# giladfrid009/WTracker

Measured on AMD Instinct MI355X. Metric: frames/sec YOLOv8s+ResMLP sim loop @640x640, higher is better.
Workload: dtype f16x3; 1 GPU; BASELINE configs[2]: full sim loop, YOLOv8s (nc=1, seeded synthetic weights) + ResMLP(imaging-100ms_pred-40ms_moving-50ms, reference weights); batch_per_gpu=64, lanes_per_gpu=2, global_batch=64, headline_mode=f16x3, parallelism=single GPU

## Files before the change

wtracker_amd/csrc/conv3x3_halo.hip:

```cpp
#include "wtk_kernels.h"

#include <cstdlib>
#include <type_traits>

namespace wtk {

typedef _Float16 half8 __attribute__((ext_vector_type(8)));
typedef float floatx4 __attribute__((ext_vector_type(4)));

namespace {

template <typename T> struct ElemH;
template <> struct ElemH<_Float16> {
    static constexpr int CE = 8;
};
template <> struct ElemH<float> {
    static constexpr int CE = 4;
};

__device__ __forceinline__ float silu_h(float x) {
    return wtk_silu_scaled(x);
}

__device__ __forceinline__ void mma_h(const uint4 &wf, const uint4 &pf, floatx4 &acc, _Float16 *) {
    acc = __builtin_amdgcn_mfma_f32_16x16x32_f16(__builtin_bit_cast(half8, wf), __builtin_bit_cast(half8, pf), acc, 0, 0, 0);
}
__device__ __forceinline__ void mma_h(const uint4 &wf, const uint4 &pf, floatx4 &acc, float *) {
    acc = __builtin_amdgcn_mfma_f32_16x16x4f32(__builtin_bit_cast(float, wf.x), __builtin_bit_cast(float, pf.x), acc, 0, 0, 0);
    acc = __builtin_amdgcn_mfma_f32_16x16x4f32(__builtin_bit_cast(float, wf.y), __builtin_bit_cast(float, pf.y), acc, 0, 0, 0);
    acc = __builtin_amdgcn_mfma_f32_16x16x4f32(__builtin_bit_cast(float, wf.z), __builtin_bit_cast(float, pf.z), acc, 0, 0, 0);
    acc = __builtin_amdgcn_mfma_f32_16x16x4f32(__builtin_bit_cast(float, wf.w), __builtin_bit_cast(float, pf.w), acc, 0, 0, 0);
}

template <int NV> __device__ __forceinline__ void load_run_h(const _Float16 *p, float (&v)[NV]) {
#pragma unroll
    for (int i = 0; i < NV; i += 8) {
        half8 h = *reinterpret_cast<const half8 *>(p + i);
#pragma unroll
        for (int j = 0; j < 8; ++j) v[i + j] = (float)h[j];
    }
}
template <int NV> __device__ __forceinline__ void load_run_h(const float *p, float (&v)[NV]) {
#pragma unroll
    for (int i = 0; i < NV; i += 4) {
        float4 f = *reinterpret_cast<const float4 *>(p + i);
        v[i] = f.x, v[i + 1] = f.y, v[i + 2] = f.z, v[i + 3] = f.w;
    }
}
template <int NV> __device__ __forceinline__ void store_run_h(_Float16 *p, const float (&v)[NV]) {
#pragma unroll
    for (int i = 0; i < NV; i += 8) {
        half8 h;
#pragma unroll
        for (int j = 0; j < 8; ++j) h[j] = (_Float16)v[i + j];
        *reinterpret_cast<half8 *>(p + i) = h;
    }
}
template <int NV> __device__ __forceinline__ void store_run_h(float *p, const float (&v)[NV]) {
#pragma unroll
    for (int i = 0; i < NV; i += 4) *reinterpret_cast<float4 *>(p + i) = make_float4(v[i], v[i + 1], v[i + 2], v[i + 3]);
}

constexpr int kBM = 256;

template <bool RAW> __device__ __forceinline__ void lds_dma16(const char *src, char *lds_dst) {
    if constexpr (RAW) {
        const unsigned lds = (unsigned)(uintptr_t)(__attribute__((address_space(3))) char *)lds_dst;
        asm volatile("s_mov_b32 m0, %1\n\ts_nop 0\n\tglobal_load_lds_dwordx4 %0, off" ::"v"(src), "s"(lds) : "memory");
    } else {
        __builtin_amdgcn_global_load_lds((const __attribute__((address_space(1))) void *)src, (__attribute__((address_space(3))) void *)lds_dst, 16, 0, 0);
    }
}

#ifndef WTK_HALO_BUFFER_DMA
#define WTK_HALO_BUFFER_DMA 1
#endif
typedef int rsrc_t __attribute__((ext_vector_type(4)));
__device__ __forceinline__ rsrc_t make_rsrc(const void *base) {
    const unsigned long long b = (unsigned long long)base;
    rsrc_t r;
    r.x = (int)(unsigned)(b & 0xffffffffu);
    r.y = (int)(unsigned)((b >> 32) & 0xffffu);
    r.z = (int)0xffffff00u;
    r.w = 0x00020000;
    return r;
}
__device__ __forceinline__ void lds_dma16_buf(const rsrc_t &rs, unsigned voff, unsigned soff, char *lds_dst) {
    const unsigned lds = (unsigned)(uintptr_t)(__attribute__((address_space(3))) char *)lds_dst;
    asm volatile("s_mov_b32 m0, %3\n\ts_nop 0\n\tbuffer_load_dwordx4 %0, %1, %2 offen lds" ::"v"(voff), "s"(rs), "s"(soff), "s"(lds) : "memory");
}

__device__ __forceinline__ void wait_vmcnt(int n) {
    switch (n) {
    case 0: asm volatile("s_waitcnt vmcnt(0)" ::: "memory"); break;
    case 1: asm volatile("s_waitcnt vmcnt(1)" ::: "memory"); break;
    case 2: asm volatile("s_waitcnt vmcnt(2)" ::: "memory"); break;
    case 3: asm volatile("s_waitcnt vmcnt(3)" ::: "memory"); break;
    case 4: asm volatile("s_waitcnt vmcnt(4)" ::: "memory"); break;
    case 5: asm volatile("s_waitcnt vmcnt(5)" ::: "memory"); break;
    case 6: asm volatile("s_waitcnt vmcnt(6)" ::: "memory"); break;
    case 7: asm volatile("s_waitcnt vmcnt(7)" ::: "memory"); break;
    case 8: asm volatile("s_waitcnt vmcnt(8)" ::: "memory"); break;
    case 9: asm volatile("s_waitcnt vmcnt(9)" ::: "memory"); break;
    case 10: asm volatile("s_waitcnt vmcnt(10)" ::: "memory"); break;
    case 11: asm volatile("s_waitcnt vmcnt(11)" ::: "memory"); break;
    case 12: asm volatile("s_waitcnt vmcnt(12)" ::: "memory"); break;
    case 13: asm volatile("s_waitcnt vmcnt(13)" ::: "memory"); break;
    case 14: asm volatile("s_waitcnt vmcnt(14)" ::: "memory"); break;
    case 15: asm volatile("s_waitcnt vmcnt(15)" ::: "memory"); break;
    case 16: asm volatile("s_waitcnt vmcnt(16)" ::: "memory"); break;
    default: asm volatile("s_waitcnt vmcnt(0)" ::: "memory"); break;
    }
}

__device__ __forceinline__ bool halo_in_coords(const HaloArgs &a, int flat, int xs, int &n, int &iy, int &ix) {
    const int rho = (int)fdiv((unsigned)flat, a.d_pitch);
    const int cc = flat - rho * a.pitch;
    n = (int)fdiv((unsigned)rho, a.d_h1);
    iy = rho - n * (a.H + 1) - 1;
    ix = xs + cc - 1;
    return n < a.N && iy >= 0 && (unsigned)ix < (unsigned)a.W;
}
__device__ __forceinline__ bool halo_out_coords(const HaloArgs &a, int o, int xs, int &n, int &y, int &x) {
    const int q = (int)fdiv((unsigned)o, a.d_pitch);
    x = o - q * a.pitch;
    n = (int)fdiv((unsigned)q, a.d_h1);
    y = q - n * (a.H + 1);
    return n < a.N && y < a.H && x < a.S && xs + x < a.W;
}

template <typename T, int KMAX>
__device__ __forceinline__ void halo_piece_offsets(const HaloArgs &a, int o0, int xs, int n_base, int halo_rows, int wave, int lane, unsigned (&hoff)[KMAX],
                                                   unsigned &hvalid) {
    static_assert(KMAX <= 8, "one lane per (piece, row)");
    constexpr int CE = ElemH<T>::CE;
    const int hr_e = (wave + 8 * (lane >> 3)) * 8 + (lane & 7);
    int pn, iy, ix;
    const bool ok_e = halo_in_coords(a, o0 + hr_e, xs, pn, iy, ix) && hr_e < halo_rows;
    const unsigned row_e = ok_e ? (unsigned)(((((long long)(pn - n_base) * a.H + iy) * a.W + ix) * a.in_ld) * (long long)sizeof(T)) : 0xffffffffu;
    const unsigned lc_term = (unsigned)((((lane & 7) ^ ((lane >> 3) & 7)) * CE) * (int)sizeof(T));
    hvalid = 0;
#pragma unroll
    for (int q = 0; q < KMAX; ++q) {
        const unsigned v = (unsigned)__builtin_amdgcn_ds_bpermute((q * 8 + (lane >> 3)) * 4, (int)row_e);
        const bool ok = v != 0xffffffffu;
        hoff[q] = ok ? v + lc_term : 0u;
        hvalid |= ok ? (1u << q) : 0u;
    }
}
__device__ __forceinline__ void halo_out_pixel(const HaloArgs &a, int o_first, int xs, int lane, int &pix_e, int &col_e) {
    int n, y, x;
    const bool ok = halo_out_coords(a, o_first + lane, xs, n, y, x);
    col_e = xs + x;
    pix_e = ok ? (n * a.H + y) * a.W + col_e : -1;
}
__device__ __forceinline__ int lane_fetch(int src_lane, int v) { return __builtin_amdgcn_ds_bpermute(src_lane * 4, v); }

template <typename T, int BN, int NHALO, int MINW, int NWB, int HROWS, int BMT = 256, bool TAIL = false, bool SPLIT = false>
__global__ __launch_bounds__(512, MINW) void conv3x3_halo_kernel(const HaloArgs a) {
    static_assert(!SPLIT || (sizeof(T) == 2 && BN != 192 && (MINW <= 2 || (BN == 64 && BMT == 128 && NHALO == 1))),
                  "split mode: fp16 storage, 64 / 128 couts, 256-register budget (128 for the two-blocks-per-CU form: 64 couts x 128 pixels, one window buffer)");
#ifdef WTK_HALO_STAMPS
    const unsigned long long st_t0 = __builtin_amdgcn_s_memrealtime();
#endif
    asm volatile("" ::"s"(a.in), "s"(a.w), "s"(a.bias), "s"(a.zeros), "s"(a.in_ld), "s"(a.in_coff), "s"(a.N), "s"(a.H), "s"(a.W), "s"(a.Cin), "s"(a.CoutPad),
                 "s"(a.Kpad), "s"(a.S), "s"(a.pitch), "s"(a.strips), "s"(a.d_strips.mul), "s"(a.d_strips.sh1), "s"(a.d_strips.sh2), "s"(a.d_pitch.mul),
                 "s"(a.d_pitch.sh1), "s"(a.d_pitch.sh2), "s"(a.d_nct.mul), "s"(a.d_nct.sh1), "s"(a.d_nct.sh2), "s"(a.d_h1.mul), "s"(a.d_h1.sh1), "s"(a.d_h1.sh2), "s"(a.grid));
    constexpr int CE = ElemH<T>::CE;
    constexpr int CCH = 8 * CE;
    constexpr int WAVES_C = BN == 64 ? 1 : 2, WAVES_P = 8 / WAVES_C;
    constexpr int WC = BN / WAVES_C;
    constexpr int WP = BMT / WAVES_P, TP = WP / 16, TC = WC / 16, NV = 4 * TC;
    constexpr int WR = BN / 64;

    constexpr int kHaloBytesT = HROWS * 128;
    __shared__ __attribute__((aligned(16))) char halo0[kHaloBytesT];
    __shared__ __attribute__((aligned(16))) char halo1[NHALO == 2 ? kHaloBytesT : 16];
    static_assert(NWB == 2 || NWB == 3 || (NWB == 6 && NHALO == 2 && !TAIL && SPLIT), "slab ring: 2, 3 or 6 (split tiles, two window buffers, no fused tail)");
    constexpr bool kRing = NWB >= 3;
    __shared__ __attribute__((aligned(16))) char wbuf0[NWB > 3 ? 16 : BN * 128];
    __shared__ __attribute__((aligned(16))) char wbuf1[NWB > 3 ? 16 : BN * 128];
    __shared__ __attribute__((aligned(16))) char wbuf2[NWB == 3 ? BN * 128 : 16];
    __shared__ __attribute__((aligned(16))) char wring[NWB > 3 ? NWB * BN * 128 : 16];

    const int tid = threadIdx.x;
    const int lane = tid & 63;
    const int wave = __builtin_amdgcn_readfirstlane(tid >> 6);
    const int wave_p = wave / WAVES_C, wave_c = wave % WAVES_C;
    const int lr = lane & 15, lg = lane >> 4;

    const int nct = a.CoutPad / BN;
    int nwg = a.grid;
    if (a.n_dyn) {
        const int lim = min(max(*a.n_dyn, 0), a.N) * (a.H + 1) * a.pitch;
        const int live = ((lim + BMT - 1) / BMT) * a.strips * nct;
        if ((int)blockIdx.x >= live) return;
        nwg = min(nwg, live);
    }
    int L;
    {
        const int bid = blockIdx.x;
        const int xcd = bid & 7, q = nwg >> 3, r = nwg & 7;
        L = (xcd < r ? xcd * (q + 1) : r * (q + 1) + (xcd - r) * q) + (bid >> 3);
    }
    const unsigned t = fdiv((unsigned)L, a.d_nct);
    const int n0 = (L - (int)t * nct) * BN;
    const int rb = (int)fdiv(t, a.d_strips);
    const int strip = (int)t - rb * a.strips;
    const int o0 = rb * BMT;
    const int xs = strip * a.S;
    const int pitch = a.pitch;
    const int halo_rows = BMT + 2 * pitch + 2;
    const int halo_pieces = (halo_rows + 7) >> 3;
    const int n_base = (int)fdiv(fdiv((unsigned)o0, a.d_pitch), a.d_h1);

    const T *in = reinterpret_cast<const T *>(a.in) + (long long)n_base * a.H * a.W * a.in_ld + a.in_coff;
    const T *wgt = reinterpret_cast<const T *>(a.w);
    const char *zero_page = reinterpret_cast<const char *>(a.zeros);

    constexpr int kMaxPiecesPerWave = (HROWS / 8 + 7) / 8;
    unsigned hoff[kMaxPiecesPerWave];
    unsigned hvalid;
    halo_piece_offsets<T, kMaxPiecesPerWave>(a, o0, xs, n_base, halo_rows, wave, lane, hoff, hvalid);
    const char *img = reinterpret_cast<const char *>(in);
    auto issue_halo_piece = [&](char *buf, int q, int c) {
        const int piece = wave + 8 * q;
        if (piece >= halo_pieces) return;
        if constexpr (kRing && WTK_HALO_BUFFER_DMA) {
            lds_dma16_buf(make_rsrc(img), ((hvalid >> q) & 1u) ? hoff[q] : 0xffffffffu, (unsigned)(c * (CCH * (int)sizeof(T))), buf + piece * 1024);
        } else {
            const char *src = ((hvalid >> q) & 1u) ? img + (size_t)c * (CCH * sizeof(T)) + hoff[q] : zero_page;
            lds_dma16<kRing>(src, buf + piece * 1024);
        }
    };
    auto issue_halo_piece_always = [&](char *buf, int q, int c) __attribute__((always_inline)) {
        constexpr int kPieces = HROWS / 8;
        static_assert(kPieces >= 16, "window buffer too small");
        const bool back = q > 0 && wave + 8 * q >= kPieces;
        const int piece = back ? wave + 8 * (q - 1) : wave + 8 * q;
        const unsigned off = back ? hoff[q > 0 ? q - 1 : 0] : hoff[q];
        const bool ok = back ? ((hvalid >> (q > 0 ? q - 1 : 0)) & 1u) : ((hvalid >> q) & 1u);
        if constexpr (kRing && WTK_HALO_BUFFER_DMA) {
            lds_dma16_buf(make_rsrc(img), ok ? off : 0xffffffffu, (unsigned)(c * (CCH * (int)sizeof(T))), buf + piece * 1024);
        } else {
            const char *src = ok ? img + (size_t)c * (CCH * sizeof(T)) + off : zero_page;
            lds_dma16<kRing>(src, buf + piece * 1024);
        }
    };
    const int wrow0 = tid >> 3, wp = tid & 7;
    unsigned wvoff[WR];
#pragma unroll
    for (int i = 0; i < WR; ++i) {
        const int row = wrow0 + 64 * i;
        const int key = ((row >> 1) & 1) | (((row / NV) & 3) << 1);
        wvoff[i] = (unsigned)(((long long)row * a.Kpad + (wp ^ key) * CE) * (long long)sizeof(T));
    }
    const char *wtile = reinterpret_cast<const char *>(wgt + (long long)n0 * a.Kpad);
    auto issue_weights = [&](char *buf, int tap, int c) {
        if constexpr (kRing && WTK_HALO_BUFFER_DMA) {
            const rsrc_t rs = make_rsrc(wtile);
            const unsigned so = (unsigned)((tap * a.Cin + c * CCH) * (int)sizeof(T));
#pragma unroll
            for (int i = 0; i < WR; ++i) lds_dma16_buf(rs, wvoff[i], so, buf + (64 * i + 8 * wave) * 128);
        } else {
            const char *ub = wtile + ((size_t)tap * a.Cin + (size_t)c * CCH) * sizeof(T);
#pragma unroll
            for (int i = 0; i < WR; ++i) lds_dma16<kRing>(ub + wvoff[i], buf + (64 * i + 8 * wave) * 128);
        }
    };

    floatx4 acc[TC][TP];
    floatx4 acc1[SPLIT ? TC : 1][SPLIT ? TP : 1];
#pragma unroll
    for (int i = 0; i < TC; ++i)
#pragma unroll
        for (int j = 0; j < TP; ++j) {
            acc[i][j] = (floatx4){0.f, 0.f, 0.f, 0.f};
            if constexpr (SPLIT) acc1[i][j] = (floatx4){0.f, 0.f, 0.f, 0.f};
        }

    const int wrow_l = wave_c * WC + (lr >> 2) * NV + (lr & 3);
    const int wkey_l = ((wrow_l >> 1) & 1) | (((wrow_l / NV) & 3) << 1);
    const unsigned wfrag0 = wrow_l * 128 + ((lg ^ wkey_l) << 4);
    const int prow0 = wave_p * WP + lr;

    auto compute_tap = [&](const char *halo, const char *wb, int tapoff) {
        const int base = prow0 + tapoff;
        const unsigned pfrag0 = base * 128 + ((lg ^ (base & 7)) << 4);
        if constexpr (SPLIT) {
            uint4 ph[TP], wh[TC], wl[TC], pl[TP];
#pragma unroll
            for (int j = 0; j < TP; ++j) ph[j] = *reinterpret_cast<const uint4 *>(halo + pfrag0 + j * 2048);
#pragma unroll
            for (int i = 0; i < TC; ++i) wh[i] = *reinterpret_cast<const uint4 *>(wb + wfrag0 + i * 512);
#pragma unroll
            for (int i = 0; i < TC; ++i) wl[i] = *reinterpret_cast<const uint4 *>(wb + (wfrag0 ^ 64u) + i * 512);
#pragma unroll
            for (int j = 0; j < TP; ++j) pl[j] = *reinterpret_cast<const uint4 *>(halo + (pfrag0 ^ 64u) + j * 2048);
#pragma unroll
            for (int i = 0; i < TC; ++i)
#pragma unroll
                for (int j = 0; j < TP; ++j) {
                    mma_h(wh[i], ph[j], acc[i][j], (T *)nullptr);
                    mma_h(wl[i], ph[j], acc1[i][j], (T *)nullptr);
                }
#pragma unroll
            for (int i = 0; i < TC; ++i)
#pragma unroll
                for (int j = 0; j < TP; ++j) mma_h(wh[i], pl[j], acc1[i][j], (T *)nullptr);
            return;
        }
#pragma unroll
        for (int kh2 = 0; kh2 < 2; ++kh2) {
            const unsigned pa = kh2 ? (pfrag0 ^ 64u) : pfrag0;
            const unsigned wa = kh2 ? (wfrag0 ^ 64u) : wfrag0;
            uint4 pf[TP], wf[TC];
#pragma unroll
            for (int j = 0; j < TP; ++j) pf[j] = *reinterpret_cast<const uint4 *>(halo + pa + j * 2048);
#pragma unroll
            for (int i = 0; i < TC; ++i) wf[i] = *reinterpret_cast<const uint4 *>(wb + wa + i * 512);
#pragma unroll
            for (int i = 0; i < TC; ++i)
#pragma unroll
                for (int j = 0; j < TP; ++j) mma_h(wf[i], pf[j], acc[i][j], (T *)nullptr);
        }
    };

    constexpr int kFr = (NWB > 3 && SPLIT) ? 2 * TP + 2 * TC : 1;
    uint4 fr[NWB > 3 ? 2 : 1][kFr];
    auto load_frags = [&](uint4(&f)[kFr], const char *halo, const char *wb, int tapoff) __attribute__((always_inline)) {
        if constexpr (NWB > 3 && SPLIT) {
            const int base = prow0 + tapoff;
            const unsigned pfrag0 = base * 128 + ((lg ^ (base & 7)) << 4);
#pragma unroll
            for (int j = 0; j < TP; ++j) f[j] = *reinterpret_cast<const uint4 *>(halo + pfrag0 + j * 2048);
#pragma unroll
            for (int i = 0; i < TC; ++i) f[2 * TP + i] = *reinterpret_cast<const uint4 *>(wb + wfrag0 + i * 512);
#pragma unroll
            for (int i = 0; i < TC; ++i) f[2 * TP + TC + i] = *reinterpret_cast<const uint4 *>(wb + (wfrag0 ^ 64u) + i * 512);
#pragma unroll
            for (int j = 0; j < TP; ++j) f[TP + j] = *reinterpret_cast<const uint4 *>(halo + (pfrag0 ^ 64u) + j * 2048);
        }
    };
    auto mma_frags = [&](const uint4(&f)[kFr]) __attribute__((always_inline)) {
        if constexpr (NWB > 3 && SPLIT) {
#pragma unroll
            for (int i = 0; i < TC; ++i)
#pragma unroll
                for (int j = 0; j < TP; ++j) {
                    mma_h(f[2 * TP + i], f[j], acc[i][j], (T *)nullptr);
                    mma_h(f[2 * TP + TC + i], f[j], acc1[i][j], (T *)nullptr);
                }
#pragma unroll
            for (int i = 0; i < TC; ++i)
#pragma unroll
                for (int j = 0; j < TP; ++j) mma_h(f[2 * TP + i], f[TP + j], acc1[i][j], (T *)nullptr);
        }
    };

    const int nchunks = a.Cin / CCH;
    const int cb = n0 + wave_c * WC + lg * NV;
#pragma unroll
    for (int i = 0; i < TC; ++i) {
        const floatx4 b4 = (floatx4){a.bias[cb + i * 4 + 0], a.bias[cb + i * 4 + 1], a.bias[cb + i * 4 + 2], a.bias[cb + i * 4 + 3]};
#pragma unroll
        for (int j = 0; j < TP; ++j) acc[i][j] = b4;
    }

#ifdef WTK_HALO_STAMPS
    const unsigned long long st_t1 = __builtin_amdgcn_s_memrealtime();
#endif
// ... 1158 lines not shown
#pragma unroll
            for (int i = 0; i < TC; ++i) wh[i] = *reinterpret_cast<const uint4 *>(wb + wfrag0 + i * 512);
#pragma unroll
            for (int i = 0; i < TC; ++i) wl[i] = *reinterpret_cast<const uint4 *>(wb + (wfrag0 ^ 64u) + i * 512);
#pragma unroll
            for (int j = 0; j < TP; ++j) pl[j] = *reinterpret_cast<const uint4 *>(win + (pfrag0 ^ 64u) + j * 2048);
#pragma unroll
            for (int i = 0; i < TC; ++i)
#pragma unroll
                for (int j = 0; j < TP; ++j) {
                    mma_h(wh[i], ph[j], acc[i][j], (T *)nullptr);
                    mma_h(wl[i], ph[j], acc1[i][j], (T *)nullptr);
                }
#pragma unroll
            for (int i = 0; i < TC; ++i)
#pragma unroll
                for (int j = 0; j < TP; ++j) mma_h(wh[i], pl[j], acc1[i][j], (T *)nullptr);
            return;
        }
#pragma unroll
        for (int kh2 = 0; kh2 < 2; ++kh2) {
            const unsigned pa = kh2 ? (pfrag0 ^ 64u) : pfrag0;
            const unsigned wa = kh2 ? (wfrag0 ^ 64u) : wfrag0;
            uint4 pf[TP], wf[TC];
#pragma unroll
            for (int j = 0; j < TP; ++j) pf[j] = *reinterpret_cast<const uint4 *>(win + pa + j * 2048);
#pragma unroll
            for (int i = 0; i < TC; ++i) wf[i] = *reinterpret_cast<const uint4 *>(wb + wa + i * 512);
#pragma unroll
            for (int i = 0; i < TC; ++i)
#pragma unroll
                for (int j = 0; j < TP; ++j) mma_h(wf[i], pf[j], acc[i][j], (T *)nullptr);
        }
    };

    constexpr int kStepTap[9] =      { 0, 2, 6, 8,  3, 5,  1, 7,  4};
    constexpr int kStepDY[9] =       {-1,-1, 0, 0,  0, 0, -1, 0,  0};
    constexpr int kStepDX[9] =       {-1, 0,-1, 0, -1, 0,  0, 0,  0};
    constexpr int kStepBuf[9] =      { 0, 0, 0, 0,  1, 1,  0, 0,  1};
    constexpr int kStepReq[9] =      { 2, 2, 2, 0,  KW,0,  KW,0,  KW};
    constexpr int kStepReqFrom[9] =  { 0, 2, 4, 0,  0, 0,  0, 0,  0};
    constexpr int kNextPy[9] =       { 0, 0, 0, 0,  1, 1,  0, 0,  1};
    constexpr int kNextPx[9] =       { 1, 1, 1, 1,  0, 0,  0, 0,  1};
    static_assert(KW == 6, "request schedule written for six window pieces per wave");
    const int nchunks = a.Cin / 64;

#pragma unroll
    for (int q = 0; q < KW; ++q) issue_piece(win0, q, 1, 1, 0);
    issue_weights(wbuf0, kStepTap[0], 0);
    issue_weights(wbuf1, kStepTap[1], 0);
    asm volatile("s_waitcnt vmcnt(0)" ::: "memory");
    __syncthreads();

    auto step = [&](auto s_tag, int c, bool more) __attribute__((always_inline)) {
        constexpr int S = decltype(s_tag)::value;
        const char *wcur = S % 3 == 0 ? wbuf0 : (S % 3 == 1 ? wbuf1 : wbuf2);
        char *wnext2 = (S + 2) % 3 == 0 ? wbuf0 : ((S + 2) % 3 == 1 ? wbuf1 : wbuf2);
        const char *wcur_win = kStepBuf[S] ? win1 : win0;
        char *wnext_win = kStepBuf[S] ? win0 : win1;
        compute_tap(wcur_win, wcur, (kStepDY[S] + 1) * pitch + (kStepDX[S] + 1));
        const int cn = S == 8 ? (more ? c + 1 : c) : c;
        if constexpr (kStepReq[S] > 0) {
#pragma unroll
            for (int q = 0; q < kStepReq[S]; ++q) issue_piece(wnext_win, kStepReqFrom[S] + q, kNextPy[S], kNextPx[S], cn);
        }
        if constexpr (S < 7)
            issue_weights(wnext2, kStepTap[S + 2], c);
        else
            issue_weights(wnext2, kStepTap[S - 7], more ? c + 1 : c);
        constexpr bool plane_end = S == 3 || S == 5 || S == 7 || S == 8;
        wait_vmcnt(plane_end ? WR : WR + kStepReq[S]);
        asm volatile("s_waitcnt lgkmcnt(0)" ::: "memory");
        __builtin_amdgcn_s_barrier();
        asm volatile("" ::: "memory");
    };
    for (int c = 0; c < nchunks; ++c) {
        const bool more = c + 1 < nchunks;
        step(std::integral_constant<int, 0>{}, c, more);
        step(std::integral_constant<int, 1>{}, c, more);
        step(std::integral_constant<int, 2>{}, c, more);
        step(std::integral_constant<int, 3>{}, c, more);
        step(std::integral_constant<int, 4>{}, c, more);
        step(std::integral_constant<int, 5>{}, c, more);
        step(std::integral_constant<int, 6>{}, c, more);
        step(std::integral_constant<int, 7>{}, c, more);
        step(std::integral_constant<int, 8>{}, c, more);
    }

    int pix_e, col_e;
    halo_out_pixel(a, o0 + wave_p * WP, 0, lane, pix_e, col_e);
    long long pixj[TP];
#pragma unroll
    for (int j = 0; j < TP; ++j) pixj[j] = lane_fetch(j * 16 + lr, pix_e);
    T *out = reinterpret_cast<T *>(a.out);
    if (cb + NV <= a.Cout) {
#pragma unroll
        for (int j = 0; j < TP; ++j) {
            if (pixj[j] < 0) continue;
            float v[NV];
#pragma unroll
            for (int i = 0; i < TC; ++i)
#pragma unroll
                for (int r = 0; r < 4; ++r) {
                    if constexpr (SPLIT)
                        v[i * 4 + r] = wtk_split_value(acc[i][j][r], acc1[i][j][r]);
                    else
                        v[i * 4 + r] = acc[i][j][r];
                }
            if (a.act) {
                wtk_silu_scaled_run<NV>(v);
            }
            if constexpr (SPLIT)
                wtk_split_store<NV>(reinterpret_cast<_Float16 *>(a.out) + pixj[j] * a.out_ld + a.out_coff, cb, v);
            else
                store_run_h<NV>(out + pixj[j] * a.out_ld + a.out_coff + cb, v);
        }
    }
    asm volatile("s_waitcnt vmcnt(0)" ::: "memory");
}

template <int BMT, bool SPLIT = false> hipError_t launch_s2(HaloArgs a, hipStream_t stream) {
    const long long blocks = (long long)a.blocks_per_strip * (a.CoutPad / 128);
    if (blocks <= 0 || blocks > 0x7fffffffLL) return hipErrorInvalidValue;
    a.d_nct = make_fastdiv((unsigned)(a.CoutPad / 128));
    a.d_bps = make_fastdiv((unsigned)a.blocks_per_strip);
    a.d_strips = make_fastdiv(1u);
    a.d_pitch = make_fastdiv((unsigned)a.pitch);
    a.d_h1 = make_fastdiv((unsigned)(a.H + 1));
    a.grid = (int)blocks;
    hipLaunchKernelGGL((conv3x3_s2_kernel<BMT, SPLIT>), dim3((unsigned)blocks), dim3(512), 0, stream, a);
    return hipGetLastError();
}

template <typename T, int BN, int HROWS> hipError_t launch_hp(HaloArgs a, int num_cus, hipStream_t stream) {
    const long long tiles = (long long)a.strips * a.blocks_per_strip * (a.CoutPad / BN);
    if (tiles <= 0 || tiles > 0x3fffffffLL || num_cus < 8) return hipErrorInvalidValue;
    if (kBM + 2 * a.pitch + 2 > HROWS || (a.Cin / (8 * ElemH<T>::CE)) % 2 != 0) return hipErrorInvalidValue;
    a.d_nct = make_fastdiv((unsigned)(a.CoutPad / BN));
    a.d_bps = make_fastdiv((unsigned)a.blocks_per_strip);
    a.d_strips = make_fastdiv((unsigned)a.strips);
    a.d_pitch = make_fastdiv((unsigned)a.pitch);
    a.d_h1 = make_fastdiv((unsigned)(a.H + 1));
    const long long cap = num_cus / 8 * 8;
    const unsigned grid = (unsigned)(tiles < cap ? tiles : cap);
    a.grid = (int)grid;
    hipLaunchKernelGGL((conv3x3_halo_pkernel<T, BN, HROWS>), dim3(grid), dim3(512), 0, stream, a);
    return hipGetLastError();
}

template <typename T, int BN, int NHALO, int MINW, int NWB, int HROWS, int BMT = 256, bool TAIL = false, bool SPLIT = false> hipError_t launch_h(HaloArgs a, hipStream_t stream) {
    const long long blocks = (long long)a.strips * a.blocks_per_strip * (a.CoutPad / BN);
    if (blocks <= 0 || blocks > 0x7fffffffLL) return hipErrorInvalidValue;
    if (BMT + 2 * a.pitch + 2 > HROWS || (long long)a.blocks_per_strip * BMT < (long long)a.N * (a.H + 1) * a.pitch) return hipErrorInvalidValue;
    a.d_nct = make_fastdiv((unsigned)(a.CoutPad / BN));
    a.d_bps = make_fastdiv((unsigned)a.blocks_per_strip);
    a.d_strips = make_fastdiv((unsigned)a.strips);
    a.d_pitch = make_fastdiv((unsigned)a.pitch);
    a.d_h1 = make_fastdiv((unsigned)(a.H + 1));
    a.grid = (int)blocks;
    hipLaunchKernelGGL((conv3x3_halo_kernel<T, BN, NHALO, MINW, NWB, HROWS, BMT, TAIL, SPLIT>), dim3((unsigned)blocks), dim3(512), 0, stream, a);
    return hipGetLastError();
}

}

bool halo_eligible(int k, int stride, int cin, int is_f16) {
    const int cch = is_f16 ? 64 : 32;
    return k == 3 && stride == 1 && cin % cch == 0;
}

bool split_halo_eligible(int k, int stride, int cin, int cout) { return k == 3 && stride == 1 && cin % 32 == 0 && cout % 64 == 0; }
int split_halo_cout_tile(int cout_stored) { return cout_stored % 128 == 0 ? 128 : 64; }

hipError_t launch_conv3x3_halo_split(const HaloArgs &a, hipStream_t stream) {
    const int bn = (a.narrow && !a.tail_w) ? 64 : split_halo_cout_tile(a.Cout);
    if (a.Cin % 64 != 0 || a.CoutPad % bn != 0 || a.Cout != a.CoutPad || a.slabs == 2) return hipErrorInvalidValue;
    if (a.tail_w && a.Cout == 128) {
        if (a.res || a.out2 || !a.tail_bias || !a.tail_out || a.tail_kpad != 256 || a.tail_cout < 1 || a.tail_cout > 32 || !a.tail_f32 || a.tail_ld % 4 || a.tail_coff % 4) return hipErrorInvalidValue;
    } else if (a.tail_w && (a.Cout != 64 || a.res || a.out2 || !a.tail_bias || !a.tail_out || a.tail_kpad != 128 || a.tail_cout != 64 || (a.tail_f32 ? (a.tail_ld % 4 || a.tail_coff % 4) : (a.tail_ld % 64 || a.tail_coff % 64))))
        return hipErrorInvalidValue;
    if (a.in_ld % 64 || a.in_coff % 64 || a.out_ld % 64 || a.out_coff % 64 || a.Kpad != 9 * a.Cin) return hipErrorInvalidValue;
    if (a.pitch != (a.strips == 1 ? a.S + 1 : a.S + 2) || kBM + 2 * a.pitch + 2 > kHaloRowsMax || a.strips * a.S < a.W || (a.strips == 1 && a.S != a.W))
        return hipErrorInvalidValue;
    const int bm = a.bm == 128 ? 128 : kBM;
    if ((long long)a.blocks_per_strip * bm < (long long)a.N * (a.H + 1) * a.pitch) return hipErrorInvalidValue;
    if (a.res && (a.res_ld % 64 || a.res_coff % 64)) return hipErrorInvalidValue;
    if (a.out2 && (a.out2_ld % 64 || a.out2_coff % 64)) return hipErrorInvalidValue;
    if (bn == 128 && a.tail_w) return bm == 128 ? launch_h<_Float16, 128, 2, 2, 3, kHaloRowsMax, 128, true, true>(a, stream) : launch_h<_Float16, 128, 2, 2, 3, kHaloRowsMax, 256, true, true>(a, stream);
    if (bn == 128) return bm == 128 ? launch_h<_Float16, 128, 2, 2, 3, kHaloRowsMax, 128, false, true>(a, stream) : launch_h<_Float16, 128, 2, 2, 3, kHaloRowsMax, 256, false, true>(a, stream);
    if (a.tail_w) return bm == 128 ? launch_h<_Float16, 64, 2, 2, 3, kHaloRowsMax, 128, true, true>(a, stream) : launch_h<_Float16, 64, 2, 2, 3, kHaloRowsMax, 256, true, true>(a, stream);
    if (a.deep && bm == 128) return launch_h<_Float16, 64, 2, 1, 6, kHaloRowsMax, 128, false, true>(a, stream);
    return bm == 128 ? launch_h<_Float16, 64, 2, 2, 3, kHaloRowsMax, 128, false, true>(a, stream) : launch_h<_Float16, 64, 2, 2, 3, kHaloRowsMax, 256, false, true>(a, stream);
}

int halo_rows_max(int cout_stored, int slabs) { return (slabs == 3 && halo_cout_tile(cout_stored) == 192) ? kHaloRowsSmall : kHaloRowsMax; }

void halo_geometry(int H, int W, int rows_max, int *S, int *pitch, int *strips, int *blocks_per_strip, int bm) {
    const int smax = (rows_max - kBM - 2) / 2 - 2;
    *strips = (W + smax - 1) / smax;
    *S = (W + *strips - 1) / *strips;
    *pitch = *S + 2;
    *blocks_per_strip = (H * *pitch + bm - 1) / bm;
}

void halo_geometry_stacked(int N, int H, int W, int rows_max, int *S, int *pitch, int *strips, int *blocks_per_strip, int bm) {
    const int smax = (rows_max - kBM - 2) / 2 - 2;
    *strips = (W + smax - 1) / smax;
    *S = (W + *strips - 1) / *strips;
    *pitch = *strips == 1 ? *S + 1 : *S + 2;
    *blocks_per_strip = (int)(((long long)N * (H + 1) * *pitch + bm - 1) / bm);
}

bool s2win_eligible(int k, int stride, int cin, int cout, int cout_pad, int is_f16, int wo, bool plain) {
    return is_f16 && k == 3 && stride == 2 && cin % 64 == 0 && cin >= 128 && cout_pad % 128 == 0 && cout % 16 == 0 && plain && 256 + (wo + 1) + 2 <= kS2Rows;
}

hipError_t launch_conv3x3_s2(const HaloArgs &a, hipStream_t stream) {
    if (a.Cin % 64 || a.CoutPad % 128 || a.Cout > a.CoutPad || a.Cout % 16 || a.out2 || a.tail_w || a.res || a.Kpad < 9 * a.Cin || a.Kpad % 64) return hipErrorInvalidValue;
    if (a.in_ld % 8 || a.in_coff % 8 || a.out_ld % 8 || a.out_coff % 8) return hipErrorInvalidValue;
    const int bm = a.bm == 128 ? 128 : 256;
    if (a.strips != 1 || a.S != a.W || a.pitch != a.W + 1 || bm + a.pitch + 2 > kS2Rows) return hipErrorInvalidValue;
    if ((long long)a.blocks_per_strip * bm < (long long)a.N * (a.H + 1) * a.pitch) return hipErrorInvalidValue;
    return bm == 128 ? launch_s2<128>(a, stream) : launch_s2<256>(a, stream);
}

bool split_s2win_eligible(int k, int stride, int cin, int cout, int cout_pad, int wo, bool plain) {
    return k == 3 && stride == 2 && cin % 32 == 0 && cout_pad % 128 == 0 && cout == cout_pad && plain && 256 + (wo + 1) + 2 <= kS2Rows;
}
hipError_t launch_conv3x3_s2_split(const HaloArgs &a, hipStream_t stream) {
    if (a.Cin % 64 || a.CoutPad % 128 || a.Cout != a.CoutPad || a.out2 || a.tail_w || a.res || a.Kpad != 9 * a.Cin) return hipErrorInvalidValue;
    if (a.in_ld % 64 || a.in_coff % 64 || a.out_ld % 64 || a.out_coff % 64) return hipErrorInvalidValue;
    const int bm = a.bm == 128 ? 128 : 256;
    if (a.strips != 1 || a.S != a.W || a.pitch != a.W + 1 || bm + a.pitch + 2 > kS2Rows) return hipErrorInvalidValue;
    if ((long long)a.blocks_per_strip * bm < (long long)a.N * (a.H + 1) * a.pitch) return hipErrorInvalidValue;
    return bm == 128 ? launch_s2<128, true>(a, stream) : launch_s2<256, true>(a, stream);
}

int ws64_rows_max() { return kWsRows; }

bool ws64_eligible(int k, int stride, int cin, int cout, int cout_pad, int is_f16, bool has_out2, bool has_tail) {
    return is_f16 && k == 3 && stride == 1 && cin == 64 && cout == 64 && cout_pad == 64 && !has_out2 && !has_tail;
}

hipError_t launch_conv3x3_ws64(const HaloArgs &a, int num_cus, hipStream_t stream) {
    if (a.Cin != 64 || a.Cout != 64 || a.CoutPad != 64 || a.out2 || a.tail_w || a.Kpad < 576 || a.Kpad % 64) return hipErrorInvalidValue;
    if (a.in_ld % 8 || a.in_coff % 8 || a.out_ld % 8 || a.out_coff % 8) return hipErrorInvalidValue;
    if (a.res && (a.res_ld % 8 || a.res_coff % 8)) return hipErrorInvalidValue;
    if (a.pitch != (a.strips == 1 ? a.S + 1 : a.S + 2) || a.strips * a.S < a.W || (a.strips == 1 && a.S != a.W)) return hipErrorInvalidValue;
    if ((long long)a.blocks_per_strip * 256 < (long long)a.N * (a.H + 1) * a.pitch) return hipErrorInvalidValue;
    return launch_ws64(a, num_cus, stream);
}

int halo_cout_tile(int cout_stored) { return cout_stored % 128 == 0 ? 128 : (cout_stored % 192 == 0 ? 192 : 64); }

hipError_t launch_conv3x3_halo(const HaloArgs &a, int is_f16, hipStream_t stream) {
    const int ce = is_f16 ? 8 : 4;
    const int cch = 8 * ce;
    const int bn = (a.narrow && !a.tail_w && a.CoutPad % 64 == 0) ? 64 : halo_cout_tile(a.Cout);
    if (a.Cin % cch != 0 || a.CoutPad % bn != 0 || a.Cout > a.CoutPad || a.Cout % (bn == 192 ? 24 : 16) != 0) return hipErrorInvalidValue;
    if (a.in_ld % ce || a.in_coff % ce || a.out_ld % ce || a.out_coff % ce || a.Kpad % cch || a.Kpad < 9 * a.Cin) return hipErrorInvalidValue;
    if (a.pitch != (a.strips == 1 ? a.S + 1 : a.S + 2) || kBM + 2 * a.pitch + 2 > kHaloRowsMax || a.strips * a.S < a.W || (a.strips == 1 && a.S != a.W))
        return hipErrorInvalidValue;
    if (a.tail_w && (!is_f16 || (bn != 64 && bn != 128) || a.Cout != bn || a.CoutPad != bn || a.res || a.out2 || !a.tail_bias || !a.tail_out ||
                     a.tail_kpad < bn || a.tail_kpad % 8 || a.tail_ld % 8 || a.tail_coff % 8 || a.slabs == 2))
        return hipErrorInvalidValue;
    const int bm = a.bm == 128 ? 128 : kBM;
    if ((long long)a.blocks_per_strip * bm < (long long)a.N * (a.H + 1) * a.pitch) return hipErrorInvalidValue;
    if (a.res && (a.res_ld % ce || a.res_coff % ce)) return hipErrorInvalidValue;
    if (a.out2 && (a.out2_ld % ce || a.out2_coff % ce)) return hipErrorInvalidValue;
    const int nchunks = a.Cin / cch;
    const long long tiles = (long long)a.strips * a.blocks_per_strip * (a.CoutPad / bn);
    if (a.slabs != 2 && !a.tail_w && bm == kBM && a.persist_cus > 0 && 2 * tiles >= 3 * (long long)a.persist_cus && nchunks % 2 == 0 && (bn == 128 || bn == 192)) {
        if (is_f16) return bn == 128 ? launch_hp<_Float16, 128, kHaloRowsMax>(a, a.persist_cus, stream) : launch_hp<_Float16, 192, kHaloRowsSmall>(a, a.persist_cus, stream);
        return bn == 128 ? launch_hp<float, 128, kHaloRowsMax>(a, a.persist_cus, stream) : launch_hp<float, 192, kHaloRowsSmall>(a, a.persist_cus, stream);
    }
    if (a.tail_w && bn == 128) {
        if (bm == 128) return launch_h<_Float16, 128, 2, 2, 3, kHaloRowsMax, 128, true>(a, stream);
        return launch_h<_Float16, 128, 2, 2, 3, kHaloRowsMax, 256, true>(a, stream);
    }
    if (a.tail_w) {
        if (bm == 128) return nchunks == 1 ? launch_h<_Float16, 64, 1, 4, 3, kHaloRowsMax, 128, true>(a, stream) : launch_h<_Float16, 64, 2, 2, 3, kHaloRowsMax, 128, true>(a, stream);
        return nchunks == 1 ? launch_h<_Float16, 64, 1, 4, 3, kHaloRowsMax, 256, true>(a, stream) : launch_h<_Float16, 64, 2, 2, 3, kHaloRowsMax, 256, true>(a, stream);
    }
    if (a.slabs != 2 && bm == 128) {
        if (is_f16) {
            if (bn == 128) return launch_h<_Float16, 128, 2, 2, 3, kHaloRowsMax, 128>(a, stream);
            if (bn == 192) return launch_h<_Float16, 192, 2, 2, 3, kHaloRowsSmall, 128>(a, stream);
            if (nchunks == 1) return launch_h<_Float16, 64, 1, 4, 3, kHaloRowsMax, 128>(a, stream);
            return launch_h<_Float16, 64, 2, 2, 3, kHaloRowsMax, 128>(a, stream);
        }
        if (bn == 128) return launch_h<float, 128, 2, 2, 3, kHaloRowsMax, 128>(a, stream);
        if (bn == 192) return launch_h<float, 192, 2, 2, 3, kHaloRowsSmall, 128>(a, stream);
        if (nchunks == 1) return launch_h<float, 64, 1, 4, 3, kHaloRowsMax, 128>(a, stream);
        return launch_h<float, 64, 2, 2, 3, kHaloRowsMax, 128>(a, stream);
    }
    if (bm != kBM) return hipErrorInvalidValue;
    if (a.slabs != 2) {
        if (is_f16) {
            if (bn == 128) return launch_h<_Float16, 128, 2, 2, 3, kHaloRowsMax>(a, stream);
            if (bn == 192) return launch_h<_Float16, 192, 2, 2, 3, kHaloRowsSmall>(a, stream);
            if (nchunks == 1) return launch_h<_Float16, 64, 1, 4, 3, kHaloRowsMax>(a, stream);
            return launch_h<_Float16, 64, 2, 2, 3, kHaloRowsMax>(a, stream);
        }
        if (bn == 128) return launch_h<float, 128, 2, 2, 3, kHaloRowsMax>(a, stream);
        if (bn == 192) return launch_h<float, 192, 2, 2, 3, kHaloRowsSmall>(a, stream);
        if (nchunks == 1) return launch_h<float, 64, 1, 4, 3, kHaloRowsMax>(a, stream);
// ... 16 lines not shown
```

wtracker_amd/csrc/head.hip:

```cpp
#include "wtk_kernels.h"

namespace wtk {

template <typename T> __device__ __forceinline__ float ldf(const T *p) { return (float)*p; }

constexpr int kStatusNonFinite = 1;
__device__ __forceinline__ bool not_finite(float x) { return !(fabsf(x) <= 3.402823466e+38f); }

__device__ __forceinline__ void better(float &s, int &i, float s2, int i2) {
    if (s2 > s || (s2 == s && i2 < i)) {
        s = s2;
        i = i2;
    }
}

template <typename T>
__global__ __launch_bounds__(1024) void head_select_kernel(const HeadArgs a) {
    const int n = blockIdx.x;
    const int A0 = a.lh[0] * a.lw[0], A1 = a.lh[1] * a.lw[1], A2 = a.lh[2] * a.lw[2];
    const int A = A0 + A1 + A2;

    float best = -INFINITY, best_l = -INFINITY, second = -INFINITY;
    int best_i = 0x7fffffff;
    bool bad = false;
    auto merge = [](float &b, int &bi, float &bl, float &s2nd, float b2, int bi2, float bl2, float s2) __attribute__((always_inline)) {
        if (b2 > b || (b2 == b && bi2 < bi)) {
            s2nd = fmaxf(fmaxf(bl, s2nd), s2);
            b = b2;
            bi = bi2;
            bl = bl2;
        } else {
            s2nd = fmaxf(fmaxf(bl2, s2nd), s2);
        }
    };
    for (int i = threadIdx.x; i < A; i += 1024) {
        int lvl, j;
        if (i < A0) {
            lvl = 0, j = i;
        } else if (i < A0 + A1) {
            lvl = 1, j = i - A0;
        } else {
            lvl = 2, j = i - A0 - A1;
        }
        const int Al = lvl == 0 ? A0 : (lvl == 1 ? A1 : A2);
        const T *c = reinterpret_cast<const T *>(a.cls[lvl]) + ((long long)n * Al + j) * a.cls_ld;
        float m = ldf(c);
        bad |= not_finite(m);
        for (int k = 1; k < a.nc; ++k) {
            const float v = ldf(c + k);
            bad |= not_finite(v);
            m = fmaxf(m, v);
        }
        merge(best, best_i, best_l, second, 1.0f / (1.0f + expf(-m)), i, m, -INFINITY);
    }
    if (bad && a.status) __hip_atomic_fetch_or(a.status, kStatusNonFinite, __ATOMIC_RELAXED, __HIP_MEMORY_SCOPE_SYSTEM);
#pragma unroll
    for (int off = 32; off >= 1; off >>= 1) {
        const float b2 = __shfl_xor(best, off, 64);
        const int i2 = __shfl_xor(best_i, off, 64);
        const float l2 = __shfl_xor(best_l, off, 64);
        const float s2 = __shfl_xor(second, off, 64);
        merge(best, best_i, best_l, second, b2, i2, l2, s2);
    }
    __shared__ float ws[16], wl[16], wsec[16];
    __shared__ int wi[16];
    if ((threadIdx.x & 63) == 0) {
        ws[threadIdx.x >> 6] = best;
        wi[threadIdx.x >> 6] = best_i;
        wl[threadIdx.x >> 6] = best_l;
        wsec[threadIdx.x >> 6] = second;
    }
    __syncthreads();
    if (threadIdx.x >= 64) return;
    best = ws[0];
    best_i = wi[0];
    best_l = wl[0];
    second = wsec[0];
#pragma unroll
    for (int w = 1; w < 16; ++w) merge(best, best_i, best_l, second, ws[w], wi[w], wl[w], wsec[w]);
    if (a.out_margin && threadIdx.x == 0) a.out_margin[n] = fminf(best_l - second, fabsf(best_l - a.conf_logit));

    const float score = best;
    const bool keep = (best_i != 0x7fffffff) && (score > a.conf);

    float dist = 0.f;
    int lvl = 0, j = 0;
    if (keep) {
        if (best_i < A0) {
            lvl = 0, j = best_i;
        } else if (best_i < A0 + A1) {
            lvl = 1, j = best_i - A0;
        } else {
            lvl = 2, j = best_i - A0 - A1;
        }
    }
    const int lane = threadIdx.x;
    if (keep && lane < 4) {
        const int Al = lvl == 0 ? A0 : (lvl == 1 ? A1 : A2);
        const T *b = reinterpret_cast<const T *>(a.box[lvl]) + ((long long)n * Al + j) * 64 + lane * 16;
        float x[16];
        float mx = -INFINITY;
        bool badb = false;
#pragma unroll
        for (int k = 0; k < 16; ++k) {
            x[k] = ldf(b + k);
            badb |= not_finite(x[k]);
            mx = fmaxf(mx, x[k]);
        }
        if (badb && a.status) __hip_atomic_fetch_or(a.status, kStatusNonFinite, __ATOMIC_RELAXED, __HIP_MEMORY_SCOPE_SYSTEM);
        float sum = 0.f;
#pragma unroll
        for (int k = 0; k < 16; ++k) {
            x[k] = expf(x[k] - mx);
            sum += x[k];
        }
        float d = 0.f;
#pragma unroll
        for (int k = 0; k < 16; ++k) d += (x[k] / sum) * (float)k;
        dist = d;
    }
    const float dl = __shfl(dist, 0, 64), dt = __shfl(dist, 1, 64), dr = __shfl(dist, 2, 64), db = __shfl(dist, 3, 64);
    if (lane != 0) return;
    float *o = a.out_xywh + (long long)n * 4;
    if (!keep) {
        const float nanv = __builtin_nanf("");
        o[0] = o[1] = o[2] = o[3] = nanv;
        if (a.out_conf) a.out_conf[n] = 0.f;
        if (a.out_anchor) a.out_anchor[n] = -1;
        return;
    }
    const int w_l = a.lw[lvl];
    const float stride = lvl == 0 ? 8.f : (lvl == 1 ? 16.f : 32.f);
    const float ax = (float)(j % w_l) + 0.5f, ay = (float)(j / w_l) + 0.5f;
    const float x1 = ax - dl, y1 = ay - dt, x2 = ax + dr, y2 = ay + db;
    const float cx = (x1 + x2) / 2.f * stride, cy = (y1 + y2) / 2.f * stride;
    const float w = (x2 - x1) * stride, h = (y2 - y1) * stride;
    float bx1 = cx - w / 2.f, by1 = cy - h / 2.f, bx2 = cx + w / 2.f, by2 = cy + h / 2.f;
    bx1 = (bx1 - a.pad_x) / a.gain;
    bx2 = (bx2 - a.pad_x) / a.gain;
    by1 = (by1 - a.pad_y) / a.gain;
    by2 = (by2 - a.pad_y) / a.gain;
    bx1 = fminf(fmaxf(bx1, 0.f), a.img_w);
    bx2 = fminf(fmaxf(bx2, 0.f), a.img_w);
    by1 = fminf(fmaxf(by1, 0.f), a.img_h);
    by2 = fminf(fmaxf(by2, 0.f), a.img_h);
    o[0] = bx1;
    o[1] = by1;
    o[2] = bx2 - bx1;
    o[3] = by2 - by1;
    if (a.out_conf) a.out_conf[n] = score;
    if (a.out_anchor) a.out_anchor[n] = best_i;
}

constexpr float kNmsMaxWh = 7680.f;

template <typename T> __device__ __forceinline__ void decode_anchor(const HeadArgs &a, int n, int lvl, int j, int Al, float (&xyxy)[4]) {
    const T *b = reinterpret_cast<const T *>(a.box[lvl]) + ((long long)n * Al + j) * 64;
    float dist[4];
#pragma unroll
    for (int side = 0; side < 4; ++side) {
        float x[16];
        float mx = -INFINITY;
#pragma unroll
        for (int k = 0; k < 16; ++k) {
            x[k] = ldf(b + side * 16 + k);
            mx = fmaxf(mx, x[k]);
        }
        float sum = 0.f;
#pragma unroll
        for (int k = 0; k < 16; ++k) {
            x[k] = expf(x[k] - mx);
            sum += x[k];
        }
        float d = 0.f;
#pragma unroll
        for (int k = 0; k < 16; ++k) d += (x[k] / sum) * (float)k;
        dist[side] = d;
    }
    const int w_l = a.lw[lvl];
    const float stride = lvl == 0 ? 8.f : (lvl == 1 ? 16.f : 32.f);
    const float ax = (float)(j % w_l) + 0.5f, ay = (float)(j / w_l) + 0.5f;
    const float x1 = ax - dist[0], y1 = ay - dist[1], x2 = ax + dist[2], y2 = ay + dist[3];
    const float cx = (x1 + x2) / 2.f * stride, cy = (y1 + y2) / 2.f * stride;
    const float w = (x2 - x1) * stride, h = (y2 - y1) * stride;
    xyxy[0] = cx - w / 2.f, xyxy[1] = cy - h / 2.f, xyxy[2] = cx + w / 2.f, xyxy[3] = cy + h / 2.f;
}

template <typename T>
__global__ __launch_bounds__(1024) void head_nms_kernel(const NmsArgs q) {
    const HeadArgs &a = q.h;
    const int n = blockIdx.x;
    const int A0 = a.lh[0] * a.lw[0], A1 = a.lh[1] * a.lw[1], A2 = a.lh[2] * a.lw[2];
    const int A = A0 + A1 + A2;
    float *sc = q.scratch_score + (long long)n * A;
    int *cl = q.scratch_cls + (long long)n * A;
    float *bx = q.scratch_box + (long long)n * A * 4;
    for (int i = threadIdx.x; i < A; i += 1024) {
        int lvl, j;
        if (i < A0) {
            lvl = 0, j = i;
        } else if (i < A0 + A1) {
            lvl = 1, j = i - A0;
        } else {
            lvl = 2, j = i - A0 - A1;
        }
        const int Al = lvl == 0 ? A0 : (lvl == 1 ? A1 : A2);
        const T *c = reinterpret_cast<const T *>(a.cls[lvl]) + ((long long)n * Al + j) * a.cls_ld;
        float m = ldf(c);
        int mk = 0;
        bool bad = not_finite(m);
        for (int k = 1; k < a.nc; ++k) {
            const float v = ldf(c + k);
            bad |= not_finite(v);
            if (v > m) m = v, mk = k;
        }
        if (bad && a.status) __hip_atomic_fetch_or(a.status, kStatusNonFinite, __ATOMIC_RELAXED, __HIP_MEMORY_SCOPE_SYSTEM);
        const float score = 1.0f / (1.0f + expf(-m));
        const bool cand = score > a.conf;
        sc[i] = cand ? score : -INFINITY;
        cl[i] = mk;
        if (cand) {
            float b4[4];
            decode_anchor<T>(a, n, lvl, j, Al, b4);
            bx[4 * i + 0] = b4[0], bx[4 * i + 1] = b4[1], bx[4 * i + 2] = b4[2], bx[4 * i + 3] = b4[3];
        }
    }
    __syncthreads();
    __shared__ float ws[16];
    __shared__ int wi[16];
    __shared__ float kept[4];
    __shared__ int kept_i;
    int count = 0;
    for (int det = 0; det < q.max_det; ++det) {
        float best = -INFINITY;
        int best_i = 0x7fffffff;
        for (int i = threadIdx.x; i < A; i += 1024) {
            const float s = sc[i];
            if (s > -INFINITY) better(best, best_i, s, i);
        }
#pragma unroll
        for (int off = 32; off >= 1; off >>= 1) {
            const float s2 = __shfl_xor(best, off, 64);
            const int i2 = __shfl_xor(best_i, off, 64);
            better(best, best_i, s2, i2);
        }
        if ((threadIdx.x & 63) == 0) ws[threadIdx.x >> 6] = best, wi[threadIdx.x >> 6] = best_i;
        __syncthreads();
        if (threadIdx.x == 0) {
            float b = ws[0];
            int bi = wi[0];
            for (int w = 1; w < 16; ++w) better(b, bi, ws[w], wi[w]);
            kept_i = bi;
            if (bi != 0x7fffffff) {
                const int kc = cl[bi];
                const float x1 = bx[4 * bi], y1 = bx[4 * bi + 1], x2 = bx[4 * bi + 2], y2 = bx[4 * bi + 3];
                const float offc = (float)kc * kNmsMaxWh;
                kept[0] = x1 + offc, kept[1] = y1 + offc, kept[2] = x2 + offc, kept[3] = y2 + offc;
                float ox1 = (x1 - a.pad_x) / a.gain, ox2 = (x2 - a.pad_x) / a.gain, oy1 = (y1 - a.pad_y) / a.gain, oy2 = (y2 - a.pad_y) / a.gain;
                ox1 = fminf(fmaxf(ox1, 0.f), a.img_w), ox2 = fminf(fmaxf(ox2, 0.f), a.img_w);
                oy1 = fminf(fmaxf(oy1, 0.f), a.img_h), oy2 = fminf(fmaxf(oy2, 0.f), a.img_h);
                const long long r = (long long)n * q.max_det + det;
                q.out_xywh[4 * r] = ox1, q.out_xywh[4 * r + 1] = oy1, q.out_xywh[4 * r + 2] = ox2 - ox1, q.out_xywh[4 * r + 3] = oy2 - oy1;
                if (q.out_conf) q.out_conf[r] = b;
                if (q.out_cls) q.out_cls[r] = kc;
                if (q.out_anchor) q.out_anchor[r] = bi;
                sc[bi] = -INFINITY;
            }
        }
        __syncthreads();
        if (kept_i == 0x7fffffff) break;
        ++count;
        if (det + 1 == q.max_det) break;
        const float k0 = kept[0], k1 = kept[1], k2 = kept[2], k3 = kept[3];
        const float ka = (k2 - k0) * (k3 - k1);
        for (int i = threadIdx.x; i < A; i += 1024) {
            if (!(sc[i] > -INFINITY)) continue;
            const float offc = (float)cl[i] * kNmsMaxWh;
            const float b0 = bx[4 * i] + offc, b1 = bx[4 * i + 1] + offc, b2 = bx[4 * i + 2] + offc, b3 = bx[4 * i + 3] + offc;
            const float ix1 = fmaxf(k0, b0), iy1 = fmaxf(k1, b1), ix2 = fminf(k2, b2), iy2 = fminf(k3, b3);
            const float inter = fmaxf(ix2 - ix1, 0.f) * fmaxf(iy2 - iy1, 0.f);
            const float ba = (b2 - b0) * (b3 - b1);
            if (inter / (ka + ba - inter) > q.iou) sc[i] = -INFINITY;
        }
        __syncthreads();
    }
    for (int r = count + threadIdx.x; r < q.max_det; r += 1024) {
        const long long o = (long long)n * q.max_det + r;
        const float nanv = __builtin_nanf("");
        q.out_xywh[4 * o] = q.out_xywh[4 * o + 1] = q.out_xywh[4 * o + 2] = q.out_xywh[4 * o + 3] = nanv;
        if (q.out_conf) q.out_conf[o] = 0.f;
        if (q.out_cls) q.out_cls[o] = -1;
        if (q.out_anchor) q.out_anchor[o] = -1;
    }
    if (threadIdx.x == 0 && q.out_count) q.out_count[n] = count;
}

hipError_t launch_head_nms(const NmsArgs &a, int is_f16, hipStream_t stream) {
    if (a.h.N <= 0 || a.h.nc < 1 || a.h.cls_ld < a.h.nc || a.max_det < 1 || !a.scratch_score || !a.scratch_cls || !a.scratch_box || !a.out_xywh)
        return hipErrorInvalidValue;
    if (is_f16)
        hipLaunchKernelGGL((head_nms_kernel<_Float16>), dim3(a.h.N), dim3(1024), 0, stream, a);
    else
        hipLaunchKernelGGL((head_nms_kernel<float>), dim3(a.h.N), dim3(1024), 0, stream, a);
    return hipGetLastError();
}

hipError_t launch_head(const HeadArgs &a, int is_f16, hipStream_t stream) {
    if (a.N <= 0 || a.nc < 1 || a.cls_ld < a.nc) return hipErrorInvalidValue;
    if (is_f16)
        hipLaunchKernelGGL((head_select_kernel<_Float16>), dim3(a.N), dim3(1024), 0, stream, a);
    else
        hipLaunchKernelGGL((head_select_kernel<float>), dim3(a.N), dim3(1024), 0, stream, a);
    return hipGetLastError();
}

}
```

wtracker_amd/csrc/wtk_internal.h:

```cpp
#pragma once
#include "../../include/wtk_hip.h"
#include "wtk_kernels.h"

#include <cstring>
#include <map>
#include <mutex>
#include <string>
#include <utility>
#include <vector>

namespace wtk {
int fail(const std::string &msg);
int fail_hip(const char *what, hipError_t e);
int ensure_attributes(int device);
}
#define HIP_TRY(expr)                                                                                                          \
    do {                                                                                                                       \
        hipError_t _e = (expr);                                                                                                \
        if (_e != hipSuccess) return wtk::fail_hip(#expr, _e);                                                                 \
    } while (0)

struct DeviceGuard {
    int prev = -1;
    bool switched = false;
    hipError_t err = hipSuccess;
    explicit DeviceGuard(int device) {
        err = hipGetDevice(&prev);
        if (err == hipSuccess && prev != device) {
            err = hipSetDevice(device);
            switched = err == hipSuccess;
        }
    }
    ~DeviceGuard() {
        if (switched) (void)hipSetDevice(prev);
    }
};
#define DEVICE_GUARD(h)                                                                                                        \
    DeviceGuard _guard((h)->device);                                                                                           \
    if (_guard.err != hipSuccess) return wtk::fail_hip("selecting the handle's device", _guard.err)

inline uint16_t f32_to_f16_bits(float f) {
    _Float16 h = (_Float16)f;
    uint16_t b;
    std::memcpy(&b, &h, 2);
    return b;
}

inline float f16_bits_to_f32(uint16_t b) {
    _Float16 h;
    std::memcpy(&h, &b, 2);
    return (float)h;
}


struct ConvSpec {
    std::string name;
    int cout, cin, k, stride, act;
};

struct ModelDims {
    int c[5];
    int n[4];
    int hb, hc;
    int nc;
};

struct Buf {
    size_t elems_per_image = 0;
    int h = 0, w = 0, C = 0;
    int f32 = 0;
    void *ptr = nullptr;
};

enum OpKind { OP_STEM, OP_CONV, OP_POOL };

struct Op {
    OpKind kind;
    int in_buf = -1, in_coff = 0, cin = 0;
    int out_buf = -1, out_coff = 0;
    int out2_buf = -1, out2_coff = 0;
    int res_buf = -1, res_coff = 0;
    int tail_op = -1;
    int folded = 0;
    int in2_buf = -1, in2_coff = 0, in2_split = 0;
    int cout = 0, cout_pad = 0, k = 1, stride = 1, act = 1;
    int cfg = 0;
    int K = 0, Kpad = 0;
    int tile_w = 0;
    int halo = 0;
    int side = 0;
    int wait_feat = -1;
    int signal_feat = -1;
    void *w = nullptr;
    float *bias = nullptr;
    double macs_per_image = 0;
    int spec = -1;
    int sk = 0;
    int sk_atoms = 0;
    float *sk_partial = nullptr;
    unsigned *sk_tickets = nullptr;
};

enum ProfClass {
    PROF_STEM = 0,
    PROF_IGEMM = 1,
    PROF_POOL = 2,
    PROF_HEAD = 3,
    PROF_HALO = 4,
    PROF_FUSED = 5,
    PROF_C32 = 6,
};

enum LaunchKind { L_IGEMM, L_IGEMM_SPLIT, L_WIDE_1X1, L_HALO, L_HALO_SPLIT, L_C32, L_C32_SPLIT, L_WS64, L_S2WIN, L_S2WIN_SPLIT, L_SK };
struct ConvLaunch {
    LaunchKind kind;
    ProfClass cls;
    int cfg;
    wtk::ConvArgs a;
    wtk::HaloArgs g;
};

struct wtk_yolo {
    int device = 0;
    int is_f16 = 1;
    int esize = 2;
    int split = 0;
    const int *n_dyn = nullptr;
    int S_h = 0, S_w = 0, max_batch = 0;
    ModelDims dims;
    std::vector<Buf> bufs;
    std::vector<Op> ops;
    std::vector<std::pair<void *, size_t>> dev_allocs;
    int box_buf[3] = {-1, -1, -1}, cls_buf[3] = {-1, -1, -1};
    int lh[3] = {0, 0, 0}, lw[3] = {0, 0, 0};
    int cls_ld = 32;
    double macs_per_frame = 0;
    int anchors = 0;
    uint8_t *frames_dev = nullptr;
    size_t frames_cap = 0;
    uint8_t *lb_dev = nullptr;
    size_t lb_cap = 0;
    void *zero_page = nullptr;
    float *o_xywh = nullptr, *o_conf = nullptr;
    float *o_margin = nullptr;
    int *o_anchor = nullptr;
    float *nms_score = nullptr, *nms_box = nullptr;
    int *nms_cls = nullptr;
    int use_halo = 1;
    int front_debug = 0;
    int use_tail = 1;
    int use_tail_cls_split = 1;
    int halo_small_blocks = 1;
    int halo_persist = 1;
    int halo_slabs = 3;
    int use_c32s = 1;
    int use_s2win = 1;
    int use_ws64 = 1;
    int use_wide = 1;
    int use_c2f = 0;
    int use_front = 0;
    int num_cus = 0;
    int latency = 0;
    int sk_group = 1;
    int sk_force_tile = -1, sk_force_form = -1;
    std::map<long long, wtk::SkChoice> sk_choices;
    int sk_autotune = 1;
    int tune_pass = -1;
    std::map<long long, std::vector<wtk::SkChoice>> sk_cands;
    std::map<long long, std::vector<float>> tune_ms;
    std::vector<hipEvent_t> tune_ev;
    std::vector<long long> tune_key;
    std::vector<int> sk_tuned;
    std::vector<std::vector<int>> lat_sched;
    int small_narrow = 0;
    int halo_deep = 0;
    int *status_host = nullptr;
    int *status_dev = nullptr;
    int status_static = 0;
    int profiling = 0;
    static constexpr int kProfKernels = 7, kProfEvents = 96;
    hipEvent_t ev[kProfEvents];
    static constexpr int kSideStreams = 3;
    hipStream_t side_stream[kSideStreams] = {};
    hipEvent_t feat_ev[2] = {nullptr, nullptr}, side_done[kSideStreams] = {};
    int use_side = 1;
    int side_streams = 2;
    hipStream_t host_stream = nullptr;
    int ev_created = 0;
    double prof_ms[kProfKernels] = {};
    double prof_flops[kProfKernels] = {};
    long long prof_launches[kProfKernels] = {};
};

namespace wtk {
int pooled_stream(int device, hipStream_t *s);
void unpool_stream(int device, hipStream_t s);
}
```

wtracker_amd/csrc/wtk_kernels.h:

```cpp
#pragma once
#include <hip/hip_runtime.h>
#include <stdint.h>

namespace wtk {

struct FastDiv {
    unsigned mul, sh1, sh2;
};
inline FastDiv make_fastdiv(unsigned d) {
    FastDiv f;
    if (d == 0) d = 1;
    unsigned l = 0;
    while ((1ull << l) < d) ++l;
    const unsigned long long m = ((1ull << 32) * ((1ull << l) - d)) / d + 1;
    f.mul = (unsigned)m;
    f.sh1 = l < 1 ? l : 1;
    f.sh2 = l > 0 ? l - 1 : 0;
    return f;
}
__device__ __forceinline__ unsigned fdiv(unsigned n, const FastDiv &f) {
    const unsigned t = __umulhi(n, f.mul);
    return (t + ((n - t) >> f.sh1)) >> f.sh2;
}

// ... 59 lines not shown
#pragma unroll
        for (int j = 0; j < 8; ++j) {
            const _Float16 h = (_Float16)v[i + j];
            hv[j] = h;
            lv[j] = (_Float16)((v[i + j] - (float)h) * kSplitScale);
        }
        *reinterpret_cast<wtk_h8 *>(p + i) = hv;
        *reinterpret_cast<wtk_h8 *>(p + 32 + i) = lv;
    }
}
template <int NV> __device__ __forceinline__ void wtk_split_load(const _Float16 *pix, int c, float (&v)[NV]) {
    static_assert(NV % 8 == 0 && NV <= 32, "runs of 8 channels inside one 32-channel block");
    const _Float16 *p = pix + 64 * (c >> 5) + (c & 31);
#pragma unroll
    for (int i = 0; i < NV; i += 8) {
        const wtk_h8 hv = *reinterpret_cast<const wtk_h8 *>(p + i), lv = *reinterpret_cast<const wtk_h8 *>(p + 32 + i);
#pragma unroll
        for (int j = 0; j < 8; ++j) v[i + j] = wtk_split_value((float)hv[j], (float)lv[j]);
    }
}

struct ConvArgs {
    const void *in;
    int in_ld, in_coff;
    int N, H, W, Cin;
    int Ho, Wo, Cout;
    int CoutPad;
    int KH, KW, stride, pad;
    const void *w;
    const float *bias;
    void *out;
    int out_ld, out_coff;
    void *out2;
    int out2_ld, out2_coff;
    const void *res;
    int res_ld, res_coff;
    const void *in2;
    int in2_ld, in2_coff, in2_split;
    int act;
    int K, Kpad;
    int tile_w;
    int tiles_x, tiles_y;
    long long M;
    int ptiles;
    FastDiv d_howo, d_wo, d_tilew, d_tilesx, d_tpi, d_nct;
    const void *zeros;
    const void *tail_w;
    const float *tail_bias;
    void *tail_out;
    int tail_kpad, tail_ld, tail_coff, tail_act;
    const int *n_dyn;
#ifdef WTK_IGEMM_STAMPS
    unsigned long long *dbg_stamps;
#endif
    int out_f32;
};

enum ConvCfg { CFG_128x128 = 0, CFG_256x64 = 1, CFG_256x32 = 2, CFG_128x64 = 4 };
int conv_cfg_bm(int cfg);
int conv_cfg_bn(int cfg);
hipError_t launch_conv(const ConvArgs &a, int cfg, int is_f16, hipStream_t stream);
hipError_t launch_conv_split(const ConvArgs &a, int cfg, hipStream_t stream);
hipError_t conv_init_attributes();
int conv_sk_slices(int nk);
bool conv_sk_eligible(const ConvArgs &a, int split);
int conv_sk_plan_atoms(long long M, int cout_pad, int nk, int num_cus, int split);
size_t conv_sk_partial_bytes(const ConvArgs &a, int split, int atoms = 0);
size_t conv_sk_ticket_count(long long M, int cout_pad);
hipError_t launch_conv_sk(const ConvArgs &a, int split, int atoms, float *partial, unsigned *tickets, int num_cus, hipStream_t stream);
constexpr int kSkGroupMax = 4;
struct SkMember {
    ConvArgs a;
    int atoms;
    float *partial;
    unsigned *tickets;
};
struct SkChoice {
    int valid = 0;
    int separate = 0;
    int tile = 3;
    int S[kSkGroupMax] = {1, 1, 1, 1};
    int m_tile[kSkGroupMax] = {3, 3, 3, 3}, m_S[kSkGroupMax] = {1, 1, 1, 1};
    double est_us = 0.0;
};
hipError_t launch_conv_sk_group(const SkMember *m, int n, int split, int num_cus, int force_tile, int force_form, hipStream_t stream, struct SkChoice *choice);
constexpr int kSkMaxCandidates = 4 * (1 << kSkGroupMax);
int conv_sk_enumerate(const SkMember *m, int n, int split, int num_cus, int force_tile, int force_form, SkChoice *out, int cap);
struct SkArgs {
    const char *in;
    unsigned in_ldb, in_offb;
    const char *in2;
    unsigned in2_ldb, in2_offb;
    int in2_blocks;
    int N, H, W, Ho, Wo;
    int cpb;
    int KW, stride, pad;
    int nk, S;
    int NA;
    const char *w;
    unsigned w_rowb;
    const float *bias;
    int Cout, CoutPad, act;
    void *out;
    int out_ld, out_coff, out_f32;
    const void *res;
    int res_ld, res_coff;
    float *partial;
    unsigned *tickets;
    long long M;
    int ptiles, nct;
    FastDiv d_ptiles, d_nct, d_howo, d_wo, d_cpb, d_cg;
    const int *n_dyn;
};

struct SkGroupArgs {
    SkArgs p[kSkGroupMax];
    unsigned first[kSkGroupMax];
};
bool conv1x1_wide_eligible(const ConvArgs &a, int is_f16);
hipError_t launch_conv1x1_wide(ConvArgs a, hipStream_t stream);

constexpr int kHaloRowsMax = 432;
constexpr int kHaloRowsSmall = 352;
struct HaloArgs {
    const void *in;
    int in_ld, in_coff;
    int N, H, W, Cin;
    int Cout, CoutPad;
    const void *w;
    const float *bias;
    void *out;
    int out_ld, out_coff;
    void *out2;
    int out2_ld, out2_coff;
    const void *res;
    int res_ld, res_coff;
    int act;
    int Kpad;
    int S, pitch, strips, blocks_per_strip;
    const void *zeros;
    unsigned long long *dbg_stamps;
    const void *tail_w;
    const float *tail_bias;
    void *tail_out;
    int tail_kpad, tail_ld, tail_coff;
    int tail_cout;
    int tail_f32;
    int bm;
    int persist_cus;
    int slabs;
    int deep;
    int narrow;
    int grid;
    const int *n_dyn;
    FastDiv d_bps, d_strips, d_pitch, d_nct, d_h1;
};
bool halo_eligible(int k, int stride, int cin, int is_f16);
bool split_halo_eligible(int k, int stride, int cin, int cout);
int split_halo_cout_tile(int cout_stored);
hipError_t launch_conv3x3_halo_split(const HaloArgs &a, hipStream_t stream);
bool split_s2win_eligible(int k, int stride, int cin, int cout, int cout_pad, int wo, bool plain);
hipError_t launch_conv3x3_s2_split(const HaloArgs &a, hipStream_t stream);
int halo_rows_max(int cout_stored, int slabs);
void halo_geometry(int H, int W, int rows_max, int *S, int *pitch, int *strips, int *blocks_per_strip, int bm = 256);
void halo_geometry_stacked(int N, int H, int W, int rows_max, int *S, int *pitch, int *strips, int *blocks_per_strip, int bm = 256);
int halo_cout_tile(int cout_stored);
hipError_t launch_conv3x3_halo(const HaloArgs &a, int is_f16, hipStream_t stream);
bool s2win_eligible(int k, int stride, int cin, int cout, int cout_pad, int is_f16, int wo, bool plain);
hipError_t launch_conv3x3_s2(const HaloArgs &a, hipStream_t stream);
int ws64_rows_max();
bool ws64_eligible(int k, int stride, int cin, int cout, int cout_pad, int is_f16, bool has_out2, bool has_tail);
hipError_t launch_conv3x3_ws64(const HaloArgs &a, int num_cus, hipStream_t stream);
bool c32_eligible(int k, int stride, int cin, int cout_stored, int is_f16, bool has_out2);
hipError_t launch_conv3x3_c32(HaloArgs a, hipStream_t stream);
bool c32_split_eligible(int k, int stride, int cin, int cout, bool plain_out);
int c32_split_rows_max();
hipError_t launch_conv3x3_c32_split(HaloArgs a, hipStream_t stream);

struct StemArgs {
    const uint8_t *frames;
    int N, H, W, C;
    const void *w;
    const float *bias;
    void *out;
    int Cout;
    int Ho, Wo;
    int out_split;
    int in_split;
    const int *n_dyn;
};
hipError_t launch_stem(const StemArgs &a, int is_f16, hipStream_t stream);

struct FrontArgs {
    const uint8_t *frames;
    int N, H, W, C;
    const void *w0;
    const float *b0;
    const void *w1;
    const float *b1;
    int Kpad1;
    const void *w2;
    const float *b2;
    int Kpad2;
    void *out;
    int out_ld, out_coff;
    unsigned long long *dbg_stamps;
    void *dbg_t0, *dbg_t1;
    const int *n_dyn;
    int stem_split;
    int Ho, Wo, tiles_x, tiles_y, total_tiles;
    FastDiv d_tpi, d_tilesx;
};
struct C2fArgs {
    const void *cat;
    int cat_ld, a_coff, b_coff;
    int N, H, W;
    const void *w_m1, *w_m2;
    const float *b_m1, *b_m2;
    int Kpad_m;
    const void *w_cv2;
    const float *b_cv2;
    int Kpad_cv2;
    void *out;
    int out_ld, out_coff;
    const void *zeros;
    unsigned long long *dbg_stamps;
    int tiles_x, tiles_y, total_tiles;
    FastDiv d_tpi, d_tilesx;
};
bool c2f_fused_eligible(int is_f16, int c_hidden, int n_bottlenecks, int shortcut, int c_out);
hipError_t launch_c2f_fused(C2fArgs a, int num_cus, hipStream_t stream);

bool front_fused_eligible(int is_f16, int c0, int c1, int c2_out);
bool front_fused_split_eligible(int c0, int c1, int c2_out);
hipError_t launch_front_fused_split(FrontArgs a, int num_cus, hipStream_t stream);
hipError_t launch_front_fused(FrontArgs a, int num_cus, hipStream_t stream);

struct LetterboxArgs {
    const uint8_t *src;
    uint8_t *dst;
    int N, H, W, C;
    int Sh, Sw;
    int new_h, new_w;
    int top, left;
};
hipError_t launch_letterbox(const LetterboxArgs &a, hipStream_t stream);

struct CropArgs {
    const uint8_t *frames;
    const int *pos_xy;
    uint8_t *views;
    int N, H, W, C;
    int view_w, view_h;
    int rows, cols;
};
hipError_t launch_crop_views(const CropArgs &a, hipStream_t stream);

struct ViewLetterboxArgs {
    const uint8_t *frames;
    const int *frame_index;
    const int *pos_xy;
    uint8_t *dst;
    int N, H, W, C;
    int F;
    int view_w, view_h;
    int rows, cols;
    int Sh, Sw;
    int new_h, new_w, top, left;
};
hipError_t launch_view_letterbox(const ViewLetterboxArgs &a, hipStream_t stream);

struct PoolArgs {
    void *buf;
    int N, H, W, c;
    FastDiv d_w;
    int split;
};
hipError_t launch_sppf_pool(const PoolArgs &a, int is_f16, hipStream_t stream);
hipError_t pool_init_attributes();

struct HeadArgs {
    const void *box[3];
    const void *cls[3];
    int cls_ld;
    int nc;
    int lh[3], lw[3];
    int N;
    float conf;
    float gain, pad_x, pad_y;
    float img_w, img_h;
    float *out_xywh;
    float *out_conf;
    int *out_anchor;
    float *out_margin;
    float conf_logit;
    int *status;
};
hipError_t launch_head(const HeadArgs &a, int is_f16, hipStream_t stream);

struct NmsArgs {
    HeadArgs h;
    float iou;
    int max_det;
    float *scratch_score;
    int *scratch_cls;
    float *scratch_box;
    float *out_xywh;
    float *out_conf;
    int *out_cls;
    int *out_anchor;
    int *out_count;
};
hipError_t launch_head_nms(const NmsArgs &a, int is_f16, hipStream_t stream);

struct MlpLayerDev {
    int in_dim, out_dim;
    int in_pad;
    int out_pad;
    int relu;
    int w_off;
    int b_off;
    int pad_;
};
constexpr int kMlpMaxLayers = 64;
constexpr int kMlpMaxDim = 128;
constexpr int kMlpMaxInputFrames = 16;
struct MlpArgs {
    const float *params;
    int n_params;
    const MlpLayerDev *layers;
    int n_layers, n_blocks, layers_per_block;
    int in_dim, out_dim;
    const float *x;
    const float *track;
    int n_frames;
    const int *anchor_frames;
    int input_frames[kMlpMaxInputFrames];
    int n_in;
    int *valid;
    float *y;
    int B;
};
hipError_t launch_mlp(const MlpArgs &a, hipStream_t stream);

constexpr int kTrackMaxWindow = 64;
constexpr int kTrackMaxTimes = 16;
constexpr int kTrackMaxCoef = 8;
struct TrackMedianArgs {
    const void *track;
    int n_frames;
    const int *cycles;
    int n_samples;
    int cycle_frame_num, imaging_frame_num;
    double *pred;
    int *valid;
};
hipError_t launch_track_median(const TrackMedianArgs &a, int track_f64, hipStream_t stream);
struct TrackPolyfitArgs {
    const void *track;
    int n_frames;
    const int *cycles;
    int n_samples;
    int cycle_frame_num;
    int times[kTrackMaxTimes];
    double weights[kTrackMaxTimes];
    int n_times, degree;
    double t_eval;
    double *pred;
    int *valid;
};
hipError_t launch_track_polyfit(const TrackPolyfitArgs &a, int track_f64, hipStream_t stream);
struct TrackPairsArgs {
    const void *track;
    int n_frames;
    int row0, n_rows;
    int in_frames[kTrackMaxTimes], out_frames[kTrackMaxTimes];
    int n_in, n_out;
    float *X;
    float *Y;
    int *keep;
};
hipError_t launch_track_pairs(const TrackPairsArgs &a, int track_f64, hipStream_t stream);

struct RecheckArgs {
    const float *margins;
    int B, K;
    int *slots;
    float thr;
    const float *src_xywh, *src_conf;
    const int *src_anchor;
    float *dst_xywh, *dst_conf;
    int *dst_anchor;
    int *n_replaced;
    int *n_weak;
    int *n_overflow;
};
hipError_t launch_recheck_select(const RecheckArgs &a, hipStream_t stream);
hipError_t launch_recheck_merge(const RecheckArgs &a, hipStream_t stream);

struct RecheckQueueArgs {
    const float *margins;
    int B;
    float thr;
    const unsigned char *frames;
    long long frame_bytes;
    unsigned char *q_frames;
    int q_cap;
    int *q_len;
    float **q_xywh, **q_conf;
    int **q_anchor;
    float *dst_xywh, *dst_conf;
    int *dst_anchor;
    int *pos;
    int *n_overflow;
    const float *src_xywh, *src_conf;
    const int *src_anchor;
    int *n_replaced;
};
hipError_t launch_recheck_enqueue(const RecheckQueueArgs &a, hipStream_t stream);
hipError_t launch_recheck_scatter(const RecheckQueueArgs &a, hipStream_t stream);
hipError_t launch_recheck_gather_views(const int *slots, int K, const int *frame_index, const int *pos_xy, int *idx_out, int *pos_out, hipStream_t stream);

}
```

wtracker_amd/csrc/wtk_plan.hip:

```cpp
#include <execinfo.h>
#include <signal.h>
#include <unistd.h>

#include "wtk_internal.h"

#include <algorithm>
#include <cmath>
#include <cstdio>
#include <cstdlib>

using namespace wtk;

namespace {
static int make_divisible8(double x) { return (int)(std::ceil(x / 8.0) * 8.0); }

static ModelDims model_dims(float width, float depth, int max_ch, int nc) {
    ModelDims d;
    const int base[5] = {64, 128, 256, 512, 1024};
    for (int i = 0; i < 5; ++i) d.c[i] = make_divisible8(std::min(base[i], max_ch) * (double)width);
    const int nb[4] = {3, 6, 6, 3};
    for (int i = 0; i < 4; ++i) d.n[i] = std::max((int)std::lround(nb[i] * (double)depth), 1);
    d.hb = std::max(std::max(16, d.c[2] / 4), 64);
    d.hc = std::max(d.c[2], std::min(nc, 100));
    d.nc = nc;
// ... 172 lines not shown
        for (size_t i = 0; i < wf.size(); ++i) wh[i] = f32_to_f16_bits(wf[i]);
        if (dev_alloc(h, &op.w, wh.size() * 2)) return 1;
        HIP_TRY(hipMemcpy(op.w, wh.data(), wh.size() * 2, hipMemcpyHostToDevice));
    } else {
        if (dev_alloc(h, &op.w, wf.size() * 4)) return 1;
        HIP_TRY(hipMemcpy(op.w, wf.data(), wf.size() * 4, hipMemcpyHostToDevice));
    }
    return 0;
}

namespace {
struct Planner {
    wtk_yolo *h;
    const std::vector<ConvSpec> &specs;
    const wtk_conv_blob *blobs;
    bool failed = false;

    int new_buf(int hh, int ww, int C) {
        Buf b;
        b.h = hh;
        b.w = ww;
        b.C = C;
        b.elems_per_image = (size_t)hh * ww * C;
        h->bufs.push_back(b);
        return (int)h->bufs.size() - 1;
    }
    void conv(const std::vector<std::string> &names, int in_buf, int in_coff, int out_buf, int out_coff, int out2_buf = -1,
              int out2_coff = 0, int res_buf = -1, int res_coff = 0, int cout_store_pad = 0, int in2_buf = -1, int in2_coff = 0,
              int in2_split = 0) {
        if (failed) return;
        Op op;
        op.kind = OP_CONV;
        std::vector<const float *> wp, bp;
        std::vector<int> couts;
        int cout = 0;
        for (auto &nm : names) {
            const int i = find_spec(specs, nm);
            if (i < 0) {
                failed = true;
                fail("internal: unknown conv " + nm);
                return;
            }
            const ConvSpec &s = specs[i];
            if (op.spec < 0) op.spec = i;
            op.cin = s.cin;
            op.k = s.k;
            op.stride = s.stride;
            op.act = s.act;
            wp.push_back(blobs[i].weight);
            bp.push_back(blobs[i].bias);
            couts.push_back(s.cout);
            cout += s.cout;
        }
        op.cout = std::max(cout, cout_store_pad);
        op.cfg = pick_cfg(op.cout, op.k == 1 && op.stride == 1);
        if (h->split && op.cfg == CFG_256x64) op.cfg = CFG_128x64;
        op.in_buf = in_buf;
        op.in_coff = in_coff;
        op.out_buf = out_buf;
        op.out_coff = out_coff;
        op.out2_buf = out2_buf;
        op.out2_coff = out2_coff;
        op.res_buf = res_buf;
        op.res_coff = res_coff;
        op.in2_buf = in2_buf;
        op.in2_coff = in2_coff;
        op.in2_split = in2_split;
        if (in2_buf >= 0) {
            const Buf &lb = h->bufs[in2_buf];
            const Buf &hb = h->bufs[in_buf];
            if (op.cfg != CFG_128x128 || op.k != 1 || lb.h * 2 != hb.h || lb.w * 2 != hb.w || in2_coff + in2_split > lb.C || in2_split > op.cin) {
                failed = true;
                fail("internal: two-source conv " + names[0] + " does not fit the 128x128 loader");
                return;
            }
        }
        const Buf &ib = h->bufs[in_buf];
        const Buf &ob = h->bufs[out_buf];
        const int pad = op.k / 2;
        const int ho = (ib.h + 2 * pad - op.k) / op.stride + 1, wo = (ib.w + 2 * pad - op.k) / op.stride + 1;
        if (ho != ob.h || wo != ob.w || in_coff + op.cin > ib.C || out_coff + op.cout > ob.C) {
            failed = true;
            fail("internal: shape mismatch planning conv " + names[0]);
            return;
        }
        const int bm = conv_cfg_bm(op.cfg);
        op.tile_w = 0;
        if (op.k == 3 && wo >= 64 && wo % 16 == 0 && ho % (bm / 16) == 0) op.tile_w = 16;
        op.halo = halo_eligible(op.k, op.stride, op.cin, h->is_f16) && h->use_halo ? 1 : 0;
        if (h->split) op.halo = split_halo_eligible(op.k, op.stride, op.cin, op.cout) && h->use_halo ? 1 : 0;
        if (!h->split && h->use_halo && c32_eligible(op.k, op.stride, op.cin, op.cout, h->is_f16, out2_buf >= 0)) op.halo = 2;
        if (h->split && h->use_halo && h->use_c32s && c32_split_eligible(op.k, op.stride, op.cin, op.cout, out2_buf < 0 && in2_buf < 0 && !ob.f32)) op.halo = 2;
        op.macs_per_image = (double)ho * wo * cout * op.k * op.k * op.cin;
        if (pack_conv(h, op, wp, bp, couts)) {
            failed = true;
            return;
        }
        h->ops.push_back(op);
    }
    void c2f(const std::string &p, int in_buf, int in_coff, int c2, int n, bool shortcut, int out_buf, int out_coff, int out2_buf = -1,
             int out2_coff = 0, int in2_buf = -1, int in2_coff = 0, int in2_split = 0) {
        if (failed) return;
        const Buf ib = h->bufs[in_buf];
        const int c = c2 / 2;
        const int cat = new_buf(ib.h, ib.w, (2 + n) * c);
        const int tmp = new_buf(ib.h, ib.w, c);
        conv({p + ".cv1"}, in_buf, in_coff, cat, 0, -1, 0, -1, 0, 0, in2_buf, in2_coff, in2_split);
        for (int i = 0; i < n; ++i) {
            const std::string m = p + ".m." + std::to_string(i);
            conv({m + ".cv1"}, cat, (1 + i) * c, tmp, 0);
            conv({m + ".cv2"}, tmp, 0, cat, (2 + i) * c, -1, 0, shortcut ? cat : -1, (1 + i) * c);
        }
        conv({p + ".cv2"}, cat, 0, out_buf, out_coff, out2_buf, out2_coff);
    }
};
}

static int env_int(const char *name, int unset) {
    const char *e = std::getenv(name);
    return e && e[0] ? std::atoi(e) : unset;
}

namespace {
struct PlanSwitches {
    int latency_plan;
    bool no_side_stream;
    bool materialize_upsample;
    bool no_igemm_tail;
    bool no_sk_mixed;
    bool small_narrow;
    int halo_deep;
    bool sk_finish;
    bool no_fused_front;
    bool no_fused_c2f;
};

PlanSwitches read_switches(wtk_yolo *h) {
    h->use_halo = env_int("WTK_NO_HALO", 0) != 1;
    h->halo_slabs = env_int("WTK_HALO_SLABS", 3) == 2 ? 2 : 3;
    h->halo_persist = env_int("WTK_HALO_PERSIST", 1) != 0;
    h->halo_small_blocks = env_int("WTK_HALO_SMALL_BLOCKS", 1) != 0;
    h->use_tail = env_int("WTK_NO_FUSED_TAIL", 0) != 1;
    h->use_tail_cls_split = env_int("WTK_NO_SPLIT_CLS_TAIL", 0) != 1;
    h->use_wide = env_int("WTK_NO_WIDE_1X1", 0) != 1;
    h->use_ws64 = env_int("WTK_NO_WS64", 0) != 1;
    h->use_s2win = env_int("WTK_NO_S2WIN", 0) != 1;
    h->use_c32s = env_int("WTK_NO_C32S", 0) != 1;
    h->sk_group = env_int("WTK_SK_GROUP", 1) != 0;
    h->sk_autotune = env_int("WTK_SK_AUTOTUNE", 1) != 0;
    const int tile = env_int("WTK_SK_TILE", -1), form = env_int("WTK_SK_FORM", -1);
    h->sk_force_tile = tile >= 0 && tile <= 3 ? tile : -1;
    h->sk_force_form = form == 0 || form == 1 ? form : -1;
    h->front_debug = env_int("WTK_FRONT_DEBUG", 0) == 1;
    PlanSwitches s;
    s.latency_plan = env_int("WTK_LATENCY_PLAN", -1);
    s.no_side_stream = env_int("WTK_NO_SIDE_STREAM", 0) == 1;
    s.materialize_upsample = env_int("WTK_MATERIALIZE_UPSAMPLE", 0) == 1;
    s.no_igemm_tail = env_int("WTK_NO_IGEMM_TAIL", 0) == 1;
    s.no_sk_mixed = env_int("WTK_NO_SK_MIXED", 0) == 1;
    s.small_narrow = env_int("WTK_SMALL_NARROW", 1) != 0;
    s.halo_deep = env_int("WTK_HALO_DEEP", 1);
    s.sk_finish = env_int("WTK_SK_FINISH", 0) == 1;
    s.no_fused_front = env_int("WTK_NO_FUSED_FRONT", 0) == 1;
    s.no_fused_c2f = env_int("WTK_NO_FUSED_C2F", 0) == 1;
    return s;
}
}

namespace {
struct sigaction g_old_segv;
void segv_backtrace(int sig, siginfo_t *info, void *ctx) {
    void *frames[64];
    const int n = backtrace(frames, 64);
    static const char msg[] = "\nwtracker_amd: SIGSEGV, native frames:\n";
    if (write(2, msg, sizeof(msg) - 1) < 0) {}
    backtrace_symbols_fd(frames, n, 2);
    if ((g_old_segv.sa_flags & SA_SIGINFO) && g_old_segv.sa_sigaction)
        g_old_segv.sa_sigaction(sig, info, ctx);
    else if (!(g_old_segv.sa_flags & SA_SIGINFO) && g_old_segv.sa_handler != SIG_DFL && g_old_segv.sa_handler != SIG_IGN)
        g_old_segv.sa_handler(sig);
    signal(sig, SIG_DFL);
    raise(sig);
}
__attribute__((constructor)) void install_segv_backtrace() {
    if (env_int("WTK_SEGV_BACKTRACE", 0) != 1) return;
    void *warm[4];
    (void)backtrace(warm, 4);
    struct sigaction sa;
    std::memset(&sa, 0, sizeof(sa));
    sa.sa_sigaction = segv_backtrace;
    sa.sa_flags = SA_SIGINFO | SA_NODEFER;
    sigemptyset(&sa.sa_mask);
    (void)sigaction(SIGSEGV, &sa, &g_old_segv);
}
}

namespace {
std::mutex g_status_mu;
int *g_status_page = nullptr, *g_status_page_dev = nullptr;
std::vector<int> g_status_free;
constexpr int kStatusSlots = 4096;
int acquire_status_word(int **host, int **dev) {
    std::lock_guard<std::mutex> lk(g_status_mu);
    if (!g_status_page) {
        void *hp = nullptr, *dp = nullptr;
        if (hipHostMalloc(&hp, kStatusSlots * sizeof(int), hipHostMallocMapped | hipHostMallocPortable) != hipSuccess) return 1;
        if (hipHostGetDevicePointer(&dp, hp, 0) != hipSuccess) {
            (void)hipHostFree(hp);
            return 1;
        }
        g_status_page = reinterpret_cast<int *>(hp), g_status_page_dev = reinterpret_cast<int *>(dp);
        for (int i = kStatusSlots - 1; i >= 0; --i) g_status_free.push_back(i);
    }
    if (g_status_free.empty()) return 1;
    const int slot = g_status_free.back();
    g_status_free.pop_back();
    g_status_page[slot] = 0;
    *host = g_status_page + slot, *dev = g_status_page_dev + slot;
    return 0;
}
void release_status_word(int *host, int *) {
    std::lock_guard<std::mutex> lk(g_status_mu);
    if (g_status_page && host >= g_status_page && host < g_status_page + kStatusSlots) g_status_free.push_back((int)(host - g_status_page));
}
}


static void sk_schedule(wtk_yolo *h) {
    h->lat_sched.clear();
    const size_t n = h->ops.size();
    if (!h->latency || n <= 3) return;
    auto reads = [&](const Op &o, std::vector<int> &r) {
        r.clear();
        for (int b : {o.in_buf, o.res_buf, o.in2_buf})
            if (b >= 0) r.push_back(b);
    };
    auto writes = [&](const Op &o, std::vector<int> &w) {
        w.clear();
        if (o.kind == OP_POOL) w.push_back(o.in_buf);
        for (int b : {o.out_buf, o.out2_buf})
            if (b >= 0) w.push_back(b);
        if (o.tail_op >= 0 && h->ops[o.tail_op].out_buf >= 0) w.push_back(h->ops[o.tail_op].out_buf);
    };
    auto meets = [](const std::vector<int> &a, const std::vector<int> &b) {
        for (int x : a)
            for (int y : b)
                if (x == y) return true;
        return false;
    };
    std::vector<int> level(n, 0), ri, wi, rj, wj;
    int deepest = 0;
    for (size_t i = 0; i < n; ++i) {
        if (h->ops[i].folded) continue;
        reads(h->ops[i], ri), writes(h->ops[i], wi);
        for (size_t j = 0; j < i; ++j) {
            if (h->ops[j].folded) continue;
            reads(h->ops[j], rj), writes(h->ops[j], wj);
            if (meets(wj, ri) || meets(wj, wi) || meets(rj, wi)) level[i] = std::max(level[i], level[j] + 1);
        }
        deepest = std::max(deepest, level[i]);
    }
    for (int lv = 0; lv <= deepest; ++lv) {
        std::vector<int> group;
        for (size_t i = 3; i < n; ++i) {
            const Op &o = h->ops[i];
            if (o.folded || level[i] != lv) continue;
            if (o.kind == OP_CONV && o.sk) {
                group.push_back((int)i);
                if ((int)group.size() == kSkGroupMax) h->lat_sched.push_back(group), group.clear();
            } else {
                h->lat_sched.push_back({(int)i});
            }
        }
        if (!group.empty()) h->lat_sched.push_back(group);
    }
}

extern "C" void wtk_yolo_destroy(wtk_yolo *h) {
    if (!h) return;
    DeviceGuard guard(h->device);
    (void)hipDeviceSynchronize();
    for (int i = 0; i < h->ev_created; ++i) (void)hipEventDestroy(h->ev[i]);
    for (hipEvent_t e : h->tune_ev) (void)hipEventDestroy(e);
    for (int i = 0; i < 2; ++i)
        if (h->feat_ev[i]) (void)hipEventDestroy(h->feat_ev[i]);
    for (int i = 0; i < wtk_yolo::kSideStreams; ++i) {
        if (h->side_done[i]) (void)hipEventDestroy(h->side_done[i]);
    }
    if (h->host_stream) unpool_stream(h->device, h->host_stream);
    dev_release(h);
    (void)hipFree(h->frames_dev);
    (void)hipFree(h->lb_dev);
    (void)hipFree(h->nms_score);
    (void)hipFree(h->nms_box);
    (void)hipFree(h->nms_cls);
    if (h->status_host) release_status_word(h->status_host, h->status_dev);
    delete h;
}

extern "C" int wtk_yolo_create(wtk_yolo **out, const wtk_yolo_desc *d) { return wtk_yolo_create_planned(out, d, WTK_PLAN_AUTO); }
extern "C" int wtk_yolo_plan(wtk_yolo *h) { return h ? (h->latency ? WTK_PLAN_LATENCY : WTK_PLAN_THROUGHPUT) : -1; }

extern "C" int wtk_yolo_create_planned(wtk_yolo **out, const wtk_yolo_desc *d, int32_t plan) {
    if (!out || !d || !d->convs) return fail("wtk_yolo_create: null argument");
    if (plan != WTK_PLAN_AUTO && plan != WTK_PLAN_THROUGHPUT && plan != WTK_PLAN_LATENCY) return fail("wtk_yolo_create_planned: plan must be WTK_PLAN_AUTO, _THROUGHPUT or _LATENCY");
    if (plan == WTK_PLAN_LATENCY && d->dtype == WTK_F16) return fail("wtk_yolo_create_planned: the latency plan is built for WTK_F32 and WTK_F16X3 handles");
// ... 41 lines not shown
    }
    h->latency = d->max_batch <= 4 && !h->is_f16;
    if (sw.latency_plan >= 0) h->latency = sw.latency_plan == 1 && !h->is_f16;
    if (plan != WTK_PLAN_AUTO) h->latency = plan == WTK_PLAN_LATENCY;
    if (h->latency) h->use_tail = 0;

    Planner P{h, specs, d->convs};
    const int *c = dims.c;
    const int H = h->S_h, W = h->S_w;
    auto hw = [&](int s, int &hh, int &ww) { hh = H / s, ww = W / s; };
    int h2, w2, h4, w4, h8, w8, h16, w16, h32, w32;
    hw(2, h2, w2), hw(4, h4, w4), hw(8, h8, w8), hw(16, h16, w16), hw(32, h32, w32);

    const int t0 = P.new_buf(h2, w2, c[0]);
    const int t1 = P.new_buf(h4, w4, c[1]);
    const int t2 = P.new_buf(h4, w4, c[1]);
    const int t3 = P.new_buf(h8, w8, c[2]);
    const int cat14 = P.new_buf(h8, w8, c[3] + c[2]);
    const int t5 = P.new_buf(h16, w16, c[3]);
    const int cat11 = P.new_buf(h16, w16, c[4] + c[3]);
    const int t7 = P.new_buf(h32, w32, c[4]);
    const int t8 = P.new_buf(h32, w32, c[4]);
    const int sppcat = P.new_buf(h32, w32, 2 * c[4]);
    const int cat20 = P.new_buf(h32, w32, c[3] + c[4]);
    const int cat17 = P.new_buf(h16, w16, c[2] + c[3]);
    const int t15 = P.new_buf(h8, w8, c[2]);
    const int t18 = P.new_buf(h16, w16, c[3]);
    const int t21 = P.new_buf(h32, w32, c[4]);

    {
        Op op;
        op.kind = OP_STEM;
        op.out_buf = t0;
        op.cout = c[0];
        op.macs_per_image = (double)h2 * w2 * c[0] * 27;
        const int i0 = find_spec(specs, "model.0");
        op.spec = i0;
        const float *w0 = d->convs[i0].weight;
        const bool stem_split = h->split;
        const int taps = (h->is_f16 || stem_split) ? 16 : 9;
        std::vector<float> wp((size_t)c[0] * taps * 4, 0.f);
        for (int co = 0; co < c[0]; ++co)
            for (int tap = 0; tap < 9; ++tap)
                for (int ch = 0; ch < 3; ++ch)
                    wp[((size_t)co * taps + tap) * 4 + ch] = (float)((double)w0[((size_t)co * 9 + tap) * 3 + ch] * (double)kActScale);
        if (h->is_f16 || stem_split)
            for (float x : wp) {
                if (!(std::fabs(x) <= 65504.0f)) {
                    wtk_yolo_destroy(h);
                    return fail("wtk_yolo_create: a folded weight of conv blob " + std::to_string(i0) + " (model.0) is outside the fp16 range: this model needs dtype WTK_F32");
                }
            }
        std::vector<float> stem_bias(c[0]);
        for (int co = 0; co < c[0]; ++co) stem_bias[co] = (float)((double)d->convs[i0].bias[co] * (double)kActScale);
        void *wdev;
        float *bdev;
        std::vector<uint16_t> wh;
        const void *src = wp.data();
        size_t bytes = wp.size() * 4;
        if (h->is_f16) {
            wh.resize(wp.size());
            for (size_t i = 0; i < wp.size(); ++i) wh[i] = f32_to_f16_bits(wp[i]);
            src = wh.data();
            bytes = wh.size() * 2;
        } else if (stem_split) {
            wh.resize(2 * wp.size());
            for (size_t i = 0; i < wp.size(); ++i) {
                const uint16_t hb = f32_to_f16_bits(wp[i]);
                wh[i] = hb;
                wh[wp.size() + i] = f32_to_f16_bits((wp[i] - f16_bits_to_f32(hb)) * kSplitScale);
            }
            src = wh.data();
            bytes = wh.size() * 2;
        }
        if (dev_alloc(h, &wdev, bytes) || dev_alloc(h, (void **)&bdev, sizeof(float) * c[0])) {
            wtk_yolo_destroy(h);
            return 1;
        }
        if (hipMemcpy(wdev, src, bytes, hipMemcpyHostToDevice) != hipSuccess ||
            hipMemcpy(bdev, stem_bias.data(), sizeof(float) * c[0], hipMemcpyHostToDevice) != hipSuccess) {
            wtk_yolo_destroy(h);
            return fail("wtk_yolo_create: stem weight upload failed");
        }
        op.w = wdev;
        op.bias = bdev;
        h->ops.push_back(op);
    }
    P.conv({"model.1"}, t0, 0, t1, 0);
    P.c2f("model.2", t1, 0, c[1], dims.n[0], true, t2, 0);
    P.conv({"model.3"}, t2, 0, t3, 0);
    P.c2f("model.4", t3, 0, c[2], dims.n[1], true, cat14, c[3]);
    P.conv({"model.5"}, cat14, c[3], t5, 0);
    P.c2f("model.6", t5, 0, c[3], dims.n[2], true, cat11, c[4]);
    P.conv({"model.7"}, cat11, c[4], t7, 0);
    P.c2f("model.8", t7, 0, c[4], dims.n[3], true, t8, 0);
    P.conv({"model.9.cv1"}, t8, 0, sppcat, 0);
    if (!P.failed) {
        Op op;
        op.kind = OP_POOL;
        op.in_buf = sppcat;
        op.cin = c[4] / 2;
        h->ops.push_back(op);
    }
    const bool lazy_up = c[2] % 128 == 0 && c[3] % 128 == 0 && !sw.materialize_upsample;
    if (lazy_up) {
        P.conv({"model.9.cv2"}, sppcat, 0, cat20, c[3]);
        P.c2f("model.12", cat11, 0, c[3], dims.n[3], false, cat17, c[2], -1, 0, cat20, c[3], c[4]);
        P.c2f("model.15", cat14, 0, c[2], dims.n[3], false, t15, 0, -1, 0, cat17, c[2], c[3]);
    } else {
        P.conv({"model.9.cv2"}, sppcat, 0, cat20, c[3], cat11, 0);
        P.c2f("model.12", cat11, 0, c[3], dims.n[3], false, cat17, c[2], cat14, 0);
        P.c2f("model.15", cat14, 0, c[2], dims.n[3], false, t15, 0);
    }
    if (!P.failed) h->ops.back().signal_feat = 0;
    P.conv({"model.16"}, t15, 0, cat17, 0);
    P.c2f("model.18", cat17, 0, c[3], dims.n[3], false, t18, 0);
    if (!P.failed) h->ops.back().signal_feat = 1;
    P.conv({"model.19"}, t18, 0, cat20, 0);
    P.c2f("model.21", cat20, 0, c[4], dims.n[3], false, t21, 0);
    const int feat[3] = {t15, t18, t21};
    const int fh[3] = {h8, h16, h32}, fw[3] = {w8, w16, w32};
    h->cls_ld = (d->nc + 7) / 8 * 8;
    for (int i = 0; i < 3 && !P.failed; ++i) {
        const std::string b = "model.22.cv2." + std::to_string(i), cl = "model.22.cv3." + std::to_string(i);
        const int d1 = P.new_buf(fh[i], fw[i], dims.hb + dims.hc);
        const int d2b = P.new_buf(fh[i], fw[i], dims.hb);
        const int d2c = P.new_buf(fh[i], fw[i], dims.hc);
        h->box_buf[i] = P.new_buf(fh[i], fw[i], 64);
        h->cls_buf[i] = P.new_buf(fh[i], fw[i], h->cls_ld);
        h->bufs[h->box_buf[i]].f32 = h->bufs[h->cls_buf[i]].f32 = 1;
        h->lh[i] = fh[i];
        h->lw[i] = fw[i];
        const size_t first_op = h->ops.size();
        P.conv({b + ".0", cl + ".0"}, feat[i], 0, d1, 0);
        P.conv({b + ".1"}, d1, 0, d2b, 0);
        P.conv({cl + ".1"}, d1, dims.hb, d2c, 0);
        P.conv({b + ".2"}, d2b, 0, h->box_buf[i], 0);
        P.conv({cl + ".2"}, d2c, 0, h->cls_buf[i], 0, -1, 0, -1, 0, h->cls_ld);
        if (!P.failed && h->use_tail) {
            Op &b1 = h->ops[first_op + 1], &b2 = h->ops[first_op + 3];
            if ((h->is_f16 || h->split) && b1.halo == 1 && b1.cout == 64 && b1.cout_pad == 64 && b2.k == 1 && b2.cin == 64 && b2.cout == 64 && !b2.act &&
                b2.in_buf == b1.out_buf && b2.res_buf < 0 && b2.out2_buf < 0 && b1.res_buf < 0 && b1.out2_buf < 0 && h->halo_slabs == 3) {
                b1.tail_op = (int)first_op + 3;
                b2.folded = 1;
            }
            Op &c1 = h->ops[first_op + 2], &c2 = h->ops[first_op + 4];
            if ((h->is_f16 || (h->split && h->use_tail_cls_split)) && c1.halo == 1 && c1.cout == 128 && c1.cout_pad == 128 && c2.k == 1 && c2.cin == 128 && c2.cout <= 32 && c2.cout_pad == 32 &&
                !c2.act && c2.in_buf == c1.out_buf && c2.res_buf < 0 && c2.out2_buf < 0 && c1.res_buf < 0 && c1.out2_buf < 0 && h->halo_slabs == 3 &&
                c2.cout == h->cls_ld) {
                c1.tail_op = (int)first_op + 4;
                c2.folded = 1;
            }
        }
        if (!P.failed && i < 2) {
            for (size_t k = first_op; k < h->ops.size(); ++k) h->ops[k].side = i == 1 ? 2 : 1;
            h->ops[first_op].wait_feat = i;
        }
    }
    if (!P.failed && h->is_f16 && !sw.no_igemm_tail) {
        for (size_t i = 0; i + 1 < h->ops.size(); ++i) {
            Op &c3 = h->ops[i], &c1 = h->ops[i + 1];
            if (c3.kind != OP_CONV || c1.kind != OP_CONV || c3.halo || c3.k != 3 || c3.stride != 2 || c3.cfg != CFG_128x128 || c3.cout != 128 || c3.cout_pad != 128 ||
                !c3.act || c3.res_buf >= 0 || c3.out2_buf >= 0 || c3.in2_buf >= 0 || c3.tail_op >= 0 || c3.folded)
                continue;
            if (c1.k != 1 || c1.stride != 1 || c1.cin != 128 || c1.cout != 128 || c1.cout_pad != 128 || c1.in_buf != c3.out_buf || c1.in_coff != c3.out_coff ||
                c1.res_buf >= 0 || c1.out2_buf >= 0 || c1.in2_buf >= 0 || c1.folded || c1.tail_op >= 0 || h->bufs[c3.out_buf].C != 128)
                continue;
            bool other_reader = false;
            for (size_t j = 0; j < h->ops.size(); ++j) {
                const Op &o = h->ops[j];
                if (j != i + 1 && (o.in_buf == c3.out_buf || o.res_buf == c3.out_buf || o.in2_buf == c3.out_buf)) other_reader = true;
            }
            if (other_reader) continue;
            c3.tail_op = (int)i + 1;
            c1.folded = 1;
        }
    }
    if (P.failed) {
        wtk_yolo_destroy(h);
        return 1;
    }
    h->anchors = h8 * w8 + h16 * w16 + h32 * w32;
    for (const Op &op : h->ops) h->macs_per_frame += op.macs_per_image;
    const bool sk_mixed = !h->latency && !h->is_f16 && h->max_batch <= 16 && !sw.no_sk_mixed;
    const long long sk_mixed_max_px = h->split ? 4096 : 10000;
    h->small_narrow = !h->is_f16 && h->max_batch <= 16 && sw.small_narrow;
    h->halo_deep = h->split && (sw.halo_deep == 2 || (sw.halo_deep == 1 && h->max_batch <= 16));
    if (h->latency || sk_mixed) {
        for (size_t i = 3; i < h->ops.size(); ++i) {
            Op &op = h->ops[i];
            if (op.kind != OP_CONV || op.folded || op.tail_op >= 0 || op.out2_buf >= 0 || op.cin % 32 || (op.k != 1 && op.k != 3) || op.cout_pad % 32 || op.cout % 8) continue;
            if (op.in2_buf >= 0 && (op.k != 1 || op.in2_split % 32)) continue;
            {
                const Buf &ibx = h->bufs[op.in_buf];
                if (2LL * ibx.h * ibx.w * ibx.C * 4 > 0x7fffffffLL) continue;
            }
            if (sk_mixed && (long long)h->max_batch * h->bufs[op.out_buf].h * h->bufs[op.out_buf].w > sk_mixed_max_px) continue;
            op.sk = 1;
            const Buf &ob = h->bufs[op.out_buf];
            const long long plan_px = (long long)(h->latency ? 1 : h->max_batch) * ob.h * ob.w;
            op.sk_atoms = conv_sk_plan_atoms(plan_px, op.cout_pad, op.k * op.k * op.cin / 32, h->num_cus, h->split);
            const int S = op.sk_atoms;
            if (S > 1 && dev_alloc(h, (void **)&op.sk_partial, (size_t)S * h->max_batch * ob.h * ob.w * op.cout_pad * sizeof(float))) {
                wtk_yolo_destroy(h);
                return 1;
            }
            if (S > 1 && !sw.sk_finish) {
                const size_t nt = conv_sk_ticket_count((long long)h->max_batch * ob.h * ob.w, op.cout_pad) * sizeof(unsigned);
                if (dev_alloc(h, (void **)&op.sk_tickets, nt)) {
                    wtk_yolo_destroy(h);
                    return 1;
                }
                if (hipMemset(op.sk_tickets, 0, nt) != hipSuccess) {
                    wtk_yolo_destroy(h);
                    return fail("wtk_yolo_create: hipMemset failed");
                }
            }
        }
    }
    sk_schedule(h);
    h->use_front = !sw.no_fused_front && h->ops.size() > 3 && h->ops[0].kind == OP_STEM && h->ops[1].kind == OP_CONV && h->ops[2].kind == OP_CONV &&
                   h->ops[1].k == 3 && h->ops[1].stride == 2 && h->ops[2].k == 1 && h->ops[1].act && h->ops[2].act &&
                   h->ops[2].out2_buf < 0 && h->ops[2].res_buf < 0 &&
                   (front_fused_eligible(h->is_f16, h->ops[0].cout, h->ops[1].cout, h->ops[2].cout) ||
                    (h->split && h->ops[1].cin == 32 && front_fused_split_eligible(h->ops[0].cout, h->ops[1].cout, h->ops[2].cout)));
    if (!sw.no_fused_c2f && h->ops.size() > 6 && dims.n[0] == 1) {
        const Op &m1 = h->ops[3], &m2 = h->ops[4], &cv2 = h->ops[5], &cv1 = h->ops[2];
        h->use_c2f = m1.kind == OP_CONV && m2.kind == OP_CONV && cv2.kind == OP_CONV && m1.k == 3 && m2.k == 3 && cv2.k == 1 &&
                     m1.stride == 1 && m2.stride == 1 && m1.act && m2.act && cv2.act && m1.in_buf == cv1.out_buf &&
                     m2.res_buf == cv1.out_buf && m2.res_coff == m1.in_coff && cv2.in_buf == cv1.out_buf && cv2.in_coff == cv1.out_coff &&
                     m1.in_coff == cv1.out_coff + 32 && m2.out_coff == cv1.out_coff + 64 && cv2.cin == 96 && m1.Kpad == m2.Kpad &&
                     cv2.out2_buf < 0 && cv2.res_buf < 0 && m1.cout == 32 && m2.cout == 32 &&
                     c2f_fused_eligible(h->is_f16, m1.cin, dims.n[0], m2.res_buf >= 0, cv2.cout);
    }

    for (Buf &b : h->bufs) {
        if (dev_alloc(h, &b.ptr, b.elems_per_image * (size_t)h->max_batch * (b.f32 ? 4 : h->esize))) {
            wtk_yolo_destroy(h);
            return 1;
        }
    }
    if (dev_alloc(h, (void **)&h->o_xywh, sizeof(float) * 4 * h->max_batch) || dev_alloc(h, (void **)&h->o_conf, sizeof(float) * h->max_batch) ||
        dev_alloc(h, (void **)&h->o_anchor, sizeof(int) * h->max_batch) || dev_alloc(h, (void **)&h->o_margin, sizeof(float) * h->max_batch)) {
        wtk_yolo_destroy(h);
        return 1;
    }
    if (acquire_status_word(&h->status_host, &h->status_dev)) {
        h->status_host = nullptr;
        wtk_yolo_destroy(h);
        return fail("wtk_yolo_create: no pinned status word (hipHostMalloc failed, or more than 4096 live handles)");
    }
    if (dev_alloc(h, &h->zero_page, 256)) {
        wtk_yolo_destroy(h);
        return 1;
    }
    if (hipMemset(h->zero_page, 0, 256) != hipSuccess) {
        wtk_yolo_destroy(h);
        return fail("wtk_yolo_create: hipMemset failed");
    }
    *out = h;
    return 0;
}

extern "C" int wtk_yolo_status(wtk_yolo *h, int32_t *flags, int32_t clear) {
    if (!h || !flags) return fail("wtk_yolo_status: null argument");
    *flags = h->status_static | (h->status_host ? __atomic_load_n(h->status_host, __ATOMIC_RELAXED) : 0);
    if (clear && h->status_host) __atomic_store_n(h->status_host, 0, __ATOMIC_RELAXED);
    return 0;
}

extern "C" int wtk_yolo_workload(wtk_yolo *h, double *macs_per_frame, int32_t *anchors) {
    if (!h) return fail("wtk_yolo_workload: null handle");
    if (macs_per_frame) *macs_per_frame = h->macs_per_frame;
    if (anchors) *anchors = h->anchors;
    return 0;
}

extern "C" int wtk_yolo_set_profiling(wtk_yolo *h, int32_t enabled) {
    if (!h) return fail("wtk_yolo_set_profiling: null handle");
    if (enabled && !h->ev_created) {
        for (int i = 0; i < wtk_yolo::kProfEvents; ++i) {
            HIP_TRY(hipEventCreate(&h->ev[i]));
            h->ev_created = i + 1;
        }
    }
    h->profiling = enabled ? 1 : 0;
    for (int i = 0; i < wtk_yolo::kProfKernels; ++i) h->prof_ms[i] = 0, h->prof_flops[i] = 0, h->prof_launches[i] = 0;
    return 0;
}

extern "C" int wtk_yolo_get_kernel_profile(wtk_yolo *h, int32_t kernel_id, double *total_ms, int64_t *launches, double *flops) {
    if (!h || kernel_id < 0 || kernel_id >= wtk_yolo::kProfKernels) return fail("wtk_yolo_get_kernel_profile: bad argument");
    if (total_ms) *total_ms = h->prof_ms[kernel_id];
    if (launches) *launches = h->prof_launches[kernel_id];
    if (flops) *flops = h->prof_flops[kernel_id];
    return 0;
}

extern "C" int wtk_yolo_get_profile(wtk_yolo *h, int32_t kernel_class, double *total_ms, int64_t *launches) {
    if (!h || kernel_class < 0 || kernel_class > 3) return fail("wtk_yolo_get_profile: bad argument");
    double ms = h->prof_ms[kernel_class];
    long long n = h->prof_launches[kernel_class];
    if (kernel_class == 1)
        for (int k = 4; k < wtk_yolo::kProfKernels; ++k) ms += h->prof_ms[k], n += h->prof_launches[k];
    if (total_ms) *total_ms = ms;
    if (launches) *launches = n;
    return 0;
}
```

wtracker_amd/csrc/wtk_run.hip:

```cpp
#include "wtk_internal.h"

#include <algorithm>
#include <cmath>
#include <cstdio>
#include <cstdlib>

using namespace wtk;

#ifdef WTK_WS64_STAMPS
static unsigned long long *g_dbg_stamps = nullptr;
constexpr size_t kDbgStampBytes = 1 << 20;
extern "C" int wtk_debug_stamps(unsigned long long *host, size_t n_words) {
    if (!g_dbg_stamps || n_words * 8 > kDbgStampBytes) return 1;
    if (hipDeviceSynchronize() != hipSuccess) return 1;
    return hipMemcpy(host, g_dbg_stamps, n_words * 8, hipMemcpyDeviceToHost) == hipSuccess ? 0 : 1;
}
#endif

static void letterbox_geom(int H, int W, int Sh, int Sw, int &new_h, int &new_w, int &top, int &left, float &gain, float &pad_x, float &pad_y) {
    const double r = std::min((double)Sh / H, (double)Sw / W);
    new_w = (int)std::nearbyint(W * r);
    new_h = (int)std::nearbyint(H * r);
    const double dw = (Sw - new_w) / 2.0, dh = (Sh - new_h) / 2.0;
    top = (int)std::nearbyint(dh - 0.1);
    left = (int)std::nearbyint(dw - 0.1);
    gain = (float)std::min((double)Sh / H, (double)Sw / W);
    pad_x = (float)std::nearbyint((Sw - W * (double)gain) / 2.0 - 0.1);
    pad_y = (float)std::nearbyint((Sh - H * (double)gain) / 2.0 - 0.1);
}

struct NmsOut {
    float iou;
    int max_det;
    int *out_cls, *out_count;
};
static int run_head(wtk_yolo *h, int B, int H, int W, float conf, float *out_xywh, float *out_conf, int *out_anchor, hipStream_t st,
                    const NmsOut *nms = nullptr) {
    HeadArgs a;
    std::memset(&a, 0, sizeof(a));
    for (int i = 0; i < 3; ++i) {
        a.box[i] = h->bufs[h->box_buf[i]].ptr;
        a.cls[i] = h->bufs[h->cls_buf[i]].ptr;
        a.lh[i] = h->lh[i];
        a.lw[i] = h->lw[i];
    }
    a.cls_ld = h->cls_ld;
    a.nc = h->dims.nc;
    a.N = B;
    a.conf = conf;
    int nh, nw, top, left;
    letterbox_geom(H, W, h->S_h, h->S_w, nh, nw, top, left, a.gain, a.pad_x, a.pad_y);
    a.img_w = (float)W;
    a.img_h = (float)H;
    a.out_xywh = out_xywh;
    a.out_conf = out_conf;
    a.out_anchor = out_anchor;
    a.out_margin = h->o_margin;
    a.status = h->status_dev;
    a.conf_logit = conf > 0.f && conf < 1.f ? std::log(conf / (1.f - conf)) : (conf <= 0.f ? -INFINITY : INFINITY);
    if (nms) {
        NmsArgs q;
        std::memset(&q, 0, sizeof(q));
        q.h = a;
        q.iou = nms->iou, q.max_det = nms->max_det;
        q.scratch_score = h->nms_score, q.scratch_cls = h->nms_cls, q.scratch_box = h->nms_box;
        q.out_xywh = out_xywh, q.out_conf = out_conf, q.out_anchor = out_anchor, q.out_cls = nms->out_cls, q.out_count = nms->out_count;
        HIP_TRY(launch_head_nms(q, 0, st));
        return 0;
    }
    HIP_TRY(launch_head(a, 0, st));
    return 0;
}

static int ensure_nms_scratch(wtk_yolo *h, hipStream_t st) {
    if (h->nms_score) return 0;
    HIP_TRY(hipStreamSynchronize(st));
    const size_t n = (size_t)h->max_batch * h->anchors;
    HIP_TRY(hipMalloc(&h->nms_score, n * sizeof(float)));
    HIP_TRY(hipMalloc(&h->nms_cls, n * sizeof(int)));
    HIP_TRY(hipMalloc(&h->nms_box, n * 4 * sizeof(float)));
    return 0;
}

static std::mutex g_side_mu;

static int ensure_side_streams(wtk_yolo *h) {
    for (int i = 1; i <= 2; ++i) {
        if (!h->side_stream[i]) {
            static std::mutex mu;
            static std::vector<std::pair<int, hipStream_t>> g_shared[2];
            std::lock_guard<std::mutex> lk(mu);
            for (auto &e : g_shared[i - 1])
                if (e.first == h->device) h->side_stream[i] = e.second;
            if (!h->side_stream[i]) {
                HIP_TRY(hipStreamCreateWithFlags(&h->side_stream[i], hipStreamNonBlocking));
                g_shared[i - 1].emplace_back(h->device, h->side_stream[i]);
            }
        }
        if (!h->side_done[i]) HIP_TRY(hipEventCreateWithFlags(&h->side_done[i], hipEventDisableTiming));
    }
    for (int i = 0; i < 2; ++i)
        if (!h->feat_ev[i]) HIP_TRY(hipEventCreateWithFlags(&h->feat_ev[i], hipEventDisableTiming));
    return 0;
}


static ConvArgs conv_args(const wtk_yolo *h, const Op &op, int B) {
    const Buf &ib = h->bufs[op.in_buf], &ob = h->bufs[op.out_buf];
    ConvArgs a;
    std::memset(&a, 0, sizeof(a));
    a.in = ib.ptr, a.in_ld = ib.C, a.in_coff = op.in_coff;
    a.N = B, a.H = ib.h, a.W = ib.w, a.Cin = op.cin;
    a.Ho = ob.h, a.Wo = ob.w, a.Cout = op.cout, a.CoutPad = op.cout_pad;
    a.KH = a.KW = op.k, a.stride = op.stride, a.pad = op.k / 2;
    a.w = op.w, a.bias = op.bias, a.zeros = h->zero_page, a.n_dyn = h->n_dyn;
    a.out = ob.ptr, a.out_ld = ob.C, a.out_coff = op.out_coff, a.out_f32 = ob.f32;
    if (op.out2_buf >= 0) a.out2 = h->bufs[op.out2_buf].ptr, a.out2_ld = h->bufs[op.out2_buf].C, a.out2_coff = op.out2_coff;
    if (op.in2_buf >= 0) a.in2 = h->bufs[op.in2_buf].ptr, a.in2_ld = h->bufs[op.in2_buf].C, a.in2_coff = op.in2_coff, a.in2_split = op.in2_split;
    if (op.res_buf >= 0) a.res = h->bufs[op.res_buf].ptr, a.res_ld = h->bufs[op.res_buf].C, a.res_coff = op.res_coff;
    a.act = op.act, a.K = op.K, a.Kpad = op.Kpad;
    a.M = (long long)B * ob.h * ob.w;
    a.tile_w = op.tile_w;
    if (op.tile_w) {
        const int th = conv_cfg_bm(op.cfg) / op.tile_w;
        a.tiles_x = (ob.w + op.tile_w - 1) / op.tile_w, a.tiles_y = (ob.h + th - 1) / th;
    }
    if (h->split) {
        a.in_ld *= 2, a.in_coff *= 2, a.Cin *= 2, a.K *= 2, a.Kpad *= 2;
        a.in2_ld *= 2, a.in2_coff *= 2, a.in2_split *= 2;
        a.res_ld *= 2, a.res_coff *= 2, a.out2_ld *= 2, a.out2_coff *= 2;
        if (!a.out_f32) a.out_ld *= 2, a.out_coff *= 2;
    }
    return a;
}

static int sk_args(const wtk_yolo *h, const Op &op, int B, ConvArgs &a) {
    a = conv_args(h, op, B);
    a.tile_w = 0;
    if (!conv_sk_eligible(a, h->split)) return fail("internal: conv " + std::to_string(&op - h->ops.data()) + " of the latency plan does not fit conv_sk_kernel");
    return 0;
}

static HaloArgs halo_args(const wtk_yolo *h, const Op &op, const ConvArgs &a, int H, int W) {
    HaloArgs g;
    std::memset(&g, 0, sizeof(g));
    g.in = a.in, g.in_ld = a.in_ld, g.in_coff = a.in_coff;
    g.N = a.N, g.H = H, g.W = W, g.Cin = a.Cin;
    g.Cout = op.cout, g.CoutPad = op.cout_pad;
    g.w = op.w, g.bias = op.bias;
    g.out = a.out, g.out_ld = a.out_ld, g.out_coff = a.out_coff;
    g.out2 = a.out2, g.out2_ld = a.out2_ld, g.out2_coff = a.out2_coff;
    g.res = a.res, g.res_ld = a.res_ld, g.res_coff = a.res_coff;
    g.act = op.act, g.Kpad = a.Kpad;
    g.n_dyn = h->n_dyn, g.zeros = h->zero_page;
    if (op.tail_op >= 0) {
        const Op &t = h->ops[op.tail_op];
        g.tail_w = t.w, g.tail_bias = t.bias, g.tail_kpad = t.Kpad;
        g.tail_out = h->bufs[t.out_buf].ptr, g.tail_ld = h->bufs[t.out_buf].C, g.tail_coff = t.out_coff;
        g.tail_cout = t.cout, g.tail_f32 = h->bufs[t.out_buf].f32;
        if (h->split) {
            g.tail_kpad *= 2;
            if (!g.tail_f32) g.tail_ld *= 2, g.tail_coff *= 2;
        }
    }
    return g;
}

static HaloArgs s2win_args(const wtk_yolo *h, const Op &op, const ConvArgs &a) {
    HaloArgs g = halo_args(h, op, a, a.Ho, a.Wo);
    g.S = a.Wo, g.pitch = a.Wo + 1, g.strips = 1, g.bm = 256;
    g.blocks_per_strip = (int)(((long long)a.N * (a.Ho + 1) * g.pitch + 255) / 256);
    if (2LL * g.blocks_per_strip * (op.cout_pad / 128) <= h->num_cus) {
        g.bm = 128;
        g.blocks_per_strip = (int)(((long long)a.N * (a.Ho + 1) * g.pitch + 127) / 128);
    }
    return g;
}

static void resolve_window(const wtk_yolo *h, const Op &op, ConvLaunch &r) {
    const int B = r.a.N, H = r.a.H, W = r.a.W;
    HaloArgs &g = r.g;
    g = halo_args(h, op, r.a, H, W);
    g.slabs = h->split ? 3 : h->halo_slabs, g.persist_cus = h->halo_persist ? h->num_cus : 0;
    if (op.halo == 1 && h->use_ws64 && h->halo_slabs == 3 &&
        ws64_eligible(op.k, op.stride, op.cin, op.cout, op.cout_pad, h->is_f16, op.out2_buf >= 0, op.tail_op >= 0)) {
        halo_geometry_stacked(B, H, W, ws64_rows_max(), &g.S, &g.pitch, &g.strips, &g.blocks_per_strip);
        if ((long long)g.strips * g.blocks_per_strip >= 4LL * h->num_cus) {
            r.kind = L_WS64;
            return;
        }
    }
    const int rows_max = (op.halo == 2 && h->split) ? c32_split_rows_max() : (op.halo == 2 || h->split) ? kHaloRowsMax : halo_rows_max(op.cout, h->halo_slabs);
    if (op.halo == 2) {
        halo_geometry(H, W, rows_max, &g.S, &g.pitch, &g.strips, &g.blocks_per_strip);
        r.kind = h->split ? L_C32_SPLIT : L_C32;
        return;
    }
    r.kind = h->split ? L_HALO_SPLIT : L_HALO;
    halo_geometry_stacked(B, H, W, rows_max, &g.S, &g.pitch, &g.strips, &g.blocks_per_strip);
    if (h->halo_slabs == 3 || h->split) {
        const long long tiles = (long long)g.strips * g.blocks_per_strip * (op.cout_pad / (h->split ? split_halo_cout_tile(op.cout) : halo_cout_tile(op.cout)));
        if (h->halo_small_blocks && 2 * tiles <= h->num_cus) {
            g.bm = 128;
            halo_geometry_stacked(B, H, W, rows_max, &g.S, &g.pitch, &g.strips, &g.blocks_per_strip, 128);
            if (h->small_narrow && h->split && op.tail_op < 0 && op.cout_pad % 128 == 0 && 2LL * g.strips * g.blocks_per_strip * (op.cout_pad / 128) <= h->num_cus)
                g.narrow = 1;
        }
    }
    if (h->small_narrow && !h->split && op.tail_op < 0 && op.cout_pad % 64 == 0 && halo_cout_tile(op.cout) != 64 &&
        4LL * g.strips * g.blocks_per_strip * (op.cout_pad / halo_cout_tile(op.cout)) <= 3LL * h->num_cus)
        g.narrow = 1;
    if (h->halo_deep) g.deep = 1;
}

static int resolve_conv(const wtk_yolo *h, const Op &op, int B, ConvLaunch &r) {
    const Buf &ib = h->bufs[op.in_buf], &ob = h->bufs[op.out_buf];
    r.cls = op.sk ? PROF_IGEMM : (op.halo == 2 ? PROF_C32 : (op.halo ? PROF_HALO : PROF_IGEMM));
    r.cfg = op.cfg, r.kind = L_IGEMM;
    if (op.sk) {
        r.kind = L_SK;
        return sk_args(h, op, B, r.a);
    }
    ConvArgs &a = r.a;
    a = conv_args(h, op, B);
    const bool plain = op.res_buf < 0 && op.out2_buf < 0 && op.in2_buf < 0, halves = ib.h == 2 * ob.h && ib.w == 2 * ob.w;
    if (h->split && !op.halo && h->use_s2win && halves && split_s2win_eligible(op.k, op.stride, op.cin, op.cout, op.cout_pad, ob.w, plain && !ob.f32)) {
        r.kind = L_S2WIN_SPLIT;
        r.g = s2win_args(h, op, a);
    } else if (h->split && !op.halo) {
        r.kind = L_IGEMM_SPLIT;
        if (h->small_narrow && r.cfg == CFG_128x128 && !a.in2 && !a.tile_w && 3 * ((a.M + 127) / 128) * (a.CoutPad / 128) <= 2LL * h->num_cus) r.cfg = CFG_128x64;
    } else if (op.halo) {
        resolve_window(h, op, r);
    } else if (h->use_s2win && op.tail_op < 0 && s2win_eligible(op.k, op.stride, op.cin, op.cout, op.cout_pad, h->is_f16, ob.w, plain) && halves) {
        r.kind = L_S2WIN;
        r.g = s2win_args(h, op, a);
    } else if (op.tail_op >= 0) {
        const Op &t = h->ops[op.tail_op];
        a.tail_w = t.w, a.tail_bias = t.bias, a.tail_kpad = t.Kpad, a.tail_act = t.act;
        a.tail_out = h->bufs[t.out_buf].ptr, a.tail_ld = h->bufs[t.out_buf].C, a.tail_coff = t.out_coff;
    } else if (h->use_wide && conv1x1_wide_eligible(a, h->is_f16) && a.CoutPad >= 256 && ((a.M + 255) / 256) * (a.CoutPad / 128) >= 384) {
        r.kind = L_WIDE_1X1;
    }
    return 0;
}

constexpr long long kOpKeyBase = 100000;
static long long choice_key(long long launch, int B) { return (launch << 24) | (long long)B; }

static int issue_conv(wtk_yolo *h, const Op &op, const ConvLaunch &r, hipStream_t st) {
    switch (r.kind) {
    case L_IGEMM: HIP_TRY(launch_conv(r.a, r.cfg, h->is_f16, st)); break;
    case L_IGEMM_SPLIT: HIP_TRY(launch_conv_split(r.a, r.cfg, st)); break;
    case L_WIDE_1X1: HIP_TRY(launch_conv1x1_wide(r.a, st)); break;
    case L_HALO: HIP_TRY(launch_conv3x3_halo(r.g, h->is_f16, st)); break;
    case L_HALO_SPLIT: HIP_TRY(launch_conv3x3_halo_split(r.g, st)); break;
    case L_C32: HIP_TRY(launch_conv3x3_c32(r.g, st)); break;
    case L_C32_SPLIT: HIP_TRY(launch_conv3x3_c32_split(r.g, st)); break;
    case L_S2WIN: HIP_TRY(launch_conv3x3_s2(r.g, st)); break;
    case L_S2WIN_SPLIT: HIP_TRY(launch_conv3x3_s2_split(r.g, st)); break;
    case L_WS64:
#ifdef WTK_WS64_STAMPS
        if (std::getenv("WTK_WS64_STAMPS")) {
            if (!g_dbg_stamps) HIP_TRY(hipMalloc(&g_dbg_stamps, kDbgStampBytes));
            HaloArgs g = r.g;
            g.dbg_stamps = g_dbg_stamps;
            HIP_TRY(launch_conv3x3_ws64(g, h->num_cus, st));
            break;
        }
#endif
        HIP_TRY(launch_conv3x3_ws64(r.g, h->num_cus, st));
        break;
    case L_SK: {
        const SkMember one{r.a, op.sk_atoms, op.sk_partial, op.sk_tickets};
        HIP_TRY(launch_conv_sk_group(&one, 1, h->split, h->num_cus, h->sk_force_tile, h->sk_force_form, st, &h->sk_choices[choice_key(kOpKeyBase + (&op - h->ops.data()), r.a.N)]));
        break;
    }
    }
    return 0;
}

struct ViewSrc {
    const int32_t *pos_xy, *frame_index;
    int view_w, view_h, n_frames;
};

struct Pass {
    wtk_yolo *h;
    const uint8_t *net_in;
    int B, C;
    hipStream_t main_st;
    bool two_lanes = false;
    unsigned side_used = 0;
    int cur_class = -1, nev = 0;
    int ev_class[wtk_yolo::kProfEvents];
    long long launches[wtk_yolo::kProfKernels] = {};
    double flops[wtk_yolo::kProfKernels] = {};
    double op_flops(const Op &o) const { return 2.0 * B * o.macs_per_image; }
    void count(ProfClass cls, double fl = 0.0) { ++launches[cls], flops[cls] += fl; }
};

static int mark(Pass &p, ProfClass cls) {
    if (!p.h->profiling || cls == p.cur_class || p.nev >= wtk_yolo::kProfEvents - 1) return 0;
    HIP_TRY(hipEventRecord(p.h->ev[p.nev], p.main_st));
    p.ev_class[p.nev++] = p.cur_class = cls;
    return 0;
}

static int enqueue_input(Pass &p, const uint8_t *frames_dev, int32_t &H, int32_t &W, const ViewSrc *vs) {
    wtk_yolo *h = p.h;
    float g, px, py;
    if (vs) {
        ViewLetterboxArgs va;
        std::memset(&va, 0, sizeof(va));
        va.frames = frames_dev, va.frame_index = vs->frame_index, va.pos_xy = vs->pos_xy, va.dst = h->lb_dev;
        va.N = p.B, va.H = H, va.W = W, va.C = p.C, va.F = vs->n_frames;
        va.view_w = vs->view_w, va.view_h = vs->view_h, va.Sh = h->S_h, va.Sw = h->S_w;
        va.rows = vs->view_w, va.cols = vs->view_h;
        letterbox_geom(va.rows, va.cols, h->S_h, h->S_w, va.new_h, va.new_w, va.top, va.left, g, px, py);
        HIP_TRY(launch_view_letterbox(va, p.main_st));
        p.net_in = h->lb_dev;
        H = va.rows, W = va.cols;
    } else if (H != h->S_h || W != h->S_w) {
        LetterboxArgs la;
        std::memset(&la, 0, sizeof(la));
        la.src = frames_dev, la.dst = h->lb_dev;
        la.N = p.B, la.H = H, la.W = W, la.C = p.C, la.Sh = h->S_h, la.Sw = h->S_w;
        letterbox_geom(H, W, h->S_h, h->S_w, la.new_h, la.new_w, la.top, la.left, g, px, py);
        HIP_TRY(launch_letterbox(la, p.main_st));
        p.net_in = h->lb_dev;
    }
    return 0;
}

static int enqueue_front(Pass &p) {
    wtk_yolo *h = p.h;
    if (mark(p, PROF_FUSED)) return 1;
    const Op &o0 = h->ops[0], &o1 = h->ops[1], &o2 = h->ops[2];
    FrontArgs f;
    std::memset(&f, 0, sizeof(f));
    f.frames = p.net_in, f.N = p.B, f.H = h->S_h, f.W = h->S_w, f.C = p.C;
    f.w0 = o0.w, f.b0 = o0.bias;
    f.w1 = o1.w, f.b1 = o1.bias, f.Kpad1 = o1.Kpad;
    f.w2 = o2.w, f.b2 = o2.bias, f.Kpad2 = o2.Kpad;
    f.out = h->bufs[o2.out_buf].ptr, f.out_ld = h->bufs[o2.out_buf].C, f.out_coff = o2.out_coff;
    if (h->front_debug) f.dbg_t0 = h->bufs[o0.out_buf].ptr, f.dbg_t1 = h->bufs[o1.out_buf].ptr;
    if (h->split) {
        f.Kpad1 *= 2, f.Kpad2 *= 2, f.out_ld *= 2, f.out_coff *= 2;
        f.n_dyn = h->n_dyn, f.stem_split = 1;
        HIP_TRY(launch_front_fused_split(f, h->num_cus, p.main_st));
    } else
        HIP_TRY(launch_front_fused(f, h->num_cus, p.main_st));
    p.count(PROF_FUSED, p.op_flops(o0) + p.op_flops(o1) + p.op_flops(o2));
    return 0;
}

static int enqueue_c2f(Pass &p, const Op &op) {
    wtk_yolo *h = p.h;
    if (mark(p, PROF_FUSED)) return 1;
    const Op &m1 = h->ops[3], &m2 = h->ops[4];
    const Buf &cb = h->bufs[op.in_buf];
    C2fArgs c;
    std::memset(&c, 0, sizeof(c));
    c.cat = cb.ptr, c.cat_ld = cb.C, c.a_coff = op.in_coff, c.b_coff = m1.in_coff;
    c.N = p.B, c.H = cb.h, c.W = cb.w, c.zeros = h->zero_page;
    c.w_m1 = m1.w, c.b_m1 = m1.bias, c.w_m2 = m2.w, c.b_m2 = m2.bias, c.Kpad_m = m1.Kpad;
    c.w_cv2 = op.w, c.b_cv2 = op.bias, c.Kpad_cv2 = op.Kpad;
    c.out = h->bufs[op.out_buf].ptr, c.out_ld = h->bufs[op.out_buf].C, c.out_coff = op.out_coff;
    HIP_TRY(launch_c2f_fused(c, h->num_cus, p.main_st));
    p.count(PROF_FUSED, p.op_flops(m1) + p.op_flops(m2) + p.op_flops(op));
    return 0;
}

static int enqueue_op(Pass &p, size_t oi) {
    wtk_yolo *h = p.h;
    const Op &op = h->ops[oi];
    if (h->use_c2f && (oi == 3 || oi == 4)) return 0;
    if (op.folded) return 0;
    if (h->use_c2f && oi == 5) return enqueue_c2f(p, op);
    hipStream_t st = p.main_st;
    if (p.two_lanes && op.side) {
        const int sidx = std::min(op.side, h->side_streams);
        st = h->side_stream[sidx];
        if (op.wait_feat >= 0) HIP_TRY(hipStreamWaitEvent(st, h->feat_ev[op.wait_feat], 0));
        p.side_used |= 1u << sidx;
    }
    if (op.kind == OP_STEM) {
        if (mark(p, PROF_STEM)) return 1;
        StemArgs a;
        std::memset(&a, 0, sizeof(a));
        a.frames = p.net_in, a.N = p.B, a.H = h->S_h, a.W = h->S_w, a.C = p.C;
        a.w = op.w, a.bias = op.bias, a.out = h->bufs[op.out_buf].ptr;
        a.Cout = op.cout, a.Ho = h->S_h / 2, a.Wo = h->S_w / 2;
        a.out_split = a.in_split = h->split;
        a.n_dyn = h->n_dyn;
        HIP_TRY(launch_stem(a, h->is_f16, st));
        p.count(PROF_STEM, p.op_flops(op));
        return 0;
    }
    if (op.kind == OP_POOL) {
        if (mark(p, PROF_POOL)) return 1;
        const Buf &b = h->bufs[op.in_buf];
        PoolArgs a;
        std::memset(&a, 0, sizeof(a));
        a.buf = b.ptr, a.N = p.B, a.H = b.h, a.W = b.w, a.c = op.cin, a.split = h->split;
        HIP_TRY(launch_sppf_pool(a, h->is_f16, st));
        p.count(PROF_POOL);
        return 0;
    }
    ConvLaunch r;
    if (resolve_conv(h, op, p.B, r) || mark(p, r.cls) || issue_conv(h, op, r, st)) return 1;
    p.count(r.cls, p.op_flops(op) + (op.tail_op >= 0 ? p.op_flops(h->ops[op.tail_op]) : 0.0));
    if (p.two_lanes && op.signal_feat >= 0) HIP_TRY(hipEventRecord(h->feat_ev[op.signal_feat], p.main_st));
    return 0;
}

static int enqueue_levels(Pass &p, size_t first_op) {
    wtk_yolo *h = p.h;
    for (size_t oi = first_op; oi < 3 && oi < h->ops.size(); ++oi)
        if (enqueue_op(p, oi)) return 1;
    for (size_t li = 0; li < h->lat_sched.size(); ++li) {
        const std::vector<int> &L = h->lat_sched[li];
        if (!(h->ops[L[0]].kind == OP_CONV && h->ops[L[0]].sk)) {
            if (enqueue_op(p, (size_t)L[0])) return 1;
            continue;
        }
        if (mark(p, PROF_IGEMM)) return 1;
        SkMember m[kSkGroupMax];
        const int n = (int)L.size();
        for (int k = 0; k < n; ++k) {
            const Op &op = h->ops[L[k]];
            m[k] = SkMember{ConvArgs(), op.sk_atoms, op.sk_partial, op.sk_tickets};
            if (sk_args(h, op, p.B, m[k].a)) return 1;
            p.flops[PROF_IGEMM] += p.op_flops(op);
        }
        const long long key = choice_key((long long)li, p.B);
        SkChoice *choice = &h->sk_choices[key], cand;
        hipEvent_t *ev = h->tune_pass >= 0 ? &h->tune_ev[2 * li] : nullptr;
        if (ev) {
            std::vector<SkChoice> &cands = h->sk_cands[key];
            if (cands.empty()) {
                cands.resize(kSkMaxCandidates);
                cands.resize((size_t)std::max(conv_sk_enumerate(m, n, h->split, h->num_cus, h->sk_force_tile, h->sk_force_form, cands.data(), kSkMaxCandidates), 0));
                if (cands.empty()) return fail("internal: no launch candidate for level " + std::to_string(li));
                h->tune_ms[key].assign(cands.size(), 1e30f);
            }
            cand = cands[(size_t)h->tune_pass % cands.size()];
            choice = &cand;
            HIP_TRY(hipEventRecord(ev[0], p.main_st));
        }
        HIP_TRY(launch_conv_sk_group(m, n, h->split, h->num_cus, h->sk_force_tile, h->sk_force_form, p.main_st, choice));
        if (ev) {
            HIP_TRY(hipEventRecord(ev[1], p.main_st));
            h->tune_key[li] = key;
        }
        p.count(PROF_IGEMM);
    }
    return 0;
}

static int yolo_enqueue_pass(wtk_yolo *h, const uint8_t *frames_dev, int32_t B, int32_t H, int32_t W, int32_t C, float conf, float *out_xywh,
                             float *out_conf, int32_t *out_anchor, hipStream_t st, const ViewSrc *vs, const NmsOut *nms) {
    Pass p{h, frames_dev, B, C, st};
    if (enqueue_input(p, frames_dev, H, W, vs)) return 1;
    const bool grouped = h->latency && h->sk_group && !h->lat_sched.empty();
    if (!grouped && h->use_side && h->side_streams > 0 && !h->profiling && ensure_side_streams(h)) return 1;
    p.two_lanes = !grouped && h->use_side && h->side_streams > 0 && h->side_stream[1] && !h->profiling;
    std::unique_lock<std::mutex> side_lock;
    if (p.two_lanes) side_lock = std::unique_lock<std::mutex>(g_side_mu);
    const bool front = h->use_front && reinterpret_cast<uintptr_t>(p.net_in) % 4 == 0;
    if (front && enqueue_front(p)) return 1;
    const size_t first_op = front ? 3 : 0;
    if (grouped && enqueue_levels(p, first_op)) return 1;
    for (size_t oi = first_op; !grouped && oi < h->ops.size(); ++oi)
        if (enqueue_op(p, oi)) return 1;
    for (int i = 1; i < wtk_yolo::kSideStreams; ++i)
        if (p.side_used & (1u << i)) {
            HIP_TRY(hipEventRecord(h->side_done[i], h->side_stream[i]));
            HIP_TRY(hipStreamWaitEvent(st, h->side_done[i], 0));
        }
    if (mark(p, PROF_HEAD)) return 1;
    if (run_head(h, B, H, W, conf, out_xywh, out_conf, out_anchor, st, nms)) return 1;
    p.count(PROF_HEAD);
    if (!h->profiling) return 0;
    if (p.nev < wtk_yolo::kProfEvents) {
        HIP_TRY(hipEventRecord(h->ev[p.nev], st));
        p.ev_class[p.nev++] = -1;
    }
    HIP_TRY(hipEventSynchronize(h->ev[p.nev - 1]));
    for (int i = 0; i + 1 < p.nev; ++i) {
        float ms = 0.f;
        HIP_TRY(hipEventElapsedTime(&ms, h->ev[i], h->ev[i + 1]));
        h->prof_ms[p.ev_class[i]] += ms;
    }
    for (int i = 0; i < wtk_yolo::kProfKernels; ++i) h->prof_launches[i] += p.launches[i], h->prof_flops[i] += p.flops[i];
    return 0;
}

static int sk_autotune(wtk_yolo *h, const uint8_t *frames_dev, int32_t B, int32_t H, int32_t W, int32_t C, float conf, float *out_xywh, float *out_conf,
                       int32_t *out_anchor, hipStream_t st, const ViewSrc *vs, const NmsOut *nms) {
    const size_t n = h->lat_sched.size();
    while (h->tune_ev.size() < 2 * n) {
        hipEvent_t e;
        HIP_TRY(hipEventCreate(&e));
        h->tune_ev.push_back(e);
    }
    h->tune_key.assign(n, -1);
    constexpr int kReps = 3;
    size_t most = 1;
    int rc = 0;
    for (size_t pass = 0; pass < most * kReps && !rc; ++pass) {
        h->tune_pass = (int)pass;
        rc = yolo_enqueue_pass(h, frames_dev, B, H, W, C, conf, out_xywh, out_conf, out_anchor, st, vs, nms);
        h->tune_pass = -1;
        if (rc) break;
        if (hipStreamSynchronize(st) != hipSuccess) {
            rc = fail("sk_autotune: hipStreamSynchronize failed");
            break;
        }
        for (size_t li = 0; li < n; ++li) {
            const long long key = h->tune_key[li];
            if (key < 0) continue;
            const std::vector<SkChoice> &cands = h->sk_cands[key];
            float ms = 0.f;
            if (hipEventElapsedTime(&ms, h->tune_ev[2 * li], h->tune_ev[2 * li + 1]) != hipSuccess) continue;
            float &best = h->tune_ms[key][pass % cands.size()];
            best = std::min(best, ms);
            most = std::max(most, cands.size());
        }
    }
    if (rc) return rc;
    for (size_t li = 0; li < n; ++li) {
        const long long key = h->tune_key[li];
        if (key < 0) continue;
        const std::vector<SkChoice> &cands = h->sk_cands[key];
        const std::vector<float> &ms = h->tune_ms[key];
        size_t b = 0;
        for (size_t i = 1; i < cands.size(); ++i)
            if (ms[i] < ms[b] * 0.97f) b = i;
        h->sk_choices[key] = cands[b];
    }
    h->sk_tuned.push_back(B);
    return 0;
}

static int yolo_enqueue(wtk_yolo *h, const uint8_t *frames_dev, int32_t B, int32_t H, int32_t W, int32_t C, float conf, float *out_xywh, float *out_conf,
                        int32_t *out_anchor, hipStream_t st, const ViewSrc *vs = nullptr, const NmsOut *nms = nullptr) {
    if (h->latency && h->sk_group && h->sk_autotune && !h->lat_sched.empty() && !h->profiling && h->tune_pass < 0 &&
        std::find(h->sk_tuned.begin(), h->sk_tuned.end(), (int)B) == h->sk_tuned.end()) {
        hipStreamCaptureStatus cs = hipStreamCaptureStatusNone;
        if (hipStreamIsCapturing(st, &cs) == hipSuccess && cs == hipStreamCaptureStatusNone) {
            if (sk_autotune(h, frames_dev, B, H, W, C, conf, out_xywh, out_conf, out_anchor, st, vs, nms)) return 1;
        }
    }
    return yolo_enqueue_pass(h, frames_dev, B, H, W, C, conf, out_xywh, out_conf, out_anchor, st, vs, nms);
}

static int ensure_staging(wtk_yolo *h, hipStream_t st) {
    if (h->lb_cap) return 0;
    HIP_TRY(hipStreamSynchronize(st));
    HIP_TRY(hipMalloc(&h->lb_dev, (size_t)h->max_batch * h->S_h * h->S_w * 3));
    h->lb_cap = (size_t)h->max_batch * h->S_h * h->S_w * 3;
    return 0;
}

extern "C" int wtk_yolo_predict(wtk_yolo *h, const uint8_t *frames_dev, int32_t B, int32_t H, int32_t W, int32_t C, float conf, float iou,
                                int32_t max_det, float *out_xywh, float *out_conf, int32_t *out_anchor, void *stream) {
    (void)iou;
    if (!h || !frames_dev || !out_xywh) return fail("wtk_yolo_predict: null argument");
    if (B <= 0) return fail("wtk_yolo_predict: empty batch (the reference asserts len(frames) > 0, yolo_controller.py:65)");
    if (B > h->max_batch) return fail("wtk_yolo_predict: batch exceeds max_batch");
    if (C != 1 && C != 3) return fail("wtk_yolo_predict: frames must have 1 (gray) or 3 (BGR) channels");
    if (max_det != 1) return fail("wtk_yolo_predict: max_det must be 1 (yolo_controller.py:76 hard-wires it); wtk_yolo_predict_nms takes max_det > 1");
    if (H <= 0 || W <= 0) return fail("wtk_yolo_predict: bad frame size");
    DEVICE_GUARD(h);
    hipStream_t st = (hipStream_t)stream;
    if ((H != h->S_h || W != h->S_w) && ensure_staging(h, st)) return 1;
    return yolo_enqueue(h, frames_dev, B, H, W, C, conf, out_xywh, out_conf, out_anchor, st);
}

extern "C" int wtk_yolo_predict_nms(wtk_yolo *h, const uint8_t *frames_dev, int32_t B, int32_t H, int32_t W, int32_t C, float conf, float iou,
                                    int32_t max_det, float *out_xywh, float *out_conf, int32_t *out_cls, int32_t *out_anchor, int32_t *out_count,
                                    void *stream) {
    if (!h || !frames_dev || !out_xywh) return fail("wtk_yolo_predict_nms: null argument");
    if (B <= 0) return fail("wtk_yolo_predict_nms: empty batch (the reference asserts len(frames) > 0, yolo_controller.py:65)");
    if (B > h->max_batch) return fail("wtk_yolo_predict_nms: batch exceeds max_batch");
    if (C != 1 && C != 3) return fail("wtk_yolo_predict_nms: frames must have 1 (gray) or 3 (BGR) channels");
    if (max_det < 1 || max_det > 30000) return fail("wtk_yolo_predict_nms: max_det must be in [1, 30000]");
    if (!(iou >= 0.f && iou <= 1.f)) return fail("wtk_yolo_predict_nms: iou must be in [0, 1]");
    if (H <= 0 || W <= 0) return fail("wtk_yolo_predict_nms: bad frame size");
    DEVICE_GUARD(h);
    hipStream_t st = (hipStream_t)stream;
    if ((H != h->S_h || W != h->S_w) && ensure_staging(h, st)) return 1;
    if (ensure_nms_scratch(h, st)) return 1;
    const NmsOut nms{iou, max_det, out_cls, out_count};
    return yolo_enqueue(h, frames_dev, B, H, W, C, conf, out_xywh, out_conf, out_anchor, st, nullptr, &nms);
}

extern "C" int wtk_yolo_predict_views(wtk_yolo *h, const uint8_t *frames_dev, int32_t n_frames, int32_t H, int32_t W, int32_t C,
                                      const int32_t *frame_index_dev, const int32_t *pos_xy_dev, int32_t B, int32_t view_w, int32_t view_h, float conf,
                                      float iou, int32_t max_det, float *out_xywh, float *out_conf, int32_t *out_anchor, void *stream) {
    (void)iou;
    if (!h || !frames_dev || !pos_xy_dev || !out_xywh) return fail("wtk_yolo_predict_views: null argument");
    if (B <= 0) return fail("wtk_yolo_predict_views: empty batch (the reference asserts len(frames) > 0, yolo_controller.py:65)");
    if (B > h->max_batch) return fail("wtk_yolo_predict_views: batch exceeds max_batch");
    if (C != 1 && C != 3) return fail("wtk_yolo_predict_views: frames must have 1 (gray) or 3 (BGR) channels");
    if (max_det != 1) return fail("wtk_yolo_predict_views: max_det must be 1 (yolo_controller.py:76 hard-wires it)");
    if (H <= 0 || W <= 0 || view_w <= 0 || view_h <= 0 || n_frames <= 0) return fail("wtk_yolo_predict_views: bad frame / view size");
    if (!frame_index_dev && B > n_frames) return fail("wtk_yolo_predict_views: without frame_index the batch rows are frames 0..B-1");
    DEVICE_GUARD(h);
    hipStream_t st = (hipStream_t)stream;
    if (ensure_staging(h, st)) return 1;
    const ViewSrc vs{pos_xy_dev, frame_index_dev, view_w, view_h, n_frames};
    return yolo_enqueue(h, frames_dev, B, H, W, C, conf, out_xywh, out_conf, out_anchor, st, &vs);
}

extern "C" int wtk_yolo_predict_host(wtk_yolo *h, const uint8_t *frames_host, int32_t B, int32_t H, int32_t W, int32_t C, float conf,
                                     float iou, int32_t max_det, float *out_xywh, float *out_conf, int32_t *out_anchor) {
    if (!h || !frames_host || !out_xywh) return fail("wtk_yolo_predict_host: null argument");
    if (B <= 0) return fail("wtk_yolo_predict_host: empty batch (the reference asserts len(frames) > 0, yolo_controller.py:65)");
    if (B > h->max_batch) return fail("wtk_yolo_predict_host: batch exceeds max_batch");
    if (H <= 0 || W <= 0 || (C != 1 && C != 3)) return fail("wtk_yolo_predict_host: bad frame shape");
    DEVICE_GUARD(h);
    const size_t need = (size_t)B * H * W * C;
    if (need > h->frames_cap) {
        (void)hipFree(h->frames_dev);
        h->frames_dev = nullptr;
        h->frames_cap = 0;
        const size_t cap = std::max(need, (size_t)h->max_batch * H * W * C);
        HIP_TRY(hipMalloc(&h->frames_dev, cap));
        h->frames_cap = cap;
    }
    if (!h->host_stream && pooled_stream(h->device, &h->host_stream)) return 1;
    hipStream_t st = h->host_stream;
    HIP_TRY(hipMemcpyAsync(h->frames_dev, frames_host, need, hipMemcpyHostToDevice, st));
    if (wtk_yolo_predict(h, h->frames_dev, B, H, W, C, conf, iou, max_det, h->o_xywh, h->o_conf, h->o_anchor, st)) return 1;
    HIP_TRY(hipMemcpyAsync(out_xywh, h->o_xywh, sizeof(float) * 4 * B, hipMemcpyDeviceToHost, st));
    if (out_conf) HIP_TRY(hipMemcpyAsync(out_conf, h->o_conf, sizeof(float) * B, hipMemcpyDeviceToHost, st));
    if (out_anchor) HIP_TRY(hipMemcpyAsync(out_anchor, h->o_anchor, sizeof(int) * B, hipMemcpyDeviceToHost, st));
    HIP_TRY(hipStreamSynchronize(st));
    return 0;
}

extern "C" int wtk_yolo_set_side_streams(wtk_yolo *h, int32_t n) {
    if (!h || n < 0 || n > 2) return fail("wtk_yolo_set_side_streams: n must be 0, 1 or 2");
    h->side_streams = n;
    h->use_side = n > 0;
    return 0;
}

extern "C" int wtk_yolo_set_dynamic_batch(wtk_yolo *h, const int32_t *n_dev) {
    if (!h) return fail("wtk_yolo_set_dynamic_batch: null handle");
    h->n_dyn = n_dev;
    return 0;
}

extern "C" int wtk_yolo_margin_buffer(wtk_yolo *h, const float **margins_dev) {
    if (!h || !margins_dev) return fail("wtk_yolo_margin_buffer: null argument");
    *margins_dev = h->o_margin;
    return 0;
}

extern "C" int wtk_yolo_last_margins_host(wtk_yolo *h, int32_t B, float *margins_host) {
    if (!h || !margins_host || B <= 0 || B > h->max_batch) return fail("wtk_yolo_last_margins_host: bad argument");
    DEVICE_GUARD(h);
    HIP_TRY(hipDeviceSynchronize());
    HIP_TRY(hipMemcpy(margins_host, h->o_margin, sizeof(float) * B, hipMemcpyDeviceToHost));
    return 0;
}

static void to_f32(const void *src, float *dst, size_t n, int is_f16) {
    if (!is_f16) {
        std::memcpy(dst, src, n * 4);
        return;
    }
    const _Float16 *s = reinterpret_cast<const _Float16 *>(src);
    for (size_t i = 0; i < n; ++i) dst[i] = (float)s[i];
}

extern "C" int wtk_yolo_debug_head(wtk_yolo *h, int32_t level, int32_t B, float *box_host, float *cls_host) {
    if (!h || level < 0 || level > 2 || B <= 0 || B > h->max_batch) return fail("wtk_yolo_debug_head: bad argument");
    DEVICE_GUARD(h);
    HIP_TRY(hipDeviceSynchronize());
    const size_t A = (size_t)h->lh[level] * h->lw[level];
    if (box_host) {
        const size_t n = (size_t)B * A * 64;
        HIP_TRY(hipMemcpy(box_host, h->bufs[h->box_buf[level]].ptr, n * 4, hipMemcpyDeviceToHost));
    }
    if (cls_host) {
        const size_t n = (size_t)B * A * h->cls_ld;
        std::vector<float> full(n);
        HIP_TRY(hipMemcpy(full.data(), h->bufs[h->cls_buf[level]].ptr, n * 4, hipMemcpyDeviceToHost));
        for (size_t i = 0; i < (size_t)B * A; ++i)
            for (int k = 0; k < h->dims.nc; ++k) cls_host[i * h->dims.nc + k] = full[i * h->cls_ld + k];
    }
    return 0;
}

extern "C" int wtk_yolo_debug_tensor(wtk_yolo *h, int32_t conv_index, int32_t B, float *out_host, size_t out_cap, int32_t *shape_hwc) {
    if (!h || B <= 0 || B > h->max_batch) return fail("wtk_yolo_debug_tensor: bad argument");
    const Op *op = nullptr;
    for (const Op &o : h->ops)
        if (o.spec == conv_index && o.out_buf >= 0) op = &o;
    if (!op) return fail("wtk_yolo_debug_tensor: no op computes conv " + std::to_string(conv_index));
    const Buf &b = h->bufs[op->out_buf];
    if (shape_hwc) shape_hwc[0] = b.h, shape_hwc[1] = b.w, shape_hwc[2] = op->cout;
    if (!out_host) return 0;
    const size_t px = (size_t)B * b.h * b.w;
    if (out_cap < px * op->cout) return fail("wtk_yolo_debug_tensor: output buffer too small");
    DEVICE_GUARD(h);
    HIP_TRY(hipDeviceSynchronize());
    std::vector<char> tmp(px * b.C * (b.f32 ? 4 : h->esize));
    HIP_TRY(hipMemcpy(tmp.data(), b.ptr, tmp.size(), hipMemcpyDeviceToHost));
    std::vector<float> full(px * b.C);
    if (h->split && !b.f32) {
        const _Float16 *sp = reinterpret_cast<const _Float16 *>(tmp.data());
        for (size_t i = 0; i < px; ++i)
            for (int c = 0; c < b.C; ++c) {
                const size_t o = i * 2 * b.C + 64 * (c >> 5) + (c & 31);
                full[i * b.C + c] = (float)sp[o] + (float)sp[o + 32] * kSplitInv;
            }
    } else {
        to_f32(tmp.data(), full.data(), full.size(), b.f32 ? 0 : h->is_f16);
    }
    const float unscale = op->act ? 1.0f / kActScale : 1.0f;
    for (size_t i = 0; i < px; ++i)
        for (int k = 0; k < op->cout; ++k) out_host[i * op->cout + k] = full[i * b.C + op->out_coff + k] * unscale;
    return 0;
}

static int upload_head_logits(wtk_yolo *h, const float *box_host, const float *cls_host, int32_t B);

extern "C" int wtk_yolo_decode_nms_host(wtk_yolo *h, const float *box_host, const float *cls_host, int32_t B, int32_t H, int32_t W, float conf, float iou,
                                        int32_t max_det, float *out_xywh, float *out_conf, int32_t *out_cls, int32_t *out_anchor, int32_t *out_count) {
    if (!h || !box_host || !cls_host || !out_xywh || B <= 0 || B > h->max_batch || max_det < 1) return fail("wtk_yolo_decode_nms_host: bad argument");
    DEVICE_GUARD(h);
    HIP_TRY(hipDeviceSynchronize());
    if (upload_head_logits(h, box_host, cls_host, B)) return 1;
    if (ensure_nms_scratch(h, nullptr)) return 1;
    const size_t rows = (size_t)B * max_det;
    float *d_xywh = nullptr, *d_conf = nullptr;
    int *d_cls = nullptr, *d_anchor = nullptr, *d_count = nullptr;
    hipError_t e = hipSuccess;
    if ((e = hipMalloc(&d_xywh, rows * 16)) != hipSuccess || (e = hipMalloc(&d_conf, rows * 4)) != hipSuccess || (e = hipMalloc(&d_cls, rows * 4)) != hipSuccess ||
        (e = hipMalloc(&d_anchor, rows * 4)) != hipSuccess || (e = hipMalloc(&d_count, (size_t)B * 4)) != hipSuccess) {
        (void)hipFree(d_xywh), (void)hipFree(d_conf), (void)hipFree(d_cls), (void)hipFree(d_anchor), (void)hipFree(d_count);
        return fail_hip("wtk_yolo_decode_nms_host: hipMalloc", e);
    }
    const NmsOut nms{iou, max_det, d_cls, d_count};
    int rc = run_head(h, B, H, W, conf, d_xywh, d_conf, d_anchor, nullptr, &nms);
    if (!rc) {
        if ((e = hipMemcpy(out_xywh, d_xywh, rows * 16, hipMemcpyDeviceToHost)) != hipSuccess) rc = fail_hip("wtk_yolo_decode_nms_host: copy", e);
        if (!rc && out_conf && (e = hipMemcpy(out_conf, d_conf, rows * 4, hipMemcpyDeviceToHost)) != hipSuccess) rc = fail_hip("copy", e);
        if (!rc && out_cls && (e = hipMemcpy(out_cls, d_cls, rows * 4, hipMemcpyDeviceToHost)) != hipSuccess) rc = fail_hip("copy", e);
        if (!rc && out_anchor && (e = hipMemcpy(out_anchor, d_anchor, rows * 4, hipMemcpyDeviceToHost)) != hipSuccess) rc = fail_hip("copy", e);
        if (!rc && out_count && (e = hipMemcpy(out_count, d_count, (size_t)B * 4, hipMemcpyDeviceToHost)) != hipSuccess) rc = fail_hip("copy", e);
    }
    (void)hipFree(d_xywh), (void)hipFree(d_conf), (void)hipFree(d_cls), (void)hipFree(d_anchor), (void)hipFree(d_count);
    return rc;
}

extern "C" int wtk_yolo_decode_host(wtk_yolo *h, const float *box_host, const float *cls_host, int32_t B, int32_t H, int32_t W, float conf,
                                    float *out_xywh, float *out_conf, int32_t *out_anchor) {
    if (!h || !box_host || !cls_host || !out_xywh || B <= 0 || B > h->max_batch) return fail("wtk_yolo_decode_host: bad argument");
    DEVICE_GUARD(h);
    HIP_TRY(hipDeviceSynchronize());
    if (upload_head_logits(h, box_host, cls_host, B)) return 1;
    if (run_head(h, B, H, W, conf, h->o_xywh, h->o_conf, h->o_anchor, nullptr)) return 1;
    HIP_TRY(hipMemcpy(out_xywh, h->o_xywh, sizeof(float) * 4 * B, hipMemcpyDeviceToHost));
    if (out_conf) HIP_TRY(hipMemcpy(out_conf, h->o_conf, sizeof(float) * B, hipMemcpyDeviceToHost));
    if (out_anchor) HIP_TRY(hipMemcpy(out_anchor, h->o_anchor, sizeof(int) * B, hipMemcpyDeviceToHost));
    return 0;
}

static int upload_head_logits(wtk_yolo *h, const float *box_host, const float *cls_host, int32_t B) {
    const int A = h->anchors;
    size_t a0 = 0;
    for (int l = 0; l < 3; ++l) {
        const size_t Al = (size_t)h->lh[l] * h->lw[l];
        std::vector<float> bx((size_t)B * Al * 64), cl((size_t)B * Al * h->cls_ld, 0.f);
        for (int n = 0; n < B; ++n)
            for (size_t j = 0; j < Al; ++j) {
                std::memcpy(&bx[((size_t)n * Al + j) * 64], &box_host[((size_t)n * A + a0 + j) * 64], 64 * sizeof(float));
                for (int k = 0; k < h->dims.nc; ++k) cl[((size_t)n * Al + j) * h->cls_ld + k] = cls_host[((size_t)n * A + a0 + j) * h->dims.nc + k];
            }
        HIP_TRY(hipMemcpy(h->bufs[h->box_buf[l]].ptr, bx.data(), bx.size() * 4, hipMemcpyHostToDevice));
        HIP_TRY(hipMemcpy(h->bufs[h->cls_buf[l]].ptr, cl.data(), cl.size() * 4, hipMemcpyHostToDevice));
        a0 += Al;
    }
    return 0;
}
```

wtracker_amd/hip.py:

```python
from __future__ import annotations

import ctypes as C
import os
from typing import Optional, Sequence

import numpy as np

_LIB_PATH = os.environ.get("WTK_HIP_LIB") or os.path.join(os.path.dirname(os.path.abspath(__file__)), "libwtk_hip.so")
_lib: Optional[C.CDLL] = None

WTK_F32 = 0
WTK_F16 = 1
WTK_F16X3 = 2
DTYPES = {"fp32": WTK_F32, "f32": WTK_F32, "float32": WTK_F32, "fp16": WTK_F16, "f16": WTK_F16, "float16": WTK_F16, "f16x3": WTK_F16X3, "fp16x3": WTK_F16X3}


class WtkError(RuntimeError):
    pass


class _MlpLayer(C.Structure):
    _fields_ = [("in_dim", C.c_int32), ("out_dim", C.c_int32), ("relu", C.c_int32), ("reserved", C.c_int32),
                ("weight", C.POINTER(C.c_float)), ("bias", C.POINTER(C.c_float))]

# ... 377 lines not shown
            raise WtkError(f"plan must be one of {sorted(PLANS)}")
        table = yolo_conv_table(width, depth, max_channels, nc)
        arr = (_ConvBlob * len(table))()
        self._keep = []
        for i, t in enumerate(table):
            if t["name"] not in weights:
                raise WtkError(f"missing weights for conv {t['name']}")
            w, b = weights[t["name"]]
            w = np.ascontiguousarray(w, dtype=np.float32)
            b = np.ascontiguousarray(b, dtype=np.float32)
            if w.shape != (t["cout"], t["k"], t["k"], t["cin"]) or b.shape != (t["cout"],):
                raise WtkError(f"conv {t['name']}: expected weight {(t['cout'], t['k'], t['k'], t['cin'])}, got {w.shape}")
            self._keep += [w, b]
            arr[i] = _ConvBlob(t["cout"], t["cin"], t["k"], t["stride"], t["act"], 0, _fptr(w), _fptr(b))
        desc = _YoloDesc(device, DTYPES[dtype], int(imgsz[0]), int(imgsz[1]), int(max_batch), nc, width, depth, max_channels,
                         len(table), arr)
        self._h = C.c_void_p()
        _check(lib.wtk_yolo_create_planned(C.byref(self._h), C.byref(desc), PLANS[plan]), "wtk_yolo_create_planned")
        self.plan = "latency" if lib.wtk_yolo_plan(self._h) == PLANS["latency"] else "throughput"
        self._keep = []
        self.imgsz = (int(imgsz[0]), int(imgsz[1]))
        self.max_batch = int(max_batch)
        self.dtype = dtype
        self.nc = nc
        self.device = device
        macs, anchors = C.c_double(), C.c_int32()
        _check(lib.wtk_yolo_workload(self._h, C.byref(macs), C.byref(anchors)), "wtk_yolo_workload")
        self.macs_per_frame = macs.value
        self.anchors = anchors.value

    def close(self):
        for d in self.__dict__.pop("_dependents", []):
            d._release()
        if getattr(self, "_h", None) is not None and self._h:
            load().wtk_yolo_destroy(self._h)
            self._h = None

    def __del__(self):
        try:
            self.close()
        except Exception:
            pass

    def predict_host(self, frames: np.ndarray, conf: float = 0.1, iou: float = 0.7, max_det: int = 1):
        frames = np.ascontiguousarray(frames, dtype=np.uint8)
        if frames.ndim == 3:
            frames = frames[..., None]
        B, H, W, Cc = frames.shape
        xywh = np.empty((B, 4), dtype=np.float32)
        cf = np.empty((B,), dtype=np.float32)
        an = np.empty((B,), dtype=np.int32)
        _check(load().wtk_yolo_predict_host(self._h, _ptr(frames), B, H, W, Cc, conf, iou, max_det, _ptr(xywh), _ptr(cf),
                                            _ptr(an)), "wtk_yolo_predict_host")
        return xywh, cf, an

    def predict(self, frames_dev, B: int, H: int, W: int, Cc: int, out_xywh, out_conf=None, out_anchor=None,
                conf: float = 0.1, iou: float = 0.7, max_det: int = 1, stream: int = 0):
        _check(load().wtk_yolo_predict(self._h, _ptr(frames_dev), B, H, W, Cc, conf, iou, max_det, _ptr(out_xywh),
                                       _ptr(out_conf), _ptr(out_anchor), C.c_void_p(stream)), "wtk_yolo_predict")

    def status(self, clear: bool = False) -> int:
        f = C.c_int32()
        _check(load().wtk_yolo_status(self._h, C.byref(f), int(clear)), "wtk_yolo_status")
        return f.value

    def set_dynamic_batch(self, n_dev):
        _check(load().wtk_yolo_set_dynamic_batch(self._h, _ptr(n_dev)), "wtk_yolo_set_dynamic_batch")

    def set_side_streams(self, n: int):
        _check(load().wtk_yolo_set_side_streams(self._h, n), "wtk_yolo_set_side_streams")

    def last_margins(self, B: int) -> np.ndarray:
        out = np.empty((B,), dtype=np.float32)
        _check(load().wtk_yolo_last_margins_host(self._h, B, _ptr(out)), "wtk_yolo_last_margins_host")
        return out

    def margin_buffer(self) -> int:
        p = C.c_void_p()
        _check(load().wtk_yolo_margin_buffer(self._h, C.byref(p)), "wtk_yolo_margin_buffer")
        return int(p.value)

    def predict_nms(self, frames_dev, B: int, H: int, W: int, Cc: int, max_det: int, out_xywh, out_conf=None, out_cls=None, out_anchor=None,
                    out_count=None, conf: float = 0.1, iou: float = 0.7, stream: int = 0):
        _check(load().wtk_yolo_predict_nms(self._h, _ptr(frames_dev), B, H, W, Cc, conf, iou, max_det, _ptr(out_xywh), _ptr(out_conf),
                                           _ptr(out_cls), _ptr(out_anchor), _ptr(out_count), C.c_void_p(stream)), "wtk_yolo_predict_nms")

    def decode_nms_host(self, box: np.ndarray, cls: np.ndarray, H: int, W: int, max_det: int, conf: float = 0.1, iou: float = 0.7):
        box = np.ascontiguousarray(box, dtype=np.float32)
        cls = np.ascontiguousarray(cls, dtype=np.float32)
        B = box.shape[0]
        assert box.shape == (B, self.anchors, 64) and cls.shape == (B, self.anchors, self.nc)
        xywh = np.empty((B, max_det, 4), dtype=np.float32)
        cf = np.empty((B, max_det), dtype=np.float32)
        kc = np.empty((B, max_det), dtype=np.int32)
        an = np.empty((B, max_det), dtype=np.int32)
        cnt = np.empty((B,), dtype=np.int32)
        _check(load().wtk_yolo_decode_nms_host(self._h, _ptr(box), _ptr(cls), B, H, W, conf, iou, max_det, _ptr(xywh), _ptr(cf), _ptr(kc), _ptr(an),
                                               _ptr(cnt)), "wtk_yolo_decode_nms_host")
        return xywh, cf, kc, an, cnt

    def predict_views(self, frames_dev, n_frames: int, H: int, W: int, Cc: int, frame_index_dev, pos_xy_dev, B: int, view_w: int,
                      view_h: int, out_xywh, out_conf=None, out_anchor=None, conf: float = 0.1, iou: float = 0.7, max_det: int = 1,
                      stream: int = 0):
        _check(load().wtk_yolo_predict_views(self._h, _ptr(frames_dev), n_frames, H, W, Cc, _ptr(frame_index_dev), _ptr(pos_xy_dev), B,
                                             view_w, view_h, conf, iou, max_det, _ptr(out_xywh), _ptr(out_conf), _ptr(out_anchor),
                                             C.c_void_p(stream)), "wtk_yolo_predict_views")

    def debug_head(self, B: int):
        lib = load()
        boxes, clss = [], []
        S_h, S_w = self.imgsz
        for lvl, s in enumerate((8, 16, 32)):
            A = (S_h // s) * (S_w // s)
            bx = np.empty((B, A, 64), dtype=np.float32)
            cl = np.empty((B, A, self.nc), dtype=np.float32)
            _check(lib.wtk_yolo_debug_head(self._h, lvl, B, _ptr(bx), _ptr(cl)), "wtk_yolo_debug_head")
            boxes.append(bx)
            clss.append(cl)
        return np.concatenate(boxes, 1), np.concatenate(clss, 1)

    def debug_tensor(self, conv_index: int, B: int) -> np.ndarray:
        lib = load()
        shp = (C.c_int32 * 3)()
        _check(lib.wtk_yolo_debug_tensor(self._h, conv_index, B, None, 0, shp), "wtk_yolo_debug_tensor")
        out = np.empty((B, shp[0], shp[1], shp[2]), dtype=np.float32)
        _check(lib.wtk_yolo_debug_tensor(self._h, conv_index, B, _ptr(out), out.size, shp), "wtk_yolo_debug_tensor")
        return out

    def decode_host(self, box: np.ndarray, cls: np.ndarray, H: int, W: int, conf: float = 0.1):
        box = np.ascontiguousarray(box, dtype=np.float32)
        cls = np.ascontiguousarray(cls, dtype=np.float32)
        B = box.shape[0]
        assert box.shape == (B, self.anchors, 64) and cls.shape == (B, self.anchors, self.nc)
        xywh = np.empty((B, 4), dtype=np.float32)
        cf = np.empty((B,), dtype=np.float32)
        an = np.empty((B,), dtype=np.int32)
        _check(load().wtk_yolo_decode_host(self._h, _ptr(box), _ptr(cls), B, H, W, conf, _ptr(xywh), _ptr(cf), _ptr(an)),
               "wtk_yolo_decode_host")
        return xywh, cf, an

    def set_profiling(self, enabled: bool):
        _check(load().wtk_yolo_set_profiling(self._h, int(enabled)), "wtk_yolo_set_profiling")

    def get_profile(self) -> dict:
        names = ["stem", "conv", "pool", "head"]
        out = {}
        for i, nme in enumerate(names):
            ms, n = C.c_double(), C.c_int64()
            _check(load().wtk_yolo_get_profile(self._h, i, C.byref(ms), C.byref(n)), "wtk_yolo_get_profile")
            out[nme] = dict(total_ms=ms.value, launches=n.value)
        return out

    KERNELS = ["stem_mfma_kernel", "conv_igemm_kernel+conv1x1_wide_kernel", "sppf_pool_kernel", "head", "conv3x3_halo_kernel",
               "front_fused_kernel+c2f32_fused_kernel", "conv3x3_c32_kernel"]

    def get_kernel_profile(self) -> dict:
        out = {}
        for i, nme in enumerate(self.KERNELS):
            ms, n, fl = C.c_double(), C.c_int64(), C.c_double()
            _check(load().wtk_yolo_get_kernel_profile(self._h, i, C.byref(ms), C.byref(n), C.byref(fl)), "wtk_yolo_get_kernel_profile")
            out[nme] = dict(total_ms=ms.value, launches=n.value, flops=fl.value)
        return out
```

Before: 10920 frames/s.

## Compute box towers only around the selected anchor via a live-tile mask

The detect head's first 3x3 conv is split into a class-only launch. The head select kernel then runs on class logits alone and picks the best anchor per image. It marks 128-pixel tiles in a live mask covering that anchor's 3x3 neighbourhood, and the box-branch halo convs return early for tiles that are not marked. A new decode kernel then produces the box only for the chosen anchor. This is meant to skip most of the box-tower conv work, at the cost of extra launches, a memset, and lazy full recomputation in the debug paths. The sparse path is disabled during stream capture and when NMS is requested.

```diff
diff --git a/wtracker_amd/csrc/conv3x3_halo.hip b/wtracker_amd/csrc/conv3x3_halo.hip
--- a/wtracker_amd/csrc/conv3x3_halo.hip
+++ b/wtracker_amd/csrc/conv3x3_halo.hip
@@ -165,7 +165,7 @@
 #endif
     asm volatile("" ::"s"(a.in), "s"(a.w), "s"(a.bias), "s"(a.zeros), "s"(a.in_ld), "s"(a.in_coff), "s"(a.N), "s"(a.H), "s"(a.W), "s"(a.Cin), "s"(a.CoutPad),
                  "s"(a.Kpad), "s"(a.S), "s"(a.pitch), "s"(a.strips), "s"(a.d_strips.mul), "s"(a.d_strips.sh1), "s"(a.d_strips.sh2), "s"(a.d_pitch.mul),
-                 "s"(a.d_pitch.sh1), "s"(a.d_pitch.sh2), "s"(a.d_nct.mul), "s"(a.d_nct.sh1), "s"(a.d_nct.sh2), "s"(a.d_h1.mul), "s"(a.d_h1.sh1), "s"(a.d_h1.sh2), "s"(a.grid));
+                 "s"(a.d_pitch.sh1), "s"(a.d_pitch.sh2), "s"(a.d_nct.mul), "s"(a.d_nct.sh1), "s"(a.d_nct.sh2), "s"(a.d_h1.mul), "s"(a.d_h1.sh1), "s"(a.d_h1.sh2), "s"(a.grid), "s"(a.live_off));
     constexpr int CE = ElemH<T>::CE;
     constexpr int CCH = 8 * CE;
     constexpr int WAVES_C = BN == 64 ? 1 : 2, WAVES_P = 8 / WAVES_C;
@@ -208,6 +208,12 @@
     const int rb = (int)fdiv(t, a.d_strips);
     const int strip = (int)t - rb * a.strips;
     const int o0 = rb * BMT;
+    const char *zero_page = reinterpret_cast<const char *>(a.zeros);
+    if (a.live_off) {
+        const unsigned u = (unsigned)strip * (unsigned)a.live_ld + ((unsigned)o0 >> 7);
+        const unsigned wd = *reinterpret_cast<const unsigned *>(zero_page + a.live_off + (u & ~3u));
+        if (((wd >> ((u & 3u) * 8)) & (BMT == 256 ? 0xffffu : 0xffu)) == 0) return;
+    }
     const int xs = strip * a.S;
     const int pitch = a.pitch;
     const int halo_rows = BMT + 2 * pitch + 2;
@@ -216,7 +222,6 @@
 
     const T *in = reinterpret_cast<const T *>(a.in) + (long long)n_base * a.H * a.W * a.in_ld + a.in_coff;
     const T *wgt = reinterpret_cast<const T *>(a.w);
-    const char *zero_page = reinterpret_cast<const char *>(a.zeros);
 
     constexpr int kMaxPiecesPerWave = (HROWS / 8 + 7) / 8;
     unsigned hoff[kMaxPiecesPerWave];
@@ -1681,6 +1686,7 @@
     const long long blocks = (long long)a.strips * a.blocks_per_strip * (a.CoutPad / BN);
     if (blocks <= 0 || blocks > 0x7fffffffLL) return hipErrorInvalidValue;
     if (BMT + 2 * a.pitch + 2 > HROWS || (long long)a.blocks_per_strip * BMT < (long long)a.N * (a.H + 1) * a.pitch) return hipErrorInvalidValue;
+    if (a.live_off && ((a.live_off & 3u) || (a.live_ld & 1) || (long long)a.live_ld * 128 < (long long)a.blocks_per_strip * BMT)) return hipErrorInvalidValue;
     a.d_nct = make_fastdiv((unsigned)(a.CoutPad / BN));
     a.d_bps = make_fastdiv((unsigned)a.blocks_per_strip);
     a.d_strips = make_fastdiv((unsigned)a.strips);
diff --git a/wtracker_amd/csrc/head.hip b/wtracker_amd/csrc/head.hip
--- a/wtracker_amd/csrc/head.hip
+++ b/wtracker_amd/csrc/head.hip
@@ -15,13 +15,12 @@
 }
 
 template <typename T>
-__global__ __launch_bounds__(1024) void head_select_kernel(const HeadArgs a) {
-    const int n = blockIdx.x;
+__device__ __forceinline__ bool head_scan(const HeadArgs &a, int n, float &best, int &best_i, float &best_l, float &second) {
     const int A0 = a.lh[0] * a.lw[0], A1 = a.lh[1] * a.lw[1], A2 = a.lh[2] * a.lw[2];
     const int A = A0 + A1 + A2;
 
-    float best = -INFINITY, best_l = -INFINITY, second = -INFINITY;
-    int best_i = 0x7fffffff;
+    best = -INFINITY, best_l = -INFINITY, second = -INFINITY;
+    best_i = 0x7fffffff;
     bool bad = false;
     auto merge = [](float &b, int &bi, float &bl, float &s2nd, float b2, int bi2, float bl2, float s2) __attribute__((always_inline)) {
         if (b2 > b || (b2 == b && bi2 < bi)) {
@@ -71,18 +70,19 @@
         wsec[threadIdx.x >> 6] = second;
     }
     __syncthreads();
-    if (threadIdx.x >= 64) return;
+    if (threadIdx.x >= 64) return false;
     best = ws[0];
     best_i = wi[0];
     best_l = wl[0];
     second = wsec[0];
 #pragma unroll
     for (int w = 1; w < 16; ++w) merge(best, best_i, best_l, second, ws[w], wi[w], wl[w], wsec[w]);
-    if (a.out_margin && threadIdx.x == 0) a.out_margin[n] = fminf(best_l - second, fabsf(best_l - a.conf_logit));
-
-    const float score = best;
-    const bool keep = (best_i != 0x7fffffff) && (score > a.conf);
-
+    return true;
+}
+
+template <typename T>
+__device__ __forceinline__ void head_row(const HeadArgs &a, int n, bool keep, int best_i, float score) {
+    const int A0 = a.lh[0] * a.lw[0], A1 = a.lh[1] * a.lw[1], A2 = a.lh[2] * a.lw[2];
     float dist = 0.f;
     int lvl = 0, j = 0;
     if (keep) {
@@ -150,6 +150,56 @@
     o[3] = by2 - by1;
     if (a.out_conf) a.out_conf[n] = score;
     if (a.out_anchor) a.out_anchor[n] = best_i;
+}
+
+template <typename T>
+__global__ __launch_bounds__(1024) void head_select_kernel(const HeadArgs a) {
+    const int n = blockIdx.x;
+    float best, best_l, second;
+    int best_i;
+    if (!head_scan<T>(a, n, best, best_i, best_l, second)) return;
+    if (a.out_margin && threadIdx.x == 0) a.out_margin[n] = fminf(best_l - second, fabsf(best_l - a.conf_logit));
+
+    const float score = best;
+    const bool keep = (best_i != 0x7fffffff) && (score > a.conf);
+    head_row<T>(a, n, keep, best_i, score);
+}
+
+template <typename T>
+__global__ __launch_bounds__(1024) void head_select_kernel_sparse(const HeadSparseArgs q) {
+    const HeadArgs &a = q.h;
+    const int n = blockIdx.x;
+    float best, best_l, second;
+    int best_i;
+    if (!head_scan<T>(a, n, best, best_i, best_l, second)) return;
+    if (threadIdx.x != 0) return;
+    if (a.out_margin) a.out_margin[n] = fminf(best_l - second, fabsf(best_l - a.conf_logit));
+    const bool keep = (best_i != 0x7fffffff) && (best > a.conf);
+    q.sel_anchor[n] = keep ? best_i : -1;
+    q.sel_score[n] = best;
+    if (!keep || (q.n_dyn && n >= *q.n_dyn)) return;
+    const int A0 = a.lh[0] * a.lw[0], A1 = a.lh[1] * a.lw[1];
+    const int lvl = best_i < A0 ? 0 : (best_i < A0 + A1 ? 1 : 2);
+    const int j = best_i - (lvl == 0 ? 0 : (lvl == 1 ? A0 : A0 + A1));
+    const int H = a.lh[lvl], W = a.lw[lvl], S = q.S[lvl], pitch = q.pitch[lvl], ld = q.ld[lvl];
+    const int y = j / W, x = j % W;
+    unsigned char *live0 = q.live + q.off0[lvl], *live1 = q.live + q.off1[lvl];
+    for (int dy = -1; dy <= 1; ++dy)
+        for (int dx = -1; dx <= 1; ++dx) {
+            const int yy = y + dy, xx = x + dx;
+            if (yy < 0 || yy >= H || xx < 0 || xx >= W) continue;
+            const int s = xx / S;
+            const int u = s * ld + (((n * (H + 1) + yy) * pitch + (xx - s * S)) >> 7);
+            live0[u] = 1;
+            if (dy == 0 && dx == 0) live1[u] = 1;
+        }
+}
+
+template <typename T>
+__global__ __launch_bounds__(64) void head_decode_kernel(const HeadSparseArgs q) {
+    const int n = blockIdx.x;
+    const int best_i = q.sel_anchor[n];
+    head_row<T>(q.h, n, best_i >= 0, best_i, q.sel_score[n]);
 }
 
 constexpr float kNmsMaxWh = 7680.f;
@@ -305,6 +355,17 @@
     return hipGetLastError();
 }
 
+hipError_t launch_head_select_sparse(const HeadSparseArgs &a, hipStream_t stream) {
+    if (a.h.N <= 0 || a.h.nc < 1 || a.h.cls_ld < a.h.nc || !a.live || !a.sel_anchor || !a.sel_score) return hipErrorInvalidValue;
+    hipLaunchKernelGGL((head_select_kernel_sparse<float>), dim3(a.h.N), dim3(1024), 0, stream, a);
+    return hipGetLastError();
+}
+hipError_t launch_head_decode(const HeadSparseArgs &a, hipStream_t stream) {
+    if (a.h.N <= 0 || !a.sel_anchor || !a.sel_score || !a.h.out_xywh) return hipErrorInvalidValue;
+    hipLaunchKernelGGL((head_decode_kernel<float>), dim3(a.h.N), dim3(64), 0, stream, a);
+    return hipGetLastError();
+}
+
 hipError_t launch_head(const HeadArgs &a, int is_f16, hipStream_t stream) {
     if (a.N <= 0 || a.nc < 1 || a.cls_ld < a.nc) return hipErrorInvalidValue;
     if (is_f16)
diff --git a/wtracker_amd/csrc/wtk_internal.h b/wtracker_amd/csrc/wtk_internal.h
--- a/wtracker_amd/csrc/wtk_internal.h
+++ b/wtracker_amd/csrc/wtk_internal.h
@@ -109,6 +109,7 @@
     PROF_HALO = 4,
     PROF_FUSED = 5,
     PROF_C32 = 6,
+    PROF_SPARSE = 7,
 };
 
 enum LaunchKind { L_IGEMM, L_IGEMM_SPLIT, L_WIDE_1X1, L_HALO, L_HALO_SPLIT, L_C32, L_C32_SPLIT, L_WS64, L_S2WIN, L_S2WIN_SPLIT, L_SK };
@@ -159,6 +160,15 @@
     int use_wide = 1;
     int use_c2f = 0;
     int use_front = 0;
+    int use_sparse_box = 1;
+    struct DetLevel {
+        int op0 = -1, box1 = -1, box2 = -1;
+    } det[3];
+    size_t live_bytes = 0;
+    int *sel_anchor = nullptr;
+    float *sel_score = nullptr;
+    int sparse_B = 0;
+    ConvLaunch sparse_done[6];
     int num_cus = 0;
     int latency = 0;
     int sk_group = 1;
@@ -178,7 +188,7 @@
     int *status_dev = nullptr;
     int status_static = 0;
     int profiling = 0;
-    static constexpr int kProfKernels = 7, kProfEvents = 96;
+    static constexpr int kProfKernels = 8, kProfEvents = 96;
     hipEvent_t ev[kProfEvents];
     static constexpr int kSideStreams = 3;
     hipStream_t side_stream[kSideStreams] = {};
@@ -193,6 +203,10 @@
 };
 
 namespace wtk {
+constexpr int kSparseBlockPx = 256, kSparseMinRounds = 4;
+inline bool sparse_box_pays(int B, int h8, int w8, int num_cus) {
+    return num_cus > 0 && (long long)B * (h8 + 1) * (w8 + 1) >= (long long)kSparseMinRounds * kSparseBlockPx * num_cus;
+}
 int pooled_stream(int device, hipStream_t *s);
 void unpool_stream(int device, hipStream_t s);
 }
diff --git a/wtracker_amd/csrc/wtk_kernels.h b/wtracker_amd/csrc/wtk_kernels.h
--- a/wtracker_amd/csrc/wtk_kernels.h
+++ b/wtracker_amd/csrc/wtk_kernels.h
@@ -235,9 +235,12 @@
     int deep;
     int narrow;
     int grid;
+    unsigned live_off;
     const int *n_dyn;
     FastDiv d_bps, d_strips, d_pitch, d_nct, d_h1;
-};
+    int live_ld;
+};
+static_assert(sizeof(HaloArgs) == 288, "live_off / live_ld fill padding: the struct of a dense launch is what it was before the live mask");
 bool halo_eligible(int k, int stride, int cin, int is_f16);
 bool split_halo_eligible(int k, int stride, int cin, int cout);
 int split_halo_cout_tile(int cout_stored);
@@ -381,6 +384,18 @@
 };
 hipError_t launch_head(const HeadArgs &a, int is_f16, hipStream_t stream);
 
+struct HeadSparseArgs {
+    HeadArgs h;
+    unsigned char *live;
+    int *sel_anchor;
+    float *sel_score;
+    int S[3], pitch[3], ld[3];
+    unsigned off0[3], off1[3];
+    const int *n_dyn;
+};
+hipError_t launch_head_select_sparse(const HeadSparseArgs &a, hipStream_t stream);
+hipError_t launch_head_decode(const HeadSparseArgs &a, hipStream_t stream);
+
 struct NmsArgs {
     HeadArgs h;
     float iou;
diff --git a/wtracker_amd/csrc/wtk_plan.hip b/wtracker_amd/csrc/wtk_plan.hip
--- a/wtracker_amd/csrc/wtk_plan.hip
+++ b/wtracker_amd/csrc/wtk_plan.hip
@@ -348,6 +348,7 @@
     h->sk_force_tile = tile >= 0 && tile <= 3 ? tile : -1;
     h->sk_force_form = form == 0 || form == 1 ? form : -1;
     h->front_debug = env_int("WTK_FRONT_DEBUG", 0) == 1;
+    h->use_sparse_box = env_int("WTK_NO_SPARSE_BOX", 0) != 1;
     PlanSwitches s;
     s.latency_plan = env_int("WTK_LATENCY_PLAN", -1);
     s.no_side_stream = env_int("WTK_NO_SIDE_STREAM", 0) == 1;
@@ -695,6 +696,7 @@
                 c2.folded = 1;
             }
         }
+        if (!P.failed) h->det[i].op0 = (int)first_op, h->det[i].box1 = (int)first_op + 1, h->det[i].box2 = (int)first_op + 3;
         if (!P.failed && i < 2) {
             for (size_t k = first_op; k < h->ops.size(); ++k) h->ops[k].side = i == 1 ? 2 : 1;
             h->ops[first_op].wait_feat = i;
@@ -793,11 +795,24 @@
         wtk_yolo_destroy(h);
         return fail("wtk_yolo_create: no pinned status word (hipHostMalloc failed, or more than 4096 live handles)");
     }
-    if (dev_alloc(h, &h->zero_page, 256)) {
+    if (h->split && !h->latency && h->use_sparse_box && wtk::sparse_box_pays(h->max_batch, h->lh[0], h->lw[0], h->num_cus)) {
+        size_t total = 0;
+        for (int i = 0; i < 3; ++i) {
+            int S, pitch, strips, bps;
+            halo_geometry_stacked(h->max_batch, h->lh[i], h->lw[i], kHaloRowsMax, &S, &pitch, &strips, &bps, 256);
+            total += 2 * (((size_t)strips * 2 * bps + 3) & ~(size_t)3);
+        }
+        h->live_bytes = total;
+        if (dev_alloc(h, (void **)&h->sel_anchor, sizeof(int) * h->max_batch) || dev_alloc(h, (void **)&h->sel_score, sizeof(float) * h->max_batch)) {
+            wtk_yolo_destroy(h);
+            return 1;
+        }
+    }
+    if (dev_alloc(h, &h->zero_page, 256 + h->live_bytes)) {
         wtk_yolo_destroy(h);
         return 1;
     }
-    if (hipMemset(h->zero_page, 0, 256) != hipSuccess) {
+    if (hipMemset(h->zero_page, 0, 256 + h->live_bytes) != hipSuccess) {
         wtk_yolo_destroy(h);
         return fail("wtk_yolo_create: hipMemset failed");
     }
diff --git a/wtracker_amd/csrc/wtk_run.hip b/wtracker_amd/csrc/wtk_run.hip
--- a/wtracker_amd/csrc/wtk_run.hip
+++ b/wtracker_amd/csrc/wtk_run.hip
@@ -34,8 +34,7 @@
     int max_det;
     int *out_cls, *out_count;
 };
-static int run_head(wtk_yolo *h, int B, int H, int W, float conf, float *out_xywh, float *out_conf, int *out_anchor, hipStream_t st,
-                    const NmsOut *nms = nullptr) {
+static HeadArgs head_args(wtk_yolo *h, int B, int H, int W, float conf, float *out_xywh, float *out_conf, int *out_anchor) {
     HeadArgs a;
     std::memset(&a, 0, sizeof(a));
     for (int i = 0; i < 3; ++i) {
@@ -58,6 +57,11 @@
     a.out_margin = h->o_margin;
     a.status = h->status_dev;
     a.conf_logit = conf > 0.f && conf < 1.f ? std::log(conf / (1.f - conf)) : (conf <= 0.f ? -INFINITY : INFINITY);
+    return a;
+}
+static int run_head(wtk_yolo *h, int B, int H, int W, float conf, float *out_xywh, float *out_conf, int *out_anchor, hipStream_t st,
+                    const NmsOut *nms = nullptr) {
+    const HeadArgs a = head_args(h, B, H, W, conf, out_xywh, out_conf, out_anchor);
     if (nms) {
         NmsArgs q;
         std::memset(&q, 0, sizeof(q));
@@ -245,6 +249,60 @@
     return 0;
 }
 
+struct SparseBox {
+    ConvLaunch cls0[3], box0[3], box1[3];
+    HeadSparseArgs hs;
+    int level_of_op0(const wtk_yolo *h, size_t oi) const {
+        for (int l = 0; l < 3; ++l)
+            if ((int)oi == h->det[l].op0) return l;
+        return -1;
+    }
+    bool skips(const wtk_yolo *h, size_t oi) const {
+        for (int l = 0; l < 3; ++l)
+            if ((int)oi == h->det[l].box1 || (int)oi == h->det[l].box2) return true;
+        return false;
+    }
+};
+
+static bool resolve_sparse(const wtk_yolo *h, int B, SparseBox &sp) {
+    if (!h->use_sparse_box || !h->split || h->latency || !h->live_bytes) return false;
+    if (!sparse_box_pays(B, h->lh[0], h->lw[0], h->num_cus)) return false;
+    std::memset(&sp.hs, 0, sizeof(sp.hs));
+    unsigned off = 0;
+    for (int l = 0; l < 3; ++l) {
+        const wtk_yolo::DetLevel &d = h->det[l];
+        if (d.op0 < 0 || d.box1 < 0 || d.box2 < 0) return false;
+        const Op &o0 = h->ops[d.op0], &b1 = h->ops[d.box1], &b2 = h->ops[d.box2];
+        if (o0.folded || o0.tail_op >= 0 || o0.cout != h->dims.hb + h->dims.hc || h->dims.hb != 64 || h->dims.hc % 64 || b1.tail_op != d.box2 || !b2.folded) return false;
+        ConvLaunch r0, r1;
+        if (resolve_conv(h, o0, B, r0) || resolve_conv(h, b1, B, r1)) return false;
+        if (r0.kind != L_HALO_SPLIT || r1.kind != L_HALO_SPLIT || r0.g.res || r0.g.out2 || r1.g.res || r1.g.out2) return false;
+        if (split_halo_cout_tile(o0.cout) != 64 || r0.g.narrow || r1.g.narrow) return false;
+        if (r0.g.S != r1.g.S || r0.g.pitch != r1.g.pitch || r0.g.strips != r1.g.strips) return false;
+        const int ld = 2 * (int)(((long long)B * (h->lh[l] + 1) * r0.g.pitch + 255) / 256);
+        const unsigned bytes = ((unsigned)r0.g.strips * (unsigned)ld + 3u) & ~3u;
+        sp.hs.S[l] = r0.g.S, sp.hs.pitch[l] = r0.g.pitch, sp.hs.ld[l] = ld;
+        sp.hs.off0[l] = off, sp.hs.off1[l] = off + bytes;
+        off += 2 * bytes;
+        if (off > h->live_bytes) return false;
+        const int hb = h->dims.hb;
+        sp.box0[l] = r0;
+        sp.box0[l].g.Cout = sp.box0[l].g.CoutPad = hb;
+        sp.box0[l].g.live_off = 256u + sp.hs.off0[l], sp.box0[l].g.live_ld = ld;
+        sp.cls0[l] = r0;
+        HaloArgs &c = sp.cls0[l].g;
+        c.Cout = c.CoutPad = o0.cout - hb, c.narrow = 1;
+        c.w = reinterpret_cast<const char *>(c.w) + (size_t)hb * c.Kpad * 2;
+        c.bias = c.bias + hb;
+        c.out_coff += 2 * hb;
+        sp.box1[l] = r1;
+        sp.box1[l].g.live_off = 256u + sp.hs.off1[l], sp.box1[l].g.live_ld = ld;
+    }
+    sp.hs.live = reinterpret_cast<unsigned char *>(h->zero_page) + 256;
+    sp.hs.sel_anchor = h->sel_anchor, sp.hs.sel_score = h->sel_score, sp.hs.n_dyn = h->n_dyn;
+    return true;
+}
+
 constexpr long long kOpKeyBase = 100000;
 static long long choice_key(long long launch, int B) { return (launch << 24) | (long long)B; }
 
@@ -292,6 +350,7 @@
     hipStream_t main_st;
     bool two_lanes = false;
     unsigned side_used = 0;
+    const struct SparseBox *sparse = nullptr;
     int cur_class = -1, nev = 0;
     int ev_class[wtk_yolo::kProfEvents];
     long long launches[wtk_yolo::kProfKernels] = {};
@@ -378,6 +437,7 @@
     if (h->use_c2f && (oi == 3 || oi == 4)) return 0;
     if (op.folded) return 0;
     if (h->use_c2f && oi == 5) return enqueue_c2f(p, op);
+    if (p.sparse && p.sparse->skips(h, oi)) return 0;
     hipStream_t st = p.main_st;
     if (p.two_lanes && op.side) {
         const int sidx = std::min(op.side, h->side_streams);
@@ -406,6 +466,12 @@
         a.buf = b.ptr, a.N = p.B, a.H = b.h, a.W = b.w, a.c = op.cin, a.split = h->split;
         HIP_TRY(launch_sppf_pool(a, h->is_f16, st));
         p.count(PROF_POOL);
+        return 0;
+    }
+    if (const int l = p.sparse ? p.sparse->level_of_op0(h, oi) : -1; l >= 0) {
+        const ConvLaunch &c = p.sparse->cls0[l];
+        if (mark(p, c.cls) || issue_conv(h, op, c, st)) return 1;
+        p.count(c.cls, p.op_flops(op) * h->dims.hc / (h->dims.hb + h->dims.hc));
         return 0;
     }
     ConvLaunch r;
@@ -459,9 +525,55 @@
     return 0;
 }
 
+static int enqueue_sparse_tail(Pass &p, const SparseBox &sp, int H, int W, float conf, float *out_xywh, float *out_conf, int *out_anchor) {
+    wtk_yolo *h = p.h;
+    hipStream_t st = p.main_st;
+    HeadSparseArgs hs = sp.hs;
+    hs.h = head_args(h, p.B, H, W, conf, out_xywh, out_conf, out_anchor);
+    if (mark(p, PROF_HEAD)) return 1;
+    HIP_TRY(hipMemsetAsync(hs.live, 0, h->live_bytes, st));
+    HIP_TRY(launch_head_select_sparse(hs, st));
+    p.count(PROF_HEAD);
+    if (mark(p, PROF_SPARSE)) return 1;
+    for (int l = 0; l < 3; ++l) {
+        if (issue_conv(h, h->ops[h->det[l].op0], sp.box0[l], st)) return 1;
+        p.count(PROF_SPARSE);
+    }
+    for (int l = 0; l < 3; ++l) {
+        if (issue_conv(h, h->ops[h->det[l].box1], sp.box1[l], st)) return 1;
+        p.count(PROF_SPARSE);
+    }
+    if (mark(p, PROF_HEAD)) return 1;
+    HIP_TRY(launch_head_decode(hs, st));
+    p.count(PROF_HEAD);
+    h->sparse_B = p.B;
+    for (int l = 0; l < 3; ++l) {
+        h->sparse_done[l] = sp.box0[l], h->sparse_done[3 + l] = sp.box1[l];
+        h->sparse_done[l].g.live_off = h->sparse_done[3 + l].g.live_off = 0;
+        h->sparse_done[l].g.live_ld = h->sparse_done[3 + l].g.live_ld = 0;
+    }
+    return 0;
+}
+
+static int complete_box_towers(wtk_yolo *h) {
+    if (!h->sparse_B) return 0;
+    for (int l = 0; l < 3; ++l)
+        if (issue_conv(h, h->ops[h->det[l].op0], h->sparse_done[l], nullptr)) return 1;
+    for (int l = 0; l < 3; ++l)
+        if (issue_conv(h, h->ops[h->det[l].box1], h->sparse_done[3 + l], nullptr)) return 1;
+    HIP_TRY(hipDeviceSynchronize());
+    h->sparse_B = 0;
+    return 0;
+}
+
 static int yolo_enqueue_pass(wtk_yolo *h, const uint8_t *frames_dev, int32_t B, int32_t H, int32_t W, int32_t C, float conf, float *out_xywh,
                              float *out_conf, int32_t *out_anchor, hipStream_t st, const ViewSrc *vs, const NmsOut *nms) {
     Pass p{h, frames_dev, B, C, st};
+    SparseBox sp;
+    if (!nms && resolve_sparse(h, B, sp)) {
+        hipStreamCaptureStatus cs = hipStreamCaptureStatusNone;
+        if (hipStreamIsCapturing(st, &cs) == hipSuccess && cs == hipStreamCaptureStatusNone) p.sparse = &sp;
+    }
     if (enqueue_input(p, frames_dev, H, W, vs)) return 1;
     const bool grouped = h->latency && h->sk_group && !h->lat_sched.empty();
     if (!grouped && h->use_side && h->side_streams > 0 && !h->profiling && ensure_side_streams(h)) return 1;
@@ -479,9 +591,14 @@
             HIP_TRY(hipEventRecord(h->side_done[i], h->side_stream[i]));
             HIP_TRY(hipStreamWaitEvent(st, h->side_done[i], 0));
         }
-    if (mark(p, PROF_HEAD)) return 1;
-    if (run_head(h, B, H, W, conf, out_xywh, out_conf, out_anchor, st, nms)) return 1;
-    p.count(PROF_HEAD);
+    if (p.sparse) {
+        if (enqueue_sparse_tail(p, sp, H, W, conf, out_xywh, out_conf, out_anchor)) return 1;
+    } else {
+        h->sparse_B = 0;
+        if (mark(p, PROF_HEAD)) return 1;
+        if (run_head(h, B, H, W, conf, out_xywh, out_conf, out_anchor, st, nms)) return 1;
+        p.count(PROF_HEAD);
+    }
     if (!h->profiling) return 0;
     if (p.nev < wtk_yolo::kProfEvents) {
         HIP_TRY(hipEventRecord(h->ev[p.nev], st));
@@ -682,6 +799,7 @@
     if (!h || level < 0 || level > 2 || B <= 0 || B > h->max_batch) return fail("wtk_yolo_debug_head: bad argument");
     DEVICE_GUARD(h);
     HIP_TRY(hipDeviceSynchronize());
+    if (box_host && complete_box_towers(h)) return 1;
     const size_t A = (size_t)h->lh[level] * h->lw[level];
     if (box_host) {
         const size_t n = (size_t)B * A * 64;
@@ -710,6 +828,10 @@
     if (out_cap < px * op->cout) return fail("wtk_yolo_debug_tensor: output buffer too small");
     DEVICE_GUARD(h);
     HIP_TRY(hipDeviceSynchronize());
+    for (int l = 0; l < 3; ++l) {
+        const int oi = (int)(op - h->ops.data());
+        if ((oi == h->det[l].op0 || oi == h->det[l].box1 || oi == h->det[l].box2) && complete_box_towers(h)) return 1;
+    }
     std::vector<char> tmp(px * b.C * (b.f32 ? 4 : h->esize));
     HIP_TRY(hipMemcpy(tmp.data(), b.ptr, tmp.size(), hipMemcpyDeviceToHost));
     std::vector<float> full(px * b.C);
@@ -788,5 +910,6 @@
         HIP_TRY(hipMemcpy(h->bufs[h->cls_buf[l]].ptr, cl.data(), cl.size() * 4, hipMemcpyHostToDevice));
         a0 += Al;
     }
-    return 0;
-}
+    h->sparse_B = 0;
+    return 0;
+}
diff --git a/wtracker_amd/hip.py b/wtracker_amd/hip.py
--- a/wtracker_amd/hip.py
+++ b/wtracker_amd/hip.py
@@ -553,7 +553,7 @@
         return out
 
     KERNELS = ["stem_mfma_kernel", "conv_igemm_kernel+conv1x1_wide_kernel", "sppf_pool_kernel", "head", "conv3x3_halo_kernel",
-               "front_fused_kernel+c2f32_fused_kernel", "conv3x3_c32_kernel"]
+               "front_fused_kernel+c2f32_fused_kernel", "conv3x3_c32_kernel", "conv3x3_halo_kernel(sparse box towers)"]
 
     def get_kernel_profile(self) -> dict:
         out = {}
```

After: 11470 frames/s, median of 6. 5.1% higher.
